# aurelienpierreeng/ansel

Hardware: AMD Instinct MI355X
Metric: MPix/s full export pixelpipe (100 MP raw); % MI355X HBM roofline (higher is better)
Workload: dtype f32

## Files before the change

### __graft_entry__.py

```python
import os
import subprocess
import sys

ROOT = os.path.dirname(os.path.abspath(__file__))
if ROOT not in sys.path:
    sys.path.insert(0, ROOT)


def build():
    from ansel_amd import build as b
    b.build()
    subprocess.check_call(["make", "-s", "-C", os.path.join(ROOT, "oracle"), "oracle"])
    subprocess.check_call(["make", "-s", "-C", os.path.join(ROOT, "oracle"), "ref"])
    nat = os.path.join(ROOT, "tests", "native")
    so = os.path.join(nat, "libdevmath_host.so")
    src = os.path.join(nat, "devmath_host.cpp")
    hdr = os.path.join(ROOT, "ansel_amd", "csrc", "devmath.h")
    if not os.path.exists(so) or os.path.getmtime(so) < max(os.path.getmtime(src), os.path.getmtime(hdr)):
        subprocess.check_call(["g++", "-O2", "-std=c++17", "-mfma", "-ffp-contract=off", "-fPIC", "-shared",
                               "-I" + os.path.join(ROOT, "ansel_amd", "csrc"), src, "-o", so, "-lm"])
    so = os.path.join(nat, "libnlm2_host.so")
    src = os.path.join(nat, "nlm2_host.cpp")
    hdrs = [os.path.join(ROOT, "ansel_amd", "csrc", h) for h in ("nlm2_body.h", "nlm3_body.h", "nlm_tail_body.h")]
    if not os.path.exists(so) or os.path.getmtime(so) < max([os.path.getmtime(src)] + [os.path.getmtime(h) for h in hdrs]):
        subprocess.check_call(["g++", "-O2", "-std=c++20", "-ffp-contract=off", "-fPIC", "-shared", "-pthread",
                               "-I" + os.path.join(ROOT, "ansel_amd", "csrc"), src, "-o", so])
    sys.path.insert(0, os.path.join(ROOT, "tests"))
    import test_amaze_host
    test_amaze_host.build()
    if os.path.isdir("/root/reference/src"):
        sys.path.insert(0, os.path.join(ROOT, "tests"))
        import test_boundary_compile
        test_boundary_compile.build()
    ex = os.path.join(ROOT, "examples", "export_pipe")
    subprocess.check_call(["gcc", "-std=c99", "-O2", "-Wall", "-I" + os.path.join(ROOT, "include"), ex + ".c",
                           "-L" + os.path.join(ROOT, "ansel_amd"), "-lansel_hip", "-Wl,-rpath,$ORIGIN/../ansel_amd", "-o", ex])
    import ansel_amd
    from ansel_amd import lib
    l = lib.load()
    if l._ansel_missing:
        raise RuntimeError("libansel_hip.so lacks: %s" % l._ansel_missing)


def smoke():
    sys.path.insert(0, os.path.join(ROOT, "tests"))
    import numpy as np
    import checkers as ck
    import hipcheck as hc
    from ansel_amd import filmic, lib, params, pipe, synth
    hc.hip()
    w, h = 400, 300
    raw = synth.bayer_mosaic(w, h, seed=1)
    lut = params.srgb_encode_lut()
    coeffs = params.unbounded_coeffs(lut)
    d_lut = lib.DeviceBuffer.from_numpy(0, lut)
    dev_nodes = pipe.light_pipe_nodes(w, h, d_lut.ptr, float(lut[0]), coeffs, with_filmic=True, filmic=filmic.default_data())
    d_in = lib.DeviceBuffer.from_numpy(0, raw)
    d_out = lib.DeviceBuffer(0, w * h * 8)
    p = pipe.DevicePipe(0, dev_nodes, fusion=True)
    groups = p.num_groups
    p.process(d_in.ptr, d_out.ptr)
    assert lib.load().dt_hip_finish(0) == 1
    got = d_out.to_numpy((h, w, 4), np.uint16)
    p.close()
    o = ck.oracle()
    assert o is not None, "oracle/liboracle.so missing: run build()"
    host_nodes = pipe.light_pipe_nodes(w, h, lut.ctypes.data, float(lut[0]), coeffs, with_filmic=True,
                                       filmic=filmic.default_data())
    src = raw
    for n in host_nodes:
        if n.op == "export_u16":
            exp = np.zeros((h, w, 4), np.uint16)
            o.oracle_export_convert_u16(w, h, ck.ptr(src), ck.ptr(exp))
            break
        dst = np.zeros((h, w) if n.op in ("rawprepare", "temperature", "highlights") else (h, w, 4), np.float32)
        assert ck.call(o, "oracle_" + n.op, n.piece, n.data, np.ascontiguousarray(src), dst) == 0, n.op
        src = dst
    bad = int((got != exp).sum())
    assert bad == 0, "smoke: %d of %d output words differ from the oracle" % (bad, got.size)
    print("smoke ok: %d-module light pipe, %d launch groups, %dx%d bit-exact vs oracle on %s"
          % (len(dev_nodes), groups, w, h, hc.hip().dt_hip_get_device_name(0).decode()))


if __name__ == "__main__":
    build()
    if len(sys.argv) > 1 and sys.argv[1] == "smoke":
        smoke()
```

### ansel_amd/csrc/hip_common.h

```cpp
#pragma once
#include <hip/hip_runtime.h>
#include <stdint.h>
#include <stdio.h>
#include <string.h>
#include "ansel_hip.h"
#include "dev_buf.h"

#ifdef ANSEL_HIP_MEASURING
#include <stdlib.h>
static inline const char *measuring_env(const char *name) { return getenv(name); }
#else
static inline constexpr const char *measuring_env(const char *) { return nullptr; }
#endif

namespace ansel
{

enum dispatch_key_t
{
  DISPATCH_NLM_V2 = 0,
  DISPATCH_NLM_FUSED,
  DISPATCH_AMAZE_UNFUSED,
  DISPATCH_AMAZE_SLAB,
  DISPATCH_AMAZE_BLOCKS,
  DISPATCH_BILAT_BLUR_SPLIT,
  DISPATCH_STRIP_ROWS,
  DISPATCH_KEYS
};
int dispatch_override(dispatch_key_t key);

static inline int strip_rows(const int gx, const int classes, const int per_class, const int longest = 32)
{
  const int forced = dispatch_override(DISPATCH_STRIP_ROWS);
  if(forced) return forced;
  int strip = longest;
  while(strip > 4 && (size_t)gx * classes * ((per_class + strip - 1) / strip) < 2048) strip /= 2;
  return strip;
}

void set_last_error(const char *fmt, ...);

hipStream_t stream_of(int devid);
int upload_small(int devid, void *dst_dev, const void *src_host, size_t bytes);
bool make_current(int devid);
int hip_device_of(int devid);
bool valid_device(int devid);

struct launch_scope
{
  int devid;
  const char *tag;
  hipEvent_t start, stop;
  bool active;
  launch_scope(int devid, const char *tag);
  ~launch_scope();
};

static inline int check_launch(const char *what)
{
  const hipError_t e = hipGetLastError();
  if(e != hipSuccess)
  {
    set_last_error("%s: %s", what, hipGetErrorString(e));
    return DT_HIP_DEFAULT_ERROR;
  }
  return DT_HIP_SUCCESS;
}

#define ANSEL_HIP_CHECK(expr)                                                                   \
  do                                                                                            \
  {                                                                                             \
    const hipError_t _e = (expr);                                                               \
    if(_e != hipSuccess)                                                                        \
    {                                                                                           \
      ansel::set_last_error("%s:%d %s: %s", __FILE__, __LINE__, #expr, hipGetErrorString(_e));  \
      return DT_HIP_DEFAULT_ERROR;                                                              \
    }                                                                                           \
  } while(0)

typedef float v4f_t __attribute__((ext_vector_type(4)));
__device__ __forceinline__ void nt_store(float4 *p, const float4 v)
{
  const v4f_t t = { v.x, v.y, v.z, v.w };
  __builtin_nontemporal_store(t, reinterpret_cast<v4f_t *>(p));
}

template <typename T> __device__ __forceinline__ const T &kernarg_at(const int offset)
{
  typedef const T __attribute__((address_space(4))) *p4;
  return *(const T *)(p4)((const char __attribute__((address_space(4))) *)__builtin_amdgcn_kernarg_segment_ptr() + offset);
}
template <typename T, typename... Before> constexpr int kernarg_offset_after()
{
  size_t off = 0;
  ((off = (off + alignof(Before) - 1) / alignof(Before) * alignof(Before) + sizeof(Before)), ...);
  return (int)((off + alignof(T) - 1) / alignof(T) * alignof(T));
}

static inline unsigned xcd_pad(const int gx) { return (unsigned)((gx + 7) / 8) * 8; }
__device__ __forceinline__ int xcd_col() { return (int)((blockIdx.x + blockIdx.y / 64) % gridDim.x); }

#define HL_MIN_CLIPPED 25
struct hl_journal
{
  unsigned long long count;
  unsigned long long index[HL_MIN_CLIPPED];
  float value[HL_MIN_CLIPPED];
};
int highlights_resolve_launch(int devid, float *out, const hl_journal *journal);

struct rcd_band_t
{
  int tv0, tv1;
  int in_row0, in_rows;
  int out_row0, out_rows;
};

struct band_view_t
{
  int frame_h;
  int buf_row0;
  int row0, row1;
};
int nlmeans_halo_rows(const dt_hip_piece_t *piece, const dt_hip_nlmeans_data_t *d);
int nlmeans_process_band(int devid, const dt_hip_piece_t *piece, const dt_hip_nlmeans_data_t *d, const band_view_t *band,
                         dt_hip_mem_t dev_in, dt_hip_mem_t dev_out);
int diffuse_halo_rows(const dt_hip_piece_t *piece, const dt_hip_diffuse_data_t *d);
int diffuse_process_rows(int devid, const dt_hip_piece_t *piece, const dt_hip_diffuse_data_t *d, int first_row,
                         dt_hip_mem_t dev_in, dt_hip_mem_t dev_out);
int diffuse_process_post_lab(int devid, const dt_hip_piece_t *piece, const dt_hip_diffuse_data_t *d, dt_hip_mem_t dev_in,
                             dt_hip_mem_t dev_out, const dt_hip_lab_data_t *lab);
int denoiseprofile_halo_rows(const dt_hip_piece_t *piece, const dt_hip_denoiseprofile_data_t *d);
struct dn_band_job_t;
int denoiseprofile_band_begin(int devid, const dt_hip_piece_t *piece, const dt_hip_denoiseprofile_data_t *d,
                              const band_view_t *band, int buf_rows, dt_hip_mem_t dev_in, dt_hip_mem_t dev_out,
                              dn_band_job_t **job);
int denoiseprofile_band_step(dn_band_job_t *job, dt_hip_mem_t *halo_buf, int *halo_rows, double **sums, size_t *sum_count);
int denoiseprofile_band_finish(dn_band_job_t *job, dt_hip_mem_t dev_out);
void denoiseprofile_band_abort(dn_band_job_t *job);
int guided_filter_launch(int devid, const float4 *guide, float *mask, int width, int height, int w, float sqrt_eps,
                         float guide_weight, float minv, float maxv);
int detail_refine_launch(int devid, const float *rawdetail, const float *form, float fill, float level, int width, int height,
                         float *refined);
int bilat_band_supported(const dt_hip_piece_t *piece, const dt_hip_bilat_data_t *d);
int blend_refines_with_detail_mask(const dt_hip_blend_data_t *d);
int bilat_band_begin(int devid, const dt_hip_piece_t *piece, const dt_hip_bilat_data_t *d, dt_hip_mem_t *grid, size_t *bytes);
int bilat_band_splat(int devid, const dt_hip_piece_t *piece, const dt_hip_bilat_data_t *d, dt_hip_mem_t grid,
                     dt_hip_mem_t in_rows, int row0, int rows);
int bilat_band_finish(int devid, const dt_hip_piece_t *piece, const dt_hip_bilat_data_t *d, dt_hip_mem_t grid,
                      dt_hip_mem_t in_rows, dt_hip_mem_t out_rows, int row0, int rows);

static inline unsigned stream_grid(size_t work_items, unsigned block)
{
  size_t g = (work_items + block - 1) / block;
  if(g > 2048u * 4u) g = 2048u * 4u;
  if(g < 1) g = 1;
  return (unsigned)g;
}

static inline unsigned pixel_grid(size_t pixels)
{
  const size_t g = (pixels + 255) / 256;
  return (unsigned)(g < 1 ? 1 : (g > 0x7fffffffu ? 0x7fffffffu : g));
}

}
```

### ansel_amd/csrc/nlm3_body.h

```cpp
#pragma once

#include "nlm2_body.h"

#include <type_traits>

#define NL3_THREADS 1024
#define NL3_TP 84
#define NL3_XO 3
#define NL3_FP 80
#define NL3_WPH 46
#define NL3_A1_LANES 384

namespace nlm3
{
using nlm2::f2;
using nlm2::imin;

struct alignas(16) f4
{
  float x, y, z, w;
};

#ifdef __HIPCC__
NLM2_FN f4 ld4(const float *const p) { return *reinterpret_cast<const f4 *>(p); }
NLM2_FN void st4(float *const p, const f4 v) { *reinterpret_cast<f4 *>(p) = v; }
NLM2_FN f2 ld2(const float *const p) { return *reinterpret_cast<const f2 *>(p); }
NLM2_FN void st2(float *const p, const f2 v) { *reinterpret_cast<f2 *>(p) = v; }
#else
NLM2_FN f4 ld4(const float *const p)
{
  f4 v;
  __builtin_memcpy(&v, p, 16);
  return v;
}
NLM2_FN void st4(float *const p, const f4 v) { __builtin_memcpy(p, &v, 16); }
NLM2_FN f2 ld2(const float *const p)
{
  f2 v;
  __builtin_memcpy(&v, p, 8);
  return v;
}
NLM2_FN void st2(float *const p, const f2 v) { __builtin_memcpy(p, &v, 8); }
#endif

template <int NPXL> constexpr int max_rows() { return NPXL == 9 ? 56 : 74; }

template <int P> constexpr int a1_segments() { return P == 1 ? 3 : 2; }

template <int NPXL, int P = 2> inline size_t lds_floats(const int chk_h, const int reach)
{
  return (size_t)4 * max_rows<NPXL>() * NL3_TP + 2 * (2 * P + 1) * NL3_FP + (size_t)(chk_h + 2 * reach) * 2 * NL3_WPH * 3;
}

constexpr int FUSED_MAXCH = 64;
template <int NPXL, int P = 2> inline size_t lds_floats_fused(const int chk_h, const int reach)
{
  return (size_t)3 * FUSED_MAXCH * NL3_TP + 2 * (2 * P + 1) * NL3_FP + (size_t)(chk_h + 2 * reach) * 2 * NL3_WPH * 3;
}
template <int MSEG, int P> inline bool a1_fits(const int chk_w, const int chk_h)
{
  constexpr int S = 2 * P + 1, NSEG = a1_segments<P>(), NCH = S * NSEG;
  static_assert(NCH <= 10, "one chain per half-wave of the five main A1 waves");
  const int ncp = (chk_w + 2 * P + 1) / 2;
  if(ncp < 32 || NCH * (ncp - 32) > 64) return false;
  const int m0 = (chk_h - 2) / S + 1;
  return (m0 + NSEG - 1) / NSEG <= MSEG;
}
template <int NPXL, int MSEG, int P = 2> inline bool fits_fused(const int chk_w, const int chk_h, const int radius, const int reach)
{
  constexpr int S = 2 * P + 1, LPR = (72 + NPXL - 1) / NPXL;
  if(radius != P || chk_w > 72 || (chk_w & 1) || chk_w + 2 * reach > 2 * NL3_WPH || chk_h > FUSED_MAXCH || chk_h < 2 * S) return false;
  if(LPR != 8) return false;
  return a1_fits<MSEG, P>(chk_w, chk_h);
}

template <int NPXL, int MSEG, int P = 2> inline bool fits(const int chk_w, const int chk_h, const int radius, const int reach)
{
  constexpr int S = 2 * P + 1, LPR = (72 + NPXL - 1) / NPXL;
  if(radius != P || chk_w > 72 || (chk_w & 1) || chk_w + 2 * reach > 2 * NL3_WPH || chk_h > max_rows<NPXL>() || chk_h < 2 * S) return false;
  if(LPR * chk_h > 448) return false;
  return a1_fits<MSEG, P>(chk_w, chk_h);
}

inline constexpr bool border_fits(const int cw, const int ch) { return ch >= 10 && cw >= 1; }

template <class I2> inline bool regular_grid(const I2 *const patches, const int n, int *const ndx_out)
{
  if(n < 1) return false;
  int ndx = 1;
  while(ndx < n && patches[ndx].x == patches[0].x) ndx++;
  if(n % ndx) return false;
  for(int p = 0; p < n; p++)
  {
    const int row = p / ndx, j = p - row * ndx;
    if(patches[p].x != patches[row * ndx].x || patches[p].y != patches[0].y + j) return false;
  }
  *ndx_out = ndx;
  return true;
}

template <int T0, int T1, int ROWBYTES, class Env, bool BLOCKS = false> struct column_chain
{
  static NLM2_FN void run(const Env &env, float *const wave_base, const int lane, float &v, const float *const term)
  {
    if constexpr(BLOCKS && T0 + 8 <= T1)
    {
      env.template chain8<T0, ROWBYTES>(wave_base, lane, v, term);
      if constexpr(T0 + 8 < T1) column_chain<T0 + 8, T1, ROWBYTES, Env, BLOCKS>::run(env, wave_base, lane, v, term);
    }
    else
    {
      v = v + term[T0];
      env.template st_addtid<T0 * ROWBYTES>(wave_base, lane, v);
      if constexpr(T0 + 1 < T1) column_chain<T0 + 1, T1, ROWBYTES, Env, BLOCKS>::run(env, wave_base, lane, v, term);
    }
  }
};

constexpr int TALL_HEAD = 64;
constexpr int TALL_SEED_PITCH = 80;
template <int NPXL, int MSEG, bool BORDER = false, bool FUSED = false, bool TALL = false, int P = 2, bool CENTER = false, class Env,
          class Args, class F4, class I2>
NLM2_FN void body(const Env &env, const F4 *__restrict__ in, F4 *__restrict__ out, const Args &a, const I2 *__restrict__ patches,
                  const int ndx, float *__restrict__ seeds_out = nullptr)
{
  static_assert(!TALL || FUSED, "the head of a tall chunk runs on the fused body");
  constexpr int S = 2 * P + 1, TP = NL3_TP, XO = NL3_XO, FP = NL3_FP, WPH = NL3_WPH;
  constexpr int NSEG = a1_segments<P>(), NCH = S * NSEG;
  constexpr int MAXCH = FUSED ? FUSED_MAXCH : max_rows<NPXL>();
  constexpr int NT = FUSED ? 3 : 4;
  auto tslot = [](const int p) { return FUSED ? p % 3 : (p & 3); };
  constexpr int LPR = (72 + NPXL - 1) / NPXL;
  const int tid = env.tid();
  const int W = a.W, H = a.H;
  const int cy_launch = env.bid() / a.nchx, cx = env.bid() - cy_launch * a.nchx;
  const int cy = cy_launch + a.cy0;
  const int top = cy * a.chk_h, left = cx * a.chk_w;
  const int bot = imin(top + a.chk_h, H), right = imin(left + a.chk_w, W);
  const int ch_grid = bot - top, cw = right - left;
  const int reach = a.reach;
  const bool interior = top >= reach && bot + reach <= H && left >= reach && right + reach <= W && ch_grid == a.chk_h && cw == a.chk_w;
  const int ch = TALL ? imin(TALL_HEAD, ch_grid) : ch_grid;
  if(BORDER ? (interior || !border_fits(cw, ch)) : !interior) return;

  float *const lds = env.lds();
  constexpr int tabsz = MAXCH * TP;
  const int wh = ch + 2 * reach;
  const int n = a.npatch, ndy = n / ndx;
  float *const XY = lds;
  float *const Z = XY + 2 * (wh * 2 * WPH);
  float *const tab = Z + wh * 2 * WPH;
  float *const Fb = tab + NT * tabsz;
  const int r0 = top - reach, c0 = left - reach;
  const float n0 = a.norm[0], n1 = a.norm[1], n2 = a.norm[2];
  const int ww = cw + 2 * reach;

  for(int i0 = tid; i0 < wh * 2 * WPH; i0 += 4 * NL3_THREADS)
  {
    F4 v[4];
#pragma unroll
    for(int u = 0; u < 4; u++)
    {
      const int i = i0 + u * NL3_THREADS;
      const int wy = i / (2 * WPH), rem = i - wy * (2 * WPH);
      const int par = rem / WPH, h = rem - par * WPH;
      const int wx = 2 * h + par;
      const int r = r0 + wy, c = c0 + wx;
      v[u].x = v[u].y = v[u].z = v[u].w = 0.0f;
      if(i < wh * 2 * WPH && wx < ww && c < W && (!BORDER || (r >= 0 && r < H && c >= 0))) v[u] = in[(long)r * W + c];
    }
#pragma unroll
    for(int u = 0; u < 4; u++)
    {
      const int i = i0 + u * NL3_THREADS;
      if(i < wh * 2 * WPH)
      {
        f2 xy;
        xy.x = v[u].x;
        xy.y = v[u].y;
        st2(XY + 2 * i, xy);
        Z[i] = v[u].z;
      }
    }
  }
  env.sync();
  auto widx = [&](const int wy, const int wx) { return (wy * 2 + (wx & 1)) * WPH + (wx >> 1); };

  const int w = tid >> 6, lane = tid & 63;
#if defined(__HIPCC__) && !defined(ANSEL_HIP_MEASURING)
  constexpr int var = 0;
#else
  const int var = a.variant;
#endif
  const bool lay1 = !FUSED && !CENTER && (var & 4096);
  const int a1_index = FUSED ? ((w >= 2 && w <= 7) ? w - 2 : -1)
                       : CENTER ? (w == 7 ? 0 : (w == 11 ? 1 : (w >= 12 ? w - 10 : -1)))
                                : (lay1 ? ((w >= 3 && w <= 6) ? w - 3 : ((w == 8 || w == 9) ? w - 4 : -1))
                                        : (w == 3 ? 0 : ((w >= 4 && w <= 7) ? w - 3 : (w == 10 ? 5 : -1))));
  const int c_index = FUSED ? w - 8
                      : CENTER ? (w <= 6 ? w - 3 : w - 4)
                               : (lay1 ? (w == 7 ? 0 : w - 9) : (w == 8 ? 0 : (w == 9 ? 1 : w - 9)));
  if(a1_index >= 0)
  {
    const int ai = a1_index;
    const int ncp = (cw + 2 * P + 1) / 2;
    constexpr int nseg = NSEG;
    const int m0 = (ch - 2) / S + 1;
    const int mseg = (m0 + nseg - 1) / nseg;
    const int extra = ncp - 32;
    int g, q;
    if(ai < 5)
    {
      q = imin(2 * ai + (lane >> 5), NCH - 1);
      g = lane & 31;
    }
    else
    {
      const int l = extra > 0 ? imin(lane, S * nseg * extra - 1) : 0;
      q = extra > 0 ? l / extra : 0;
      g = extra > 0 ? 32 + l - q * extra : 0;
    }
    const int k = q % S, seg = q / S;
    const int mk = (ch - 2 - k >= 0) ? (ch - 2 - k) / S + 1 : 0;
    const int j0 = seg * mseg;
    const int left_over = mk - j0;
    const int jn = left_over < 0 ? 0 : (left_over > mseg ? mseg : left_over);
    const bool head = seg == 0;
    const int wr0 = reach - P + k + j0 * S;
    const int x0 = 1 + 2 * g;
    const int wc0 = reach - P - 1 + x0;
    constexpr int RSTEP = S * 2 * WPH;
    const int rowbase = wr0 * 2 * WPH;
    constexpr int DUMMY = 0;
    const int toff0 = (1 + k + j0 * S) * TP + XO + x0;
    const int foff = k * FP + XO + x0;
    float ox[MSEG + 1][2], oy[MSEG + 1][2], oz[MSEG + 1][2];
#pragma unroll
    for(int i = 0; i <= MSEG; i++)
#pragma unroll
      for(int c = 0; c < 2; c++)
      {
        const int wx = wc0 + c;
        const int wi = rowbase + i * RSTEP + (wx & 1) * WPH + (wx >> 1);
        const f2 v = ld2(XY + 2 * wi);
        ox[i][c] = v.x;
        oy[i][c] = v.y;
        oz[i][c] = Z[wi];
      }
    bool own_row[MSEG + 1], row_ok[MSEG + 1], own_col[2];
#pragma unroll
    for(int i = 0; i <= MSEG; i++)
    {
      const int R = r0 + wr0 + i * S;
      own_row[i] = row_ok[i] = !BORDER || (R >= 0 && R < H);
    }
#pragma unroll
    for(int c = 0; c < 2; c++) own_col[c] = !BORDER || (c0 + wc0 + c >= 0 && c0 + wc0 + c < W);
    float sx[MSEG + 1][2], sy[MSEG + 1][2], sz[MSEG + 1][2];
#pragma unroll
    for(int i = 0; i <= MSEG; i++) sx[i][0] = sx[i][1] = sy[i][0] = sy[i][1] = sz[i][0] = sz[i][1] = 0.0f;

    auto load_row_head = [&](const int dy, const int dx) {
      const int dyo = rowbase + dy * 2 * WPH;
#pragma unroll
      for(int c = 0; c < 2; c++)
      {
        const int wx = wc0 + c + dx;
        const int base = dyo + (wx & 1) * WPH + (wx >> 1);
#pragma unroll
        for(int i = 0; i <= MSEG; i++)
        {
          const int wi = base + i * RSTEP;
          const f2 v = ld2(XY + 2 * wi);
          sx[i][c] = v.x;
          sy[i][c] = v.y;
          sz[i][c] = Z[wi];
        }
      }
    };
    auto step = [&](auto ph_tag, const int p, const int dx) {
      constexpr int PH = decltype(ph_tag)::value;
      float *const T = tab + tslot(p) * tabsz;
      float *const F = Fb + (p & 1) * S * FP;
      const int fo = head ? foff : DUMMY;
      bool col_ok[2] = { true, true };
      if(BORDER)
      {
#pragma unroll
        for(int c = 0; c < 2; c++) col_ok[c] = own_col[c] && (unsigned)(c0 + wc0 + c + dx) < (unsigned)W;
      }
      float px2[2], py2[2], pz2[2];
#pragma unroll
      for(int c = 0; c < 2; c++)
      {
        const int sl = (c + PH) & 1;
        const float dx_ = ox[0][c] - sx[0][sl], dy_ = oy[0][c] - sy[0][sl], dz_ = oz[0][c] - sz[0][sl];
        px2[c] = dx_ * dx_;
        py2[c] = dy_ * dy_;
        pz2[c] = dz_ * dz_;
        if(BORDER && !(row_ok[0] && col_ok[c])) px2[c] = py2[c] = pz2[c] = 0.0f;
      }
      {
        f2 d;
        d.x = px2[0] * n0 + py2[0] * n1 + pz2[0] * n2;
        d.y = px2[1] * n0 + py2[1] * n1 + pz2[1] * n2;
        st2(F + fo, d);
      }
#pragma unroll
      for(int i = 1; i <= MSEG; i++)
      {
        f2 t;
        float nx2[2], ny2[2], nz2[2];
#pragma unroll
        for(int c = 0; c < 2; c++)
        {
          const int sl = (c + PH) & 1;
          const float dx_ = ox[i][c] - sx[i][sl], dy_ = oy[i][c] - sy[i][sl], dz_ = oz[i][c] - sz[i][sl];
          nx2[c] = dx_ * dx_;
          ny2[c] = dy_ * dy_;
          nz2[c] = dz_ * dz_;
          if(BORDER && !(row_ok[i] && col_ok[c])) nx2[c] = ny2[c] = nz2[c] = 0.0f;
        }
        t.x = ((nx2[0] - px2[0]) * n0 + (ny2[0] - py2[0]) * n1) + (nz2[0] - pz2[0]) * n2;
        t.y = ((nx2[1] - px2[1]) * n0 + (ny2[1] - py2[1]) * n1) + (nz2[1] - pz2[1]) * n2;
        if(i - 1 < jn) st2(T + toff0 + (i - 1) * S * TP, t);
        env.sched_fence();
#pragma unroll
        for(int c = 0; c < 2; c++)
        {
          px2[c] = nx2[c];
          py2[c] = ny2[c];
          pz2[c] = nz2[c];
        }
      }
    };
    auto slide = [&](auto ph_tag, const int dy, const int dx) {
      constexpr int PH = decltype(ph_tag)::value;
      const int wx = wc0 + 1 + dx + 1;
      const int base = rowbase + dy * 2 * WPH + (wx & 1) * WPH + (wx >> 1);
#pragma unroll
      for(int i = 0; i <= MSEG; i++)
      {
        const int wi = base + i * RSTEP;
        const f2 v = ld2(XY + 2 * wi);
        sx[i][PH] = v.x;
        sy[i][PH] = v.y;
        sz[i][PH] = Z[wi];
      }
    };
    for(int dyi = 0; dyi < ndy; dyi++)
    {
      const int dy = patches[dyi * ndx].x, dx0 = patches[dyi * ndx].y;
      if(BORDER)
      {
#pragma unroll
        for(int i = 0; i <= MSEG; i++) row_ok[i] = own_row[i] && (unsigned)(r0 + wr0 + i * S + dy) < (unsigned)H;
      }
      if(!(var & 16)) load_row_head(dy, dx0);
      for(int jb = 0; jb < ndx; jb += 2)
      {
        if(!(var & 16))
        {
          step(std::integral_constant<int, 0>(), dyi * ndx + jb, dx0 + jb);
          slide(std::integral_constant<int, 0>(), dy, dx0 + jb);
        }
        env.sync();
        if(jb + 1 < ndx)
        {
          if(!(var & 16))
          {
            step(std::integral_constant<int, 1>(), dyi * ndx + jb + 1, dx0 + jb + 1);
            slide(std::integral_constant<int, 1>(), dy, dx0 + jb + 1);
          }
          env.sync();
        }
      }
    }
    env.sync();
    env.sync();
    if(!FUSED) env.sync();
    return;
  }
  if(w < 2)
  {
    const int x = 1 + w * 64 + lane;
    const bool active = x <= cw + 2 * P && !(var & 32);
    if(!(var & 512)) env.prio_high();
    env.sync();
    for(int p = 0; p < n; p++)
    {
      if(active)
      {
        float *const col = tab + tslot(p) * tabsz + XO + x;
        const float *const F = Fb + (p & 1) * S * FP + XO + x;
        float f[S], term[MAXCH];
#pragma unroll
        for(int r = 0; r < S; r++) f[r] = F[r * FP];
#pragma unroll
        for(int t = 1; t < MAXCH; t++) term[t] = col[t * TP];
        float v = 0.0f;
#pragma unroll
        for(int r = 0; r < S; r++) v += f[r];
        float *const wave_base = tab + tslot(p) * tabsz + XO + 1 + w * 64;
        env.template st_addtid<0>(wave_base, lane, v);
        column_chain<1, MAXCH, TP * 4, Env, !FUSED && P == 2 && !CENTER>::run(env, wave_base, lane, v, term);
        if constexpr(TALL)
        {
          static_assert(!TALL || MAXCH == TALL_HEAD, "the exported sum is the one behind the head's last row");
          seeds_out[(size_t)p * TALL_SEED_PITCH + x] = v;
        }
      }
      env.sync();
    }
    env.sync();
    if(!FUSED) env.sync();
    return;
  }
  if(!FUSED && w == 2)
  {
    const bool active = lane < ch && !(var & 64);
    if(!(var & 512)) env.prio_high();
    env.sync();
    env.sync();
    for(int p = 0; p < n; p++)
    {
      if(active)
      {
        float *const rowp = tab + (p & 3) * tabsz + lane * TP;
        float cs[80];
#pragma unroll
        for(int b = 4; b < 80; b += 4)
        {
          const f4 v = ld4(rowp + b);
          cs[b] = v.x;
          cs[b + 1] = v.y;
          cs[b + 2] = v.z;
          cs[b + 3] = v.w;
        }
        cs[XO] = 0.0f;
        float distortion = 0.0f;
#pragma unroll
        for(int kk = 1; kk < S; kk++) distortion += cs[XO + kk];
        float d[72];
#pragma unroll
        for(int b = 0; b < 72; b += 4)
        {
#pragma unroll
          for(int c = b; c < b + 4; c++)
          {
            distortion = distortion + (cs[XO + c + S] - cs[XO + c]);
            d[c] = distortion;
          }
          f4 v;
          v.x = d[b];
          v.y = d[b + 1];
          v.z = d[b + 2];
          v.w = d[b + 3];
          st4(rowp + 4 + b, v);
          if(!(var & 1024)) env.sched_fence();
        }
      }
      env.sync();
    }
    env.sync();
    return;
  }
  {
    constexpr int NR = CENTER ? NPXL : NPXL + 1;
    constexpr int DB = CENTER ? 1 : 2;
    constexpr int AB = CENTER ? 1 : 3;
    static_assert(CENTER || NR % 2 == 0, "the distortions alternate between two register sets with the ring's period");
    const int ci = c_index;
    static_assert(LPR == 8, "the lane layout of the C role");
    const int r = 8 * ci + 2 * ((lane & 31) >> 3) + (lane >> 5), j8 = lane & 7;
    const int cb = NPXL * j8;
    const bool active = r < ch && cb < cw && !(var & 128);
    float accx[NPXL], accy[NPXL], accz[NPXL], accw[NPXL];
    float qx[NR], qy[NR], qz[NR];
    float dist[DB][NPXL];
    unsigned reached[2] = { ~0u, ~0u };
#pragma unroll
    for(int i = 0; i < NPXL; i++) accx[i] = accy[i] = accz[i] = accw[i] = dist[0][i] = dist[DB - 1][i] = 0.0f;
#pragma unroll
    for(int i = 0; i < NR; i++) qx[i] = qy[i] = qz[i] = 0.0f;
    const int doff = r * TP + 4 + cb;
    const float sharp_m23 = a.sharpness * -8388608.0f;
    [[maybe_unused]] float ox[CENTER ? NPXL : 1], oy[CENTER ? NPXL : 1], oz[CENTER ? NPXL : 1];
    [[maybe_unused]] const float cden = 1.0f + a.center_weight;
    [[maybe_unused]] const float crcp = Env::rcp_refined(cden);
    if constexpr(CENTER)
    {
#pragma unroll
      for(int i = 0; i < NPXL; i++)
      {
        const int wi = widx(reach + r, reach + cb + i);
        const f2 v = ld2(XY + 2 * wi);
        ox[i] = v.x;
        oy[i] = v.y;
        oz[i] = Z[wi];
      }
    }
    [[maybe_unused]] float cs[NPXL + S];
    [[maybe_unused]] const bool row_head = j8 == 0;
    [[maybe_unused]] auto fetch_sums = [&](const int p) {
      const float *const T = tab + tslot(p) * tabsz + r * TP + XO + cb;
#pragma unroll
      for(int i = 0; i < NPXL + S; i++) cs[i] = T[i];
    };
    [[maybe_unused]] auto row_chain = [&](auto m_tag) {
      constexpr int M = decltype(m_tag)::value;
      float e[NPXL];
      e[0] = cs[S] - (row_head ? 0.0f : cs[0]);
#pragma unroll
      for(int i = 1; i < NPXL; i++) e[i] = cs[i + S] - cs[i];
      float first = 0.0f;
#pragma unroll
      for(int kk = 1; kk < S; kk++) first += cs[kk];
      float carry = first;
#pragma unroll
      for(int ph = 0; ph < LPR; ph++)
      {
        float d = carry;
#pragma unroll
        for(int i = 0; i < NPXL; i++)
        {
          d = d + e[i];
          dist[M & (DB - 1)][i] = d;
        }
        if(ph + 1 < LPR)
        {
          const float from_left = env.lane_shr1(d);
          carry = row_head ? first : from_left;
        }
      }
    };

    auto fetch = [&](auto m_tag, const int p, const bool first, const int dy, const int dx) {
      constexpr int M = decltype(m_tag)::value;
      if constexpr(!FUSED)
      {
        const float *const T = tab + (p & 3) * tabsz + doff;
#pragma unroll
        for(int i = 0; i < NPXL; i++) dist[M & (DB - 1)][i] = T[i];
      }
      if(BORDER)
      {
        unsigned m = 0;
        if((unsigned)(top + r + dy) < (unsigned)H)
        {
#pragma unroll
          for(int i = 0; i < NPXL; i++) m |= ((unsigned)(left + cb + i + dx) < (unsigned)W ? 1u : 0u) << i;
        }
        reached[M & (DB - 1)] = m;
      }
      const int wy = reach + r + dy;
      if(first)
      {
#pragma unroll
        for(int i = 0; i < NPXL; i++)
        {
          const int wi = widx(wy, reach + cb + i + dx);
          const f2 v = ld2(XY + 2 * wi);
          qx[i] = v.x;
          qy[i] = v.y;
          qz[i] = Z[wi];
        }
      }
      else
      {
        constexpr int SL = (NPXL - 1 + M) % NR;
        const int wi = widx(wy, reach + cb + NPXL - 1 + dx);
        const f2 v = ld2(XY + 2 * wi);
        qx[SL] = v.x;
        qy[SL] = v.y;
        qz[SL] = Z[wi];
      }
    };
    auto accumulate = [&](auto m_tag) {
      constexpr int M = decltype(m_tag)::value;
      static_assert(NPXL % AB == 0, "accumulate() takes the pixels of a lane AB at a time");
#pragma unroll
      for(int g = 0; g < NPXL; g += AB)
      {
        float v[AB], wgt[AB], t[AB];
        int k0[AB];
        if constexpr(CENTER)
        {
          float cx2[AB], cy2[AB], cz2[AB];
#pragma unroll
          for(int j = 0; j < AB; j++)
          {
            const float dx_ = ox[g + j] - qx[(g + j + M) % NR], dy_ = oy[g + j] - qy[(g + j + M) % NR], dz_ = oz[g + j] - qz[(g + j + M) % NR];
            cx2[j] = dx_ * dx_ * a.cpn;
            cy2[j] = dy_ * dy_ * a.cpn;
            cz2[j] = dz_ * dz_ * a.cpn;
          }
          env.sched_fence();
#pragma unroll
          for(int j = 0; j < AB; j++) v[j] = dist[M & (DB - 1)][g + j] + (cx2[j] + cy2[j] + cz2[j]);
          env.sched_fence();
#pragma unroll
          for(int j = 0; j < AB; j++) v[j] = Env::div_uniform(v[j], cden, crcp);
          env.sched_fence();
#pragma unroll
          for(int j = 0; j < AB; j++) v[j] = Env::min_num(0.0f, v[j] * sharp_m23 + 16777216.0f);
          env.sched_fence();
        }
        else
        {
#pragma unroll
          for(int j = 0; j < AB; j++) v[j] = dist[M & (DB - 1)][g + j] * sharp_m23;
          env.sched_fence();
#pragma unroll
          for(int j = 0; j < AB; j++) v[j] = Env::max_num(v[j], -__builtin_inff());
          env.sched_fence();
        }
#pragma unroll
        for(int j = 0; j < AB; j++) k0[j] = Env::cvt_i32_sat(v[j]);
        env.sched_fence();
#pragma unroll
        for(int j = 0; j < AB; j++) k0[j] = (int)(0x3f800000u + (unsigned)k0[j]);
        env.sched_fence();
#pragma unroll
        for(int j = 0; j < AB; j++)
        {
          wgt[j] = Env::int_as_float(k0[j] >= 0x800000 ? k0[j] : 0);
          if(BORDER && !(reached[M & (DB - 1)] >> (g + j) & 1u)) wgt[j] = 0.0f;
        }
        env.sched_fence();
#pragma unroll
        for(int j = 0; j < AB; j++) t[j] = qx[(g + j + M) % NR] * wgt[j];
        env.sched_fence();
#pragma unroll
        for(int j = 0; j < AB; j++) accx[g + j] = accx[g + j] + t[j];
#pragma unroll
        for(int j = 0; j < AB; j++) t[j] = qy[(g + j + M) % NR] * wgt[j];
        env.sched_fence();
#pragma unroll
        for(int j = 0; j < AB; j++) accy[g + j] = accy[g + j] + t[j];
#pragma unroll
        for(int j = 0; j < AB; j++) t[j] = qz[(g + j + M) % NR] * wgt[j];
        env.sched_fence();
#pragma unroll
        for(int j = 0; j < AB; j++) accz[g + j] = accz[g + j] + t[j];
#pragma unroll
        for(int j = 0; j < AB; j++) accw[g + j] = accw[g + j] + 1.0f * wgt[j];
        env.sched_fence();
      }
    };
    env.sync();
    env.sync();
    if(!FUSED) env.sync();
    for(int dyi = 0; dyi < ndy; dyi++)
    {
      const int dy = patches[dyi * ndx].x, dx0 = patches[dyi * ndx].y;
      for(int jb = 0; jb < ndx; jb += NR)
      {
        auto run = [&](auto m_tag) {
          constexpr int M = decltype(m_tag)::value;
          if constexpr(M < NR)
          {
            if(jb + M < ndx)
            {
              if constexpr(CENTER)
              {
                if(active && jb + M > 0) accumulate(std::integral_constant<int, (M + NR - 1) % NR>());
                if constexpr(FUSED) fetch_sums(dyi * ndx + jb + M);
                if(active) fetch(m_tag, dyi * ndx + jb + M, jb + M == 0, dy, dx0 + jb + M);
                if constexpr(FUSED)
                {
                  if(!(var & 64)) row_chain(m_tag);
                }
                if(active && jb + M + 1 == ndx) accumulate(m_tag);
              }
              else if constexpr(FUSED)
              {
                if(active && jb + M > 0) accumulate(std::integral_constant<int, (M + NR - 1) % NR>());
                env.sched_fence();
                fetch_sums(dyi * ndx + jb + M);
                if(active) fetch(m_tag, dyi * ndx + jb + M, jb + M == 0, dy, dx0 + jb + M);
                if(!(var & 64)) row_chain(m_tag);
                if(active && jb + M + 1 == ndx) accumulate(m_tag);
              }
              else if(active)
              {
                if(jb + M > 0) accumulate(std::integral_constant<int, (M + NR - 1) % NR>());
                env.sched_fence();
                fetch(m_tag, dyi * ndx + jb + M, jb + M == 0, dy, dx0 + jb + M);
                if(jb + M + 1 == ndx) accumulate(m_tag);
              }
              env.sync();
            }
          }
        };
        run(std::integral_constant<int, 0>());
        run(std::integral_constant<int, 1>());
        run(std::integral_constant<int, 2>());
        run(std::integral_constant<int, 3>());
        run(std::integral_constant<int, 4>());
        run(std::integral_constant<int, 5>());
        run(std::integral_constant<int, 6>());
        run(std::integral_constant<int, 7>());
        run(std::integral_constant<int, 8>());
        run(std::integral_constant<int, 9>());
        if constexpr(NR > 10)
        {
          run(std::integral_constant<int, 10>());
          run(std::integral_constant<int, 11>());
          run(std::integral_constant<int, 12>());
          run(std::integral_constant<int, 13>());
        }
      }
    }
    if(!active) return;
    const int row = top + r;
    if(row < a.out_row0 || row >= a.out_row1) return;
#pragma unroll
    for(int i = 0; i < NPXL; i++)
    {
      if(cb + i >= cw) continue;
      const long o = (long)row * W + left + cb + i;
      F4 res;
      if(a.skip_blend)
      {
        res.x = accx[i] / accw[i];
        res.y = accy[i] / accw[i];
        res.z = accz[i] / accw[i];
        res.w = accw[i] / accw[i];
      }
      else
      {
        const F4 ip = in[o];
        res.x = (ip.x * (1.0f - a.luma)) + (accx[i] / accw[i] * a.luma);
        res.y = (ip.y * (1.0f - a.chroma)) + (accy[i] / accw[i] * a.chroma);
        res.z = (ip.z * (1.0f - a.chroma)) + (accz[i] / accw[i] * a.chroma);
        res.w = (ip.w * 0.0f) + (accw[i] / accw[i] * 1.0f);
      }
      out[o] = res;
      env.store_cell(a, o, res.x);
    }
  }
}

}
```

### ansel_amd/csrc/nlmeans.hip

```cpp
#include "hip_common.h"
#include "nlmeans_core_params.h"
#include "nlm2_body.h"
#include "ieee_inrange.h"
#include "px_bilat.h"
#include "nlm3_body.h"
#include "nlm_tail_body.h"

#include <math.h>
#include <algorithm>
#include <vector>
#include <type_traits>

using namespace ansel;

namespace
{

#define SLICE_WIDTH 72
#define SLICE_HEIGHT 60
#define NLM_THREADS 1024
#define MAX_PX_PER_THREAD 5
#define CS_LANES 128

struct nlm_args
{
  int W, H;
  int chk_w, chk_h, nchx;
  int radius, npatch;
  int cs_pitch, wt_pitch;
  float sharpness, center_weight, inv_den;
  float cpn;
  float norm[3];
  float luma, chroma;
  int skip_blend;
  int reach;
  int win_pitch;
  int cy0, out_row0, out_row1;
  int variant;
  float2 *zc;
  float zc_sigma_r;
  int zc_size_z;
};

__device__ __forceinline__ void nlm_store_cell(const nlm_args &a, const long o, const float L)
{
  if(a.zc)
  {
    float zf;
    const int zi = bilat_axis(L, a.zc_sigma_r, a.zc_size_z, zf);
    a.zc[o] = make_float2(zf, __int_as_float(zi));
  }
}

__device__ __forceinline__ int imin(const int a, const int b) { return a < b ? a : b; }
__device__ __forceinline__ int imax(const int a, const int b) { return a > b ? a : b; }

__device__ __forceinline__ int cvtt(const float v)
{
  return (v >= -2147483648.0f && v < 2147483648.0f) ? (int)v : (int)0x80000000;
}

__device__ __forceinline__ float mexp2(const float x)
{
  const int k0 = (int)(0x3f800000u + (unsigned)cvtt(x * -8388608.0f));
  return __int_as_float(k0 >= 0x800000 ? k0 : 0);
}

__device__ __forceinline__ float pixdiff(const float4 a, const float4 b, const float n0, const float n1, const float n2)
{
  const float dx = a.x - b.x, dy = a.y - b.y, dz = a.z - b.z;
  return dx * dx * n0 + dy * dy * n1 + dz * dz * n2;
}

__device__ __forceinline__ float pixdiff2(const float4 a, const float4 b, const float4 c, const float4 d, const float n0,
                                          const float n1, const float n2)
{
  const float ax = a.x - b.x, ay = a.y - b.y, az = a.z - b.z;
  const float cx = c.x - d.x, cy = c.y - d.y, cz = c.z - d.z;
  return (ax * ax - cx * cx) * n0 + (ay * ay - cy * cy) * n1 + (az * az - cz * cz) * n2;
}

template <bool STAGED> struct pixel_source
{
  const float4 *in;
  const float *wr, *wg, *wb;
  int W, r0, c0, pitch;
  __device__ __forceinline__ float4 operator()(const int r, const int c) const
  {
    if(STAGED)
    {
      const int i = (r - r0) * pitch + (c - c0);
      return make_float4(wr[i], wg[i], wb[i], 0.0f);
    }
    return in[(long)r * W + c];
  }
};

template <bool STAGED>
__global__ __launch_bounds__(NLM_THREADS) void nlm_chunks(const float4 *__restrict__ in, float4 *__restrict__ out,
                                                          const nlm_args a, const int2 *__restrict__ patches)
{
  extern __shared__ float lds[];
  const int tid = threadIdx.x;
  const int cy_launch = blockIdx.x / a.nchx, cx = blockIdx.x - cy_launch * a.nchx;
  const int cy = cy_launch + a.cy0;
  const int top = cy * a.chk_h, left = cx * a.chk_w;
  const int bot = imin(top + a.chk_h, a.H), right = imin(left + a.chk_w, a.W);
  const int ch = bot - top, cw = right - left;
  const int P = a.radius, W = a.W, H = a.H;
  const int csw = a.chk_w + 2 * P + 1;
  const int cs0 = left - P - 1;
  float *const cs = lds;
  float *const dist = lds + (a.chk_h + 16) * a.cs_pitch;
  const float n0 = a.norm[0], n1 = a.norm[1], n2 = a.norm[2];

  pixel_source<STAGED> px;
  px.in = in;
  px.W = W;
  px.r0 = top - a.reach;
  px.c0 = left - a.reach;
  px.pitch = a.win_pitch;
  if(STAGED)
  {
    float *const win = dist + a.chk_h * a.wt_pitch;
    const int wh = a.chk_h + 2 * a.reach, plane = wh * a.win_pitch;
    px.wr = win;
    px.wg = win + plane;
    px.wb = win + 2 * plane;
    for(int i = tid; i < plane; i += NLM_THREADS)
    {
      const int wy = i / a.win_pitch, wx = i - wy * a.win_pitch;
      const int r = px.r0 + wy, c = px.c0 + wx;
      float4 v = make_float4(0.f, 0.f, 0.f, 0.f);
      if(r >= 0 && r < H && c >= 0 && c < W) v = in[(long)r * W + c];
      win[i] = v.x;
      win[i + plane] = v.y;
      win[i + 2 * plane] = v.z;
    }
    __syncthreads();
  }

  float4 acc[MAX_PX_PER_THREAD];
  int rc[MAX_PX_PER_THREAD];
#pragma unroll
  for(int k = 0; k < MAX_PX_PER_THREAD; k++)
  {
    acc[k] = make_float4(0.f, 0.f, 0.f, 0.f);
    const int idx = tid + NLM_THREADS * k;
    const int r = idx / cw;
    rc[k] = idx < ch * cw ? ((r << 16) | (idx - r * cw)) : -1;
  }

  for(int p = 0; p < a.npatch; p++)
  {
    const int srow = patches[p].x, scol = patches[p].y;
    const int row_min = imax(top, imax(0, -srow)), row_max = imin(bot, H - imax(0, srow));
    if(row_min >= row_max) continue;
    const int row_top = imax(row_min, imax(P, P - srow));
    const int row_bot = imin(row_max, H - 1 - imax(P, P + srow));
    const int col_min = imax(left, -scol), col_max = imin(right, W - scol);
    const int pc_min = left - imin(P, imin(left, left + scol));
    const int pc_max = right + imin(P, imin(W - right, W - (right + scol)));
    const int nrows = row_max - row_min;
    const int first_end = imin(row_top, row_bot);

    const int ci = tid & (CS_LANES - 1);
    for(int t = tid / CS_LANES; t < nrows; t += NLM_THREADS / CS_LANES)
    {
      if(ci >= csw) continue;
      const int c = cs0 + ci;
      float v = 0.0f;
      if(c >= pc_min && c < pc_max)
      {
        if(t == 0)
        {
          const int row = row_min;
          const int rmin = row - imin(P, imin(row, row + srow));
          const int rmax = row + imin(P, imin(H - 1 - row, H - 1 - (row + srow)));
          for(int r = rmin; r <= rmax; r++) v += pixdiff(px(r, c), px(r + srow, c + scol), n0, n1, n2);
        }
        else
        {
          const int row = row_min + t - 1;
          if(row < first_end)
          {
            const int b = row + 1 + P;
            v = pixdiff(px(b, c), px(b + srow, c + scol), n0, n1, n2);
          }
          else if(row < row_bot)
          {
            const int b = row + 1 + P, tt = row - P;
            v = pixdiff2(px(b, c), px(b + srow, c + scol), px(tt, c), px(tt + srow, c + scol), n0, n1, n2);
          }
          else if(row >= row_top)
          {
            const int tt = row - P;
            v = pixdiff(px(tt, c), px(tt + srow, c + scol), n0, n1, n2);
          }
        }
      }
      cs[t * a.cs_pitch + ci] = v;
    }
    __syncthreads();

    if(tid < csw)
    {
      float v = cs[tid];
      for(int t0 = 1; t0 < nrows; t0 += 16)
      {
        float term[16];
        float *const col = cs + t0 * a.cs_pitch + tid;
#pragma unroll
        for(int u = 0; u < 16; u++) term[u] = col[u * a.cs_pitch];
#pragma unroll
        for(int u = 0; u < 16; u++)
        {
          const int row = row_min + t0 + u - 1;
          const bool live = t0 + u < nrows;
          const float plus = v + term[u], minus = v - term[u];
          v = (live && row < row_bot) ? plus : ((live && row >= row_top) ? minus : v);
          term[u] = v;
        }
#pragma unroll
        for(int u = 0; u < 16; u++) col[u * a.cs_pitch] = term[u];
      }
    }
    __syncthreads();

    if(tid < nrows)
    {
      const float *const row_cs = cs + tid * a.cs_pitch - cs0;
      float distortion = 0.0f;
      for(int i = col_min - P; i < imin(col_min + P, col_max); i++) distortion += row_cs[i];
      float *const drow = dist + (row_min + tid - top) * a.wt_pitch - left;
      for(int c0 = col_min; c0 < col_max; c0 += 16)
      {
        float hi[16], lo[16];
#pragma unroll
        for(int u = 0; u < 16; u++)
        {
          hi[u] = row_cs[c0 + u + P];
          lo[u] = row_cs[c0 + u - P - 1];
        }
#pragma unroll
        for(int u = 0; u < 16; u++)
        {
          const float next = distortion + (hi[u] - lo[u]);
          distortion = (c0 + u < col_max) ? next : distortion;
          hi[u] = distortion;
        }
#pragma unroll
        for(int u = 0; u < 16; u++) drow[c0 + u] = hi[u];
      }
    }
    __syncthreads();

#pragma unroll
    for(int k = 0; k < MAX_PX_PER_THREAD; k++)
    {
      if(rc[k] < 0) continue;
      const int row = top + (rc[k] >> 16), col = left + (rc[k] & 0xffff);
      if(row < row_min || row >= row_max || col < col_min || col >= col_max) continue;
      const float distortion = dist[(row - top) * a.wt_pitch + (col - left)];
      const float4 q = px(row + srow, col + scol);
      float w;
      if(a.center_weight < 0)
        w = mexp2(distortion * a.sharpness);
      else
      {
        const float dis = (distortion + pixdiff(px(row, col), q, a.cpn, a.cpn, a.cpn)) / (1.0f + a.center_weight);
        w = mexp2(fmaxf(0.0f, dis * a.sharpness - 2.0f));
      }
      acc[k].x += q.x * w;
      acc[k].y += q.y * w;
      acc[k].z += q.z * w;
      acc[k].w += 1.0f * w;
    }
    __syncthreads();
  }

#pragma unroll
  for(int k = 0; k < MAX_PX_PER_THREAD; k++)
  {
    if(rc[k] < 0) continue;
    const int row = top + (rc[k] >> 16), col = left + (rc[k] & 0xffff);
    if(row < a.out_row0 || row >= a.out_row1) continue;
    const long o = (long)row * W + col;
    const float4 s = acc[k];
    float4 r;
    if(a.skip_blend)
      r = make_float4(s.x / s.w, s.y / s.w, s.z / s.w, s.w / s.w);
    else
    {
      const float4 ip = in[o];
      r.x = (ip.x * (1.0f - a.luma)) + (s.x / s.w * a.luma);
      r.y = (ip.y * (1.0f - a.chroma)) + (s.y / s.w * a.chroma);
      r.z = (ip.z * (1.0f - a.chroma)) + (s.z / s.w * a.chroma);
      r.w = (ip.w * 0.0f) + (s.w / s.w * 1.0f);
    }
    out[o] = r;
    nlm_store_cell(a, o, r.x);
  }
}

#define NLP_SERIAL 256
#define NLP_PAR (NLM_THREADS - NLP_SERIAL)
#define NLP_PX 7
#define NLP_WP 96
#define NLP_TP 81

typedef float f2 __attribute__((ext_vector_type(2)));

struct nlm_geom
{
  int srow, scol, row_min, row_max, row_top, row_bot, col_min, col_max, pc_min, pc_max, nrows;
};

__device__ __forceinline__ nlm_geom geom_of(const int2 sh, const int top, const int bot, const int left, const int right,
                                            const int P, const int W, const int H)
{
  nlm_geom g;
  g.srow = sh.x;
  g.scol = sh.y;
  g.row_min = imax(top, imax(0, -g.srow));
  g.row_max = imin(bot, H - imax(0, g.srow));
  g.nrows = g.row_max - g.row_min;
  g.row_top = imax(g.row_min, imax(P, P - g.srow));
  g.row_bot = imin(g.row_max, H - 1 - imax(P, P + g.srow));
  g.col_min = imax(left, -g.scol);
  g.col_max = imin(right, W - g.scol);
  g.pc_min = left - imin(P, imin(left, left + g.scol));
  g.pc_max = right + imin(P, imin(W - right, W - (right + g.scol)));
  return g;
}

__device__ __forceinline__ void pipelined_body(const int chunk, float *const lds, const float4 *__restrict__ in,
                                               float4 *__restrict__ out, const nlm_args &a, const int2 *__restrict__ patches)
{
  const int tid = threadIdx.x;
  const int cy_launch = chunk / a.nchx, cx = chunk - cy_launch * a.nchx;
  const int cy = cy_launch + a.cy0;
  const int top = cy * a.chk_h, left = cx * a.chk_w;
  const int bot = imin(top + a.chk_h, a.H), right = imin(left + a.chk_w, a.W);
  const int ch = bot - top, cw = right - left;
  const int P = a.radius, W = a.W, H = a.H;
  const int csw = a.chk_w + 2 * P + 1;
  const int cs0 = left - P - 1;
  constexpr int pitch = NLP_TP;
  const int tabsz = a.chk_h * pitch;
  float *const win = lds + 2 * tabsz + 16 * pitch + 64;
  const int r0 = top - a.reach, c0 = left - a.reach;
  const float n0 = a.norm[0], n1 = a.norm[1], n2 = a.norm[2];
  const int n = a.npatch;

  {
    const int wh = a.chk_h + 2 * a.reach;
    for(int i = tid; i < wh * NLP_WP; i += NLM_THREADS)
    {
      const int wy = i / NLP_WP, wx = i - wy * NLP_WP;
      const int r = r0 + wy, c = c0 + wx;
      float4 v = make_float4(0.f, 0.f, 0.f, 0.f);
      if(r >= 0 && r < H && c >= 0 && c < W) v = in[(long)r * W + c];
      float *const w = win + wy * 3 * NLP_WP + wx;
      w[0] = v.x;
      w[NLP_WP] = v.y;
      w[2 * NLP_WP] = v.z;
    }
  }

  const bool par = tid >= NLP_SERIAL;
  if(!par) __builtin_amdgcn_s_setprio(3);
  const int u = tid - NLP_SERIAL;
  float4 acc[NLP_PX];
  int prc[NLP_PX];
#pragma unroll
  for(int k = 0; k < NLP_PX; k++)
  {
    acc[k] = make_float4(0.f, 0.f, 0.f, 0.f);
    const int idx = u + NLP_PAR * k;
    const int r = idx / cw, c = idx - r * cw;
    const bool ok = par && idx < ch * cw;
    prc[k] = ok ? ((r << 16) | c) : -1;
  }
  const int wbase0 = ((top - r0) * 3) * NLP_WP + (left - c0);
  int a1[NLP_PX];
#pragma unroll
  for(int k = 0; k < NLP_PX; k++)
  {
    const int idx = u + NLP_PAR * k;
    const int t = idx / (csw - 1), ci = 1 + idx - t * (csw - 1);
    a1[k] = (t * 3 * NLP_WP + ci) | (((t + 1) * pitch + ci) << 16);
  }
  __syncthreads();

  auto run = [&](auto interior_tag) {
    constexpr bool INTERIOR = decltype(interior_tag)::value;
    auto A1 = [&](const nlm_geom &g, float *const T) {
      const int dS = g.srow * 3 * NLP_WP + g.scol;
      const int dT = (2 * P + 1) * 3 * NLP_WP;
      const float *const wb = win + ((g.row_min + 1 + P - r0) * 3) * NLP_WP + (cs0 - c0);
      const int tend = g.nrows * pitch;
      const bool plain = INTERIOR || (g.row_top <= g.row_min && g.row_bot >= g.row_max - 1 && g.pc_min == left - P
                         && g.pc_max == left + a.chk_w + P);
      const f2 n01 = { n0, n1 };
      if(u < g.nrows - 1) T[(u + 1) * pitch] = 0.0f;
      if(plain)
      {
  #pragma unroll
        for(int k = 0; k < NLP_PX; k++)
        {
          if(k == 4) asm volatile("" ::: "memory");
          int pk = a1[k];
          asm volatile("" : "+v"(pk));
          const int ti = (unsigned)pk >> 16;
          if(ti >= tend) continue;
          const float *const pb = wb + (pk & 0xffff);
          const float *const pt = pb - dT;
          const f2 b = { pb[0], pb[NLP_WP] }, bs = { pb[dS], pb[dS + NLP_WP] };
          const f2 l = { pt[0], pt[NLP_WP] }, ls = { pt[dS], pt[dS + NLP_WP] };
          const f2 z = { pb[2 * NLP_WP], pt[2 * NLP_WP] }, zs = { pb[dS + 2 * NLP_WP], pt[dS + 2 * NLP_WP] };
          f2 e = b - bs, q = l - ls, w = z - zs;
          e = e * e;
          q = q * q;
          w = w * w;
          const f2 d = (e - q) * n01;
          T[ti] = d.x + d.y + (w.x - w.y) * n2;
        }
      }
      else
      {
  #pragma unroll
        for(int k = 0; k < NLP_PX; k++)
        {
          if(k == 4) asm volatile("" ::: "memory");
          int pk = a1[k];
          asm volatile("" : "+v"(pk));
          const int ti = (unsigned)pk >> 16;
          if(ti >= tend) continue;
          const int lw = pk & 0xffff;
          const int t = (int)(((unsigned)lw * 58255u) >> 24);
          const int row = g.row_min + t, c = cs0 + (lw - t * 3 * NLP_WP);
          const float *const pb = wb + lw;
          const float *const pt = pb - dT;
          const float ax = pb[0] - pb[dS], ay = pb[NLP_WP] - pb[dS + NLP_WP], az = pb[2 * NLP_WP] - pb[dS + 2 * NLP_WP];
          const float tx = pt[0] - pt[dS], ty = pt[NLP_WP] - pt[dS + NLP_WP], tz = pt[2 * NLP_WP] - pt[dS + 2 * NLP_WP];
          const bool colok = c >= g.pc_min && c < g.pc_max;
          const bool enter = colok && row < g.row_bot, leave = colok && row >= g.row_top;
          const float ex = enter ? ax * ax : 0.f, ey = enter ? ay * ay : 0.f, ez = enter ? az * az : 0.f;
          const float lx = leave ? tx * tx : 0.f, ly = leave ? ty * ty : 0.f, lz = leave ? tz * tz : 0.f;
          T[ti] = (ex - lx) * n0 + (ey - ly) * n1 + (ez - lz) * n2;
        }
      }
    };
    auto A1_first = [&](const nlm_geom &g, float *const T) {
      const int c = cs0 + tid;
      float v = 0.0f;
      if(c >= g.pc_min && c < g.pc_max)
      {
        const int row = g.row_min;
        const int rmin = row - imin(P, imin(row, row + g.srow));
        const int rmax = row + imin(P, imin(H - 1 - row, H - 1 - (row + g.srow)));
        const int dS = g.srow * 3 * NLP_WP + g.scol;
        const float *pr = win + ((rmin - r0) * 3) * NLP_WP + (c - c0);
        for(int r = rmin; r <= rmax; r++, pr += 3 * NLP_WP)
        {
          const float dx = pr[0] - pr[dS], dy = pr[NLP_WP] - pr[dS + NLP_WP], dz = pr[2 * NLP_WP] - pr[dS + 2 * NLP_WP];
          v += dx * dx * n0 + dy * dy * n1 + dz * dz * n2;
        }
      }
      T[tid] = v;
    };
    auto A2 = [&](const nlm_geom &g, float *const T) {
      float v = T[tid];
      int t0 = 1;
      for(; t0 + 16 <= g.nrows; t0 += 16)
      {
        float term[16];
        float *const col = T + t0 * pitch + tid;
  #pragma unroll
        for(int k = 0; k < 16; k++) term[k] = col[k * pitch];
        term[0] = v + term[0];
  #pragma unroll
        for(int k = 1; k < 16; k++) term[k] = term[k - 1] + term[k];
        v = term[15];
  #pragma unroll
        for(int k = 0; k < 16; k++) col[k * pitch] = term[k];
      }
      if(t0 < g.nrows)
      {
        float term[16];
        float *const col = T + t0 * pitch + tid;
        const int live = g.nrows - t0;
  #pragma unroll
        for(int k = 0; k < 16; k++) term[k] = col[k * pitch];
  #pragma unroll
        for(int k = 0; k < 16; k++)
        {
          const float next = v + term[k];
          v = k < live ? next : v;
          term[k] = v;
        }
  #pragma unroll
        for(int k = 0; k < 16; k++)
          if(k < live) col[k * pitch] = term[k];
      }
    };
    auto B = [&](const nlm_geom &g, float *const T, const int rr) {
      float *const rowp = T + rr * pitch - cs0;
      float distortion = 0.0f;
      for(int i = g.col_min - P; i < imin(g.col_min + P, g.col_max); i++) distortion += rowp[i];
      int cb = g.col_min;
      for(; cb + 16 <= g.col_max; cb += 16)
      {
        float hi[16], lo[16];
  #pragma unroll
        for(int k = 0; k < 16; k++)
        {
          hi[k] = rowp[cb + k + P];
          lo[k] = rowp[cb + k - P - 1];
        }
  #pragma unroll
        for(int k = 0; k < 16; k++) hi[k] = hi[k] - lo[k];
        hi[0] = distortion + hi[0];
  #pragma unroll
        for(int k = 1; k < 16; k++) hi[k] = hi[k - 1] + hi[k];
        distortion = hi[15];
  #pragma unroll
        for(int k = 0; k < 16; k++) rowp[cb + k - P - 1] = hi[k];
      }
      if(cb < g.col_max)
      {
        float hi[16], lo[16];
        const int live = g.col_max - cb;
  #pragma unroll
        for(int k = 0; k < 16; k++)
        {
          hi[k] = rowp[cb + k + P];
          lo[k] = rowp[cb + k - P - 1];
        }
  #pragma unroll
        for(int k = 0; k < 16; k++)
        {
          const float next = distortion + (hi[k] - lo[k]);
          distortion = k < live ? next : distortion;
          hi[k] = distortion;
        }
  #pragma unroll
        for(int k = 0; k < 16; k++)
          if(k < live) rowp[cb + k - P - 1] = hi[k];
      }
    };
    auto C = [&](const nlm_geom &g, const float *const T) {
      const int dS = g.srow * 3 * NLP_WP + g.scol;
      const int trow = (g.row_min - top) * pitch;
      const bool whole = INTERIOR || (g.row_min == top && g.row_max == bot && g.col_min == left && g.col_max == right);
      float dist[NLP_PX], qx[NLP_PX], qy[NLP_PX], qz[NLP_PX];
      bool ok[NLP_PX];
  #pragma unroll
      for(int k = 0; k < NLP_PX; k++)
      {
        int pk = prc[k];
        asm volatile("" : "+v"(pk));
        const int r = pk >> 16, c = pk & 0xffff;
        ok[k] = pk >= 0;
        if(!whole)
        {
          const int row = top + r, col = left + c;
          ok[k] = ok[k] && row >= g.row_min && row < g.row_max && col >= g.col_min && col < g.col_max;
        }
        const int ti = ok[k] ? __mul24(r, pitch) + c - trow : 0;
        dist[k] = T[ti];
        const float *const pq = win + (wbase0 + dS) + __mul24(r, 3 * NLP_WP) + c;
        qx[k] = pq[0];
        qy[k] = pq[NLP_WP];
        qz[k] = pq[2 * NLP_WP];
      }
      if(a.center_weight < 0)
      {
  #pragma unroll
        for(int k = 0; k < NLP_PX; k++)
        {
          const float w = mexp2(dist[k] * a.sharpness);
          const float sx = acc[k].x + qx[k] * w, sy = acc[k].y + qy[k] * w, sz = acc[k].z + qz[k] * w, sw = acc[k].w + 1.0f * w;
          acc[k].x = ok[k] ? sx : acc[k].x;
          acc[k].y = ok[k] ? sy : acc[k].y;
          acc[k].z = ok[k] ? sz : acc[k].z;
          acc[k].w = ok[k] ? sw : acc[k].w;
        }
      }
      else
      {
  #pragma unroll
        for(int k = 0; k < NLP_PX; k++)
        {
          int pk = prc[k];
          asm volatile("" : "+v"(pk));
          const float *const pp = win + wbase0 + __mul24(pk >> 16, 3 * NLP_WP) + (pk & 0xffff);
          const float dx = pp[0] - qx[k], dy = pp[NLP_WP] - qy[k], dz = pp[2 * NLP_WP] - qz[k];
          const float dis = (dist[k] + (dx * dx * a.cpn + dy * dy * a.cpn + dz * dz * a.cpn)) / (1.0f + a.center_weight);
          const float w = mexp2(fmaxf(0.0f, dis * a.sharpness - 2.0f));
          const float sx = acc[k].x + qx[k] * w, sy = acc[k].y + qy[k] * w, sz = acc[k].z + qz[k] * w, sw = acc[k].w + 1.0f * w;
          acc[k].x = ok[k] ? sx : acc[k].x;
          acc[k].y = ok[k] ? sy : acc[k].y;
          acc[k].z = ok[k] ? sz : acc[k].z;
          acc[k].w = ok[k] ? sw : acc[k].w;
        }
      }
    };

    auto geom = [&](const int2 sh) {
      if(!INTERIOR) return geom_of(sh, top, bot, left, right, P, W, H);
      nlm_geom g;
      g.srow = sh.x;
      g.scol = sh.y;
      g.row_min = g.row_top = top;
      g.row_max = g.row_bot = bot;
      g.nrows = ch;
      g.col_min = left;
      g.col_max = right;
      g.pc_min = left - P;
      g.pc_max = right + P;
      return g;
    };
    int2 sh_prev = make_int2(0, 0), sh_cur = patches[0], sh_next = patches[n > 1 ? 1 : 0];
    {
      const nlm_geom g = geom(sh_cur);
      if(g.nrows > 0)
      {
        if(par) A1(g, lds);
        else if(tid < csw) A1_first(g, lds);
      }
    }
    __syncthreads();
    for(int i = 0; i <= n; i++)
    {
      const int2 sh_next2 = patches[i + 2 < n ? i + 2 : n - 1];
      float *const Ti = lds + (i & 1) * tabsz;
      float *const To = lds + ((i + 1) & 1) * tabsz;
      if(par)
      {
        if(i >= 1)
        {
          const nlm_geom g = geom(sh_prev);
          if(g.nrows > 0) C(g, To);
        }
      }
      else if(tid < csw && i < n)
      {
        const nlm_geom g = geom(sh_cur);
        if(g.nrows > 0) A2(g, Ti);
      }
      __syncthreads();
      if(par)
      {
        if(i + 1 < n)
        {
          const nlm_geom g = geom(sh_next);
          if(g.nrows > 0) A1(g, To);
        }
      }
      else if(tid < 128)
      {
        if(tid < csw && i + 1 < n)
        {
          const nlm_geom g = geom(sh_next);
          if(g.nrows > 0) A1_first(g, To);
        }
      }
      else if(i < n)
      {
        const nlm_geom g = geom(sh_cur);
        if(tid - 128 < g.nrows) B(g, Ti, tid - 128);
      }
      __syncthreads();
      sh_prev = sh_cur;
      sh_cur = sh_next;
      sh_next = sh_next2;
    }

  };
  const bool interior = top >= a.reach && bot + a.reach <= H && left >= a.reach && right + a.reach <= W && ch == a.chk_h
                        && cw == a.chk_w;
  if(interior)
    run(std::true_type{});
  else
    run(std::false_type{});

#pragma unroll
  for(int k = 0; k < NLP_PX; k++)
  {
    if(prc[k] < 0) continue;
    const int row = top + (prc[k] >> 16), col = left + (prc[k] & 0xffff);
    if(row < a.out_row0 || row >= a.out_row1) continue;
    const long o = (long)row * W + col;
    const float4 s = acc[k];
    float4 r;
    if(a.skip_blend)
      r = make_float4(s.x / s.w, s.y / s.w, s.z / s.w, s.w / s.w);
    else
    {
      const float4 ip = in[o];
      r.x = (ip.x * (1.0f - a.luma)) + (s.x / s.w * a.luma);
      r.y = (ip.y * (1.0f - a.chroma)) + (s.y / s.w * a.chroma);
      r.z = (ip.z * (1.0f - a.chroma)) + (s.z / s.w * a.chroma);
      r.w = (ip.w * 0.0f) + (s.w / s.w * 1.0f);
    }
    out[o] = r;
    nlm_store_cell(a, o, r.x);
  }
}

__global__ __launch_bounds__(NLM_THREADS) void nlm_chunks_pipelined(const float4 *__restrict__ in, float4 *__restrict__ out,
                                                                    const nlm_args a, const int2 *__restrict__ patches)
{
  extern __shared__ float lds[];
  pipelined_body(blockIdx.x, lds, in, out, a, patches);
}

#pragma clang diagnostic push
#pragma clang diagnostic ignored "-Winline-asm"
struct nlm2_device_env
{
  float *lds_;
  int chunk_;
  __device__ __forceinline__ int tid() const { return threadIdx.x; }
  __device__ __forceinline__ int bid() const { return chunk_; }
  __device__ __forceinline__ float *lds() const { return lds_; }
  __device__ __forceinline__ void sync() const { __syncthreads(); }
  __device__ __forceinline__ void prio_high() const { __builtin_amdgcn_s_setprio(3); }
  __device__ __forceinline__ void store_cell(const nlm_args &a, const long o, const float L) const { nlm_store_cell(a, o, L); }
  __device__ __forceinline__ void sched_fence() const { __builtin_amdgcn_sched_barrier(0); }
  template <int OFF> __device__ __forceinline__ void st_addtid(float *const wave_base, const int, const float v) const
  {
    const unsigned m0v = __builtin_amdgcn_readfirstlane((unsigned)(size_t)(__attribute__((address_space(3))) float *)wave_base);
    asm volatile("s_mov_b32 m0, %0\n\ts_nop 0\n\tds_write_addtid_b32 %1 offset:%2" : : "s"(m0v), "v"(v), "n"(OFF) : "memory", "m0");
  }
  template <int T0, int ROWBYTES> __device__ __forceinline__ void chain8(float *const wave_base, const int, float &v, const float *const term) const
  {
    const unsigned m0v = __builtin_amdgcn_readfirstlane((unsigned)(size_t)(__attribute__((address_space(3))) float *)wave_base);
    asm volatile("s_mov_b32 m0, %[b]\n\ts_nop 0\n\t"
                 "v_add_f32 %[v], %[v], %[t0]\n\tds_write_addtid_b32 %[v] offset:%[o0]\n\t"
                 "v_add_f32 %[v], %[v], %[t1]\n\tds_write_addtid_b32 %[v] offset:%[o1]\n\t"
                 "v_add_f32 %[v], %[v], %[t2]\n\tds_write_addtid_b32 %[v] offset:%[o2]\n\t"
                 "v_add_f32 %[v], %[v], %[t3]\n\tds_write_addtid_b32 %[v] offset:%[o3]\n\t"
                 "v_add_f32 %[v], %[v], %[t4]\n\tds_write_addtid_b32 %[v] offset:%[o4]\n\t"
                 "v_add_f32 %[v], %[v], %[t5]\n\tds_write_addtid_b32 %[v] offset:%[o5]\n\t"
                 "v_add_f32 %[v], %[v], %[t6]\n\tds_write_addtid_b32 %[v] offset:%[o6]\n\t"
                 "v_add_f32 %[v], %[v], %[t7]\n\tds_write_addtid_b32 %[v] offset:%[o7]"
                 : [v] "+v"(v)
                 : [b] "s"(m0v), [t0] "v"(term[T0]), [t1] "v"(term[T0 + 1]), [t2] "v"(term[T0 + 2]), [t3] "v"(term[T0 + 3]),
                   [t4] "v"(term[T0 + 4]), [t5] "v"(term[T0 + 5]), [t6] "v"(term[T0 + 6]), [t7] "v"(term[T0 + 7]),
                   [o0] "n"(T0 * ROWBYTES), [o1] "n"((T0 + 1) * ROWBYTES), [o2] "n"((T0 + 2) * ROWBYTES), [o3] "n"((T0 + 3) * ROWBYTES),
                   [o4] "n"((T0 + 4) * ROWBYTES), [o5] "n"((T0 + 5) * ROWBYTES), [o6] "n"((T0 + 6) * ROWBYTES), [o7] "n"((T0 + 7) * ROWBYTES)
                 : "memory", "m0");
  }
  __device__ __forceinline__ bool any(const bool c) const { return __builtin_amdgcn_ballot_w64(c) != 0; }
  __device__ __forceinline__ float lane_shr1(const float v) const
  {
    return __int_as_float(__builtin_amdgcn_update_dpp(0, __float_as_int(v), 0x111, 0xf, 0xf, true));
  }
  static constexpr bool TIMED = false;
  __device__ __forceinline__ long long clock() const { return 0; }
  static __device__ __forceinline__ float int_as_float(const int v) { return __int_as_float(v); }
  static __device__ __forceinline__ float max_num(const float a, const float b) { return __builtin_fmaxf(a, b); }
  static __device__ __forceinline__ float min_num(const float a, const float b) { return __builtin_fminf(a, b); }
  static __device__ __forceinline__ int cvt_i32_sat(const float v)
  {
    int r;
    asm("v_cvt_i32_f32 %0, %1" : "=v"(r) : "v"(v));
    return r;
  }
  static __device__ __forceinline__ float rcp_refined(const float d) { return ansel_ieee::rcp_refined(d); }
  static __device__ __forceinline__ float div_uniform(const float n, const float d, const float y1) { return ansel_ieee::div_uniform(n, d, y1); }
};
#pragma clang diagnostic pop

template <int P, int WP, int TP, bool DEEP, bool CENTER>
__global__ __launch_bounds__(NL2_THREADS) void nlm_chunks_v2(const float4 *__restrict__ in, float4 *__restrict__ out,
                                                             const nlm_args a, const int2 *__restrict__ patches,
                                                             const int *__restrict__ order, const int n_border)
{
  extern __shared__ float lds[];
  const int chunk = order[blockIdx.x];
  if(blockIdx.x < n_border)
  {
    pipelined_body(chunk, lds, in, out, a, patches);
    return;
  }
  nlm2_device_env env;
  env.lds_ = lds;
  env.chunk_ = chunk;
  nlm2::body<P, WP, TP, DEEP, CENTER>(env, in, out, a, patches);
}

#ifdef ANSEL_HIP_MEASURING
struct nlm2_timed_env : nlm2_device_env
{
  static constexpr bool TIMED = true;
  __device__ __forceinline__ long long clock() const { return (long long)__builtin_readcyclecounter(); }
};
__global__ __launch_bounds__(NL2_THREADS) void nlm_chunks_v2_timed(const float4 *__restrict__ in, float4 *__restrict__ out,
                                                                   const nlm_args a, const int2 *__restrict__ patches,
                                                                   const int *__restrict__ order, const int n_border)
{
  extern __shared__ float lds[];
  if(blockIdx.x < n_border) return;
  nlm2_timed_env env;
  env.lds_ = lds;
  env.chunk_ = order[blockIdx.x];
  nlm2::body<2, NL2_WP_TIGHT, NL2_TP_TIGHT, true>(env, in, out, a, patches);
}
#endif

template <int NPXL, int MSEG, int P = 2, bool CENTER = false>
__global__ __launch_bounds__(NL3_THREADS) void nlm_chunks_v3(const float4 *__restrict__ in, float4 *__restrict__ out,
                                                             const nlm_args a_by_value, const int2 *__restrict__ patches,
                                                             const int *__restrict__ order, const int n_border, const int ndx)
{
  constexpr int at = kernarg_offset_after<nlm_args, const float4 *, float4 *>();
  static_assert(at == 16, "nlm_chunks_v3: the by-value nlm_args follows the two plane pointers");
  const nlm_args &a = kernarg_at<nlm_args>(at);
  (void)a_by_value;
  extern __shared__ float lds[];
  const int chunk = order[blockIdx.x];
  nlm2_device_env env;
  env.lds_ = lds;
  env.chunk_ = chunk;
  if(blockIdx.x < n_border)
  {
    const int cy = chunk / a.nchx + a.cy0, cx = chunk % a.nchx;
    const int cw = min(a.chk_w, a.W - cx * a.chk_w), ch = min(a.chk_h, a.H - cy * a.chk_h);
    if(a.variant & 2048 || !nlm3::border_fits(cw, ch)) pipelined_body(chunk, lds, in, out, a, patches);
    else nlm3::body<NPXL, MSEG, true, false, false, P, CENTER>(env, in, out, a, patches, ndx);
    return;
  }
  nlm3::body<NPXL, MSEG, false, false, false, P, CENTER>(env, in, out, a, patches, ndx);
}

template <int NPXL, int MSEG, bool TALL, int P = 2, bool CENTER = false>
__global__ __launch_bounds__(NL3_THREADS) void nlm_chunks_v4(const float4 *__restrict__ in, float4 *__restrict__ out,
                                                             const nlm_args a_by_value, const int2 *__restrict__ patches,
                                                             const int *__restrict__ order, const int n_border, const int ndx,
                                                             float *__restrict__ seeds)
{
  constexpr int at = kernarg_offset_after<nlm_args, const float4 *, float4 *>();
  static_assert(at == 16, "nlm_chunks_v4: the by-value nlm_args follows the two plane pointers");
  const nlm_args &a = kernarg_at<nlm_args>(at);
  (void)a_by_value;
  extern __shared__ float lds[];
  const int chunk = order[blockIdx.x];
  nlm2_device_env env;
  env.lds_ = lds;
  env.chunk_ = chunk;
  if(blockIdx.x < n_border)
  {
    const int cy = chunk / a.nchx + a.cy0, cx = chunk % a.nchx;
    const int cw = min(a.chk_w, a.W - cx * a.chk_w), ch = min(a.chk_h, a.H - cy * a.chk_h);
    if(!nlm3::border_fits(cw, TALL ? min(ch, nlm3::TALL_HEAD) : ch)) pipelined_body(chunk, lds, in, out, a, patches);
    else nlm3::body<NPXL, MSEG, true, true, TALL, P, CENTER>(env, in, out, a, patches, ndx,
                                                             TALL ? seeds + (size_t)blockIdx.x * a.npatch * nlm3::TALL_SEED_PITCH : nullptr);
    return;
  }
  nlm3::body<NPXL, MSEG, false, true, TALL, P, CENTER>(env, in, out, a, patches, ndx,
                                                       TALL ? seeds + (size_t)blockIdx.x * a.npatch * nlm3::TALL_SEED_PITCH : nullptr);
}

template <bool BORDER, int P = 2, bool CENTER = false>
__global__ __launch_bounds__(NLT_THREADS, 8) void nlm_tail(const float4 *__restrict__ in, float4 *__restrict__ out,
                                                           const nlm_args a, const int2 *__restrict__ patches,
                                                           const int *__restrict__ order, const int first,
                                                           const float *__restrict__ seeds)
{
  extern __shared__ float lds[];
  nlm2_device_env env;
  env.lds_ = lds;
  const int pos = first + (int)blockIdx.x;
  env.chunk_ = order[pos];
  nlmt::body<BORDER, P, CENTER>(env, in, out, a, patches, seeds + (size_t)pos * a.npatch * NLT_SEED_PITCH);
}

typedef void (*nlm2_kernel_t)(const float4 *, float4 *, nlm_args, const int2 *, const int *, int);
template <int P, bool CENTER> nlm2_kernel_t nlm2_kernel_of_(const bool tight, const bool deep)
{
  if(tight) return deep ? nlm_chunks_v2<P, NL2_WP_TIGHT, NL2_TP_TIGHT, true, CENTER> : nlm_chunks_v2<P, NL2_WP_TIGHT, NL2_TP_TIGHT, false, CENTER>;
  return deep ? nlm_chunks_v2<P, NL2_WP_LOOSE, NL2_TP_LOOSE, true, CENTER> : nlm_chunks_v2<P, NL2_WP_LOOSE, NL2_TP_LOOSE, false, CENTER>;
}
template <int P> nlm2_kernel_t nlm2_kernel_of(const bool tight, const bool deep, const bool center)
{
  return center ? nlm2_kernel_of_<P, true>(tight, deep) : nlm2_kernel_of_<P, false>(tight, deep);
}

int sgn(const int v) { return (v > 0) - (v < 0); }

int scatter(const float scale, const float scattering, const int i1, const int i2)
{
  const int a1 = abs(i1), a2 = abs(i2);
  return (int)(scale * ((a1 * a1 * a1 + 7.0 * a1 * sqrt((double)a2)) * sgn(i1) * scattering / 6.0 + i1));
}

int slice_height(const int height)
{
  if(height % SLICE_HEIGHT == 0) return SLICE_HEIGHT;
  int best = height % SLICE_HEIGHT, best_incr = 0;
  for(int incr = 1; incr < 10; incr++)
  {
    const int plus = height % (SLICE_HEIGHT + incr);
    if(plus == 0) return SLICE_HEIGHT + incr;
    if(plus > best)
    {
      best_incr = incr;
      best = plus;
    }
    const int minus = height % (SLICE_HEIGHT - incr);
    if(minus == 0) return SLICE_HEIGHT - incr;
    if(minus > best)
    {
      best_incr = -incr;
      best = minus;
    }
  }
  return SLICE_HEIGHT + best_incr;
}

int slice_width(const int width)
{
  int sl = SLICE_WIDTH;
  int rem = width % sl;
  if(rem < SLICE_WIDTH / 2 && (width % (sl - 4)) > rem)
  {
    sl -= 4;
    rem = width % sl;
    if(rem < SLICE_WIDTH / 2 && (width % (sl - 4)) > rem) sl -= 4;
  }
  return sl;
}

}

namespace ansel
{

enum { NLM_BODY_NONE = 0, NLM_BODY_TALL, NLM_BODY_V4, NLM_BODY_V3, NLM_BODY_V2, NLM_BODY_PIPELINED, NLM_BODY_STAGED, NLM_BODY_GLOBAL };
static int g_nlm_last[8];

int nlmeans_core_launch(int devid, const float4 *in, float4 *out, int width, int height, const nlm_core_params_t &p)
{
  if(p.band && (p.band->frame_h <= 0 || p.band->row0 < 0 || p.band->row1 > p.band->frame_h || p.band->row0 >= p.band->row1))
    return DT_HIP_INVALID_ARG;
  if(width <= 0 || height <= 0) return DT_HIP_SUCCESS;
  if(p.patch_radius < 0 || p.patch_radius > 16 || p.search_radius < 0 || p.search_radius > 32)
  {
    set_last_error("nlmeans: patch radius %d / search radius %d outside the device limits (16 / 32)", p.patch_radius,
                   p.search_radius);
    return DT_HIP_INVALID_ARG;
  }
  const int K = p.search_radius;
  std::vector<int2> patches;
  int max_shift = 0;
  for(int ri = -K; ri <= K; ri++)
    for(int ci = -K; ci <= K; ci++)
    {
      const int r = scatter(p.scale, p.scattering, ri, ci), c = scatter(p.scale, p.scattering, ci, ri);
      patches.push_back(make_int2(r, c));
      max_shift = std::max(max_shift, std::max(abs(r), abs(c)));
    }
  nlm_args a;
  memset(&a, 0, sizeof(a));
  const band_view_t *const bv = p.band;
  if(bv) height = bv->frame_h;
  a.W = width;
  a.H = height;
  a.chk_h = slice_height(height);
  a.chk_w = slice_width(width);
  a.nchx = (width + a.chk_w - 1) / a.chk_w;
  a.cy0 = bv ? bv->row0 / a.chk_h : 0;
  a.out_row0 = bv ? bv->row0 : 0;
  a.out_row1 = bv ? bv->row1 : height;
  const int nchy = bv ? (bv->row1 + a.chk_h - 1) / a.chk_h - a.cy0 : (height + a.chk_h - 1) / a.chk_h;
  if(bv)
  {
    in -= (size_t)bv->buf_row0 * width;
    out -= (size_t)bv->row0 * width;
  }
  a.radius = p.patch_radius;
  a.npatch = (int)patches.size();
  a.cs_pitch = (a.chk_w + 2 * a.radius + 1) | 1;
  a.wt_pitch = (a.chk_w + 16) | 1;
  a.zc = p.band ? nullptr : p.cell_out;
  a.zc_sigma_r = p.cell_sigma_r;
  a.zc_size_z = p.cell_size_z;
  a.sharpness = p.sharpness;
  a.center_weight = p.center_weight;
  a.cpn = p.center_weight * (2 * p.patch_radius + 1) * (2 * p.patch_radius + 1);
  for(int k = 0; k < 3; k++) a.norm[k] = p.norm[k];
  a.luma = p.luma;
  a.chroma = p.chroma;
  a.skip_blend = (p.luma == 1.0 && p.chroma == 1.0);
  if(a.chk_w * a.chk_h > NLM_THREADS * MAX_PX_PER_THREAD || a.chk_h > NLM_THREADS
     || a.chk_w + 2 * a.radius + 1 > CS_LANES)
  {
    set_last_error("nlmeans: chunk %d x %d exceeds the kernel's accumulator budget", a.chk_w, a.chk_h);
    return DT_HIP_DEFAULT_ERROR;
  }
  a.reach = a.radius + 1 + max_shift;
  a.win_pitch = (a.chk_w + 2 * a.reach) | 1;
  const size_t pipe_bytes = ((size_t)2 * a.chk_h * NLP_TP + 16 * NLP_TP + 64
                             + (size_t)(a.chk_h + 2 * a.reach) * 3 * NLP_WP) * sizeof(float);
  const bool pipelined = pipe_bytes <= 160 * 1024 && a.chk_w + 2 * a.reach <= NLP_WP && a.chk_h <= NLP_SERIAL / 2
                         && a.chk_w + 2 * a.radius + 1 <= NLP_TP && a.chk_w * a.chk_h <= NLP_PAR * NLP_PX;
  const size_t table_bytes = ((size_t)(a.chk_h + 16) * a.cs_pitch + (size_t)a.chk_h * a.wt_pitch + 64) * sizeof(float);
  const size_t window_bytes = (size_t)3 * (a.chk_h + 2 * a.reach) * a.win_pitch * sizeof(float);
  const bool staged = table_bytes + window_bytes <= 160 * 1024;
  const size_t lds_bytes = pipelined ? pipe_bytes : table_bytes + (staged ? window_bytes : 0);
  hipStream_t s = stream_of(devid);
  const void *const fn = pipelined ? (const void *)nlm_chunks_pipelined
                                   : (staged ? (const void *)nlm_chunks<true> : (const void *)nlm_chunks<false>);
  if(lds_bytes > 64 * 1024)
    ANSEL_HIP_CHECK(hipFuncSetAttribute(fn, hipFuncAttributeMaxDynamicSharedMemorySize, (int)lds_bytes));
  const int S2 = 2 * a.radius + 1, ncol2 = a.chk_w + 2 * a.radius;
  const bool tight = a.chk_w + 2 * a.reach <= NL2_WP_TIGHT && ncol2 + 1 <= NL2_TP_TIGHT && measuring_env("ANSEL_NLM2_LAYOUT") == nullptr;
  const int WP2 = tight ? NL2_WP_TIGHT : NL2_WP_LOOSE, TP2 = tight ? NL2_TP_TIGHT : NL2_TP_LOOSE;
  const bool deep = nlm2::lds_floats(4, a.chk_h, a.reach, a.npatch, WP2, TP2) * sizeof(float) <= 160 * 1024 && a.chk_h <= 64
                    && measuring_env("ANSEL_NLM2_DEEP") == nullptr;
  const size_t v2_bytes = std::max(nlm2::lds_floats(deep ? 4 : 2, a.chk_h, a.reach, a.npatch, WP2, TP2) * sizeof(float), pipe_bytes);
  const bool center = !(p.center_weight < 0);
  bool v2 = pipelined && a.radius >= 1 && a.radius <= 3 && ncol2 * S2 <= NL2_PAR
            && a.chk_w * a.chk_h <= NL2_PAR * NL2_PX && a.chk_w + 2 * a.reach <= WP2 && ncol2 + 1 <= TP2 && a.npatch <= 4096
            && a.chk_h <= NL2_SERIAL / 2 && v2_bytes <= 160 * 1024 && measuring_env("ANSEL_HIP_NLM_V1") == nullptr;
  if(v2)
  {
    const int nseg = NL2_PAR / (ncol2 * S2), m0 = (a.chk_h - 2) / S2 + 1;
    v2 = (m0 + nseg - 1) / nseg <= NL2_MSEG;
  }
  int ndx3 = 0;
  const bool force_v2 = dispatch_override(DISPATCH_NLM_V2) || measuring_env("ANSEL_HIP_NLM_V2") != nullptr;
  const bool p1 = a.radius == 1;
  const float cden = 1.0f + p.center_weight;
  const bool center_ok = !center || (cden >= 1.0f && cden <= 1048576.0f && p.sharpness >= 0x1p-60f && p.sharpness <= 0x1p60f);
  const bool v3 = v2 && center_ok && (p1 ? nlm3::fits<9, 7, 1>(a.chk_w, a.chk_h, a.radius, a.reach) : nlm3::fits<9, 6>(a.chk_w, a.chk_h, a.radius, a.reach))
                  && nlm3::regular_grid(patches.data(), a.npatch, &ndx3) && !force_v2;
  const size_t v3_bytes = std::max((p1 ? nlm3::lds_floats<9, 1>(a.chk_h, a.reach) : nlm3::lds_floats<9>(a.chk_h, a.reach)) * sizeof(float), pipe_bytes);
  const size_t v4_bytes = std::max((p1 ? nlm3::lds_floats_fused<9, 1>(a.chk_h, a.reach) : nlm3::lds_floats_fused<9>(a.chk_h, a.reach)) * sizeof(float), pipe_bytes);
  const char *const fused_env = measuring_env("ANSEL_HIP_NLM_FUSED");
  const bool force_fused = dispatch_override(DISPATCH_NLM_FUSED) || (fused_env && atoi(fused_env) != 0);
  const bool v4 = v2 && center_ok
                  && (p1 ? nlm3::fits_fused<9, 7, 1>(a.chk_w, a.chk_h, a.radius, a.reach) : nlm3::fits_fused<9, 7>(a.chk_w, a.chk_h, a.radius, a.reach))
                  && nlm3::regular_grid(patches.data(), a.npatch, &ndx3)
                  && v4_bytes <= 160 * 1024 && !force_v2 && (force_fused || !(v3 && v3_bytes <= 160 * 1024));
  typedef void (*nlm3_kernel_t)(const float4 *, float4 *, nlm_args, const int2 *, const int *, int, int);
  typedef void (*nlm4_kernel_t)(const float4 *, float4 *, nlm_args, const int2 *, const int *, int, int, float *);
  const nlm3_kernel_t k3 = p1 ? (center ? nlm_chunks_v3<9, 7, 1, true> : nlm_chunks_v3<9, 7, 1, false>)
                              : (center ? nlm_chunks_v3<9, 6, 2, true> : nlm_chunks_v3<9, 6, 2, false>);
  const nlm4_kernel_t k4 = p1 ? (center ? nlm_chunks_v4<9, 7, false, 1, true> : nlm_chunks_v4<9, 7, false, 1, false>)
                              : (center ? nlm_chunks_v4<9, 7, false, 2, true> : nlm_chunks_v4<9, 7, false, 2, false>);
  static_assert(NLT_HEAD_ROWS == nlm3::TALL_HEAD && NLT_SEED_PITCH == nlm3::TALL_SEED_PITCH, "head and tail share the export's layout");
  const size_t tall_bytes = std::max((p1 ? nlm3::lds_floats_fused<9, 1>(NLT_HEAD_ROWS, a.reach) : nlm3::lds_floats_fused<9>(NLT_HEAD_ROWS, a.reach)) * sizeof(float), pipe_bytes);
  const size_t tail_bytes = nlmt::lds_floats(a.chk_h - NLT_HEAD_ROWS, a.reach, a.npatch) * sizeof(float);
  bool tall = v2 && center_ok && !v3 && !v4 && !force_v2
                    && (p1 ? nlmt::fits<1>(a.chk_w, a.chk_h, a.radius, a.reach, a.npatch) && nlm3::fits_fused<9, 7, 1>(a.chk_w, NLT_HEAD_ROWS, a.radius, a.reach)
                           : nlmt::fits<2>(a.chk_w, a.chk_h, a.radius, a.reach, a.npatch) && nlm3::fits_fused<9, 7>(a.chk_w, NLT_HEAD_ROWS, a.radius, a.reach))
                    && nlm3::regular_grid(patches.data(), a.npatch, &ndx3)
                    && tall_bytes <= 160 * 1024 && tail_bytes <= 64 * 1024;
  const nlm4_kernel_t k4t = p1 ? (center ? nlm_chunks_v4<9, 7, true, 1, true> : nlm_chunks_v4<9, 7, true, 1, false>)
                               : (center ? nlm_chunks_v4<9, 7, true, 2, true> : nlm_chunks_v4<9, 7, true, 2, false>);
  typedef void (*nlmt_kernel_t)(const float4 *, float4 *, nlm_args, const int2 *, const int *, int, const float *);
  const nlmt_kernel_t kt_ring = p1 ? (center ? nlm_tail<true, 1, true> : nlm_tail<true, 1, false>) : (center ? nlm_tail<true, 2, true> : nlm_tail<true, 2, false>);
  const nlmt_kernel_t kt_in = p1 ? (center ? nlm_tail<false, 1, true> : nlm_tail<false, 1, false>) : (center ? nlm_tail<false, 2, true> : nlm_tail<false, 2, false>);
  static_assert(NL2_SERIAL == NLP_SERIAL && NL2_THREADS == NLM_THREADS && NL3_THREADS == NLM_THREADS,
                "nlm_chunks_v2 / _v3 share the launch shape of nlm_chunks_pipelined");
  nlm2_kernel_t k2 = nullptr;
  const int nchunks = a.nchx * nchy;
  std::vector<int> order;
  int n_border = 0;
  if(v2)
  {
    k2 = a.radius == 1 ? nlm2_kernel_of<1>(tight, deep, center)
                       : (a.radius == 2 ? nlm2_kernel_of<2>(tight, deep, center) : nlm2_kernel_of<3>(tight, deep, center));
#ifdef ANSEL_HIP_MEASURING
    if(a.radius == 2 && tight && deep && measuring_env("ANSEL_NLM2_TIMED")) k2 = nlm_chunks_v2_timed;
#endif
    if(v2_bytes > 64 * 1024)
      ANSEL_HIP_CHECK(hipFuncSetAttribute((const void *)k2, hipFuncAttributeMaxDynamicSharedMemorySize, (int)v2_bytes));
    const char *const var_env = measuring_env("ANSEL_NLM2_VARIANT");
    a.variant = var_env ? atoi(var_env) : 0;
    order.resize(nchunks);
    std::vector<int> inner;
    inner.reserve(nchunks);
    for(int c = 0; c < nchunks; c++)
    {
      const int cyl = c / a.nchx, cx = c - cyl * a.nchx, cy = cyl + a.cy0;
      const int top = cy * a.chk_h, left = cx * a.chk_w;
      const int bot = std::min(top + a.chk_h, a.H), right = std::min(left + a.chk_w, a.W);
      const bool interior = top >= a.reach && bot + a.reach <= a.H && left >= a.reach && right + a.reach <= a.W
                            && bot - top == a.chk_h && right - left == a.chk_w;
      if(interior) inner.push_back(c);
      else order[n_border++] = c;
    }
    std::copy(inner.begin(), inner.end(), order.begin() + n_border);
  }
  const size_t patch_bytes = patches.size() * sizeof(int2), order_bytes = order.size() * sizeof(int);
  std::vector<unsigned char> host_blob(patch_bytes + order_bytes);
  memcpy(host_blob.data(), patches.data(), patch_bytes);
  if(order_bytes) memcpy(host_blob.data() + patch_bytes, order.data(), order_bytes);
  const dev_buf_t patches_buf = dev_buf_t::alloc(devid, host_blob.size());
  int2 *const dev_patches = patches_buf.as<int2>();
  if(!dev_patches) return DT_HIP_SYSMEM_ALLOCATION;
  if(const int uerr = upload_small(devid, dev_patches, host_blob.data(), host_blob.size()); uerr != DT_HIP_SUCCESS) return uerr;
  const int *const dev_order = (const int *)((const unsigned char *)dev_patches + patch_bytes);
  dev_buf_t seeds_buf;
  if(tall)
  {
    seeds_buf = dev_buf_t::alloc(devid, (size_t)nchunks * a.npatch * NLT_SEED_PITCH * sizeof(float));
    if(!seeds_buf) tall = false;
  }
  float *const seeds = seeds_buf.as<float>();
  hipError_t attr_err = hipSuccess;
  if(tall)
    attr_err = hipFuncSetAttribute((const void *)k4t, hipFuncAttributeMaxDynamicSharedMemorySize, (int)tall_bytes);
  else if(v4)
    attr_err = hipFuncSetAttribute((const void *)k4, hipFuncAttributeMaxDynamicSharedMemorySize, (int)v4_bytes);
  else if(v3 && v3_bytes <= 160 * 1024)
    attr_err = hipFuncSetAttribute((const void *)k3, hipFuncAttributeMaxDynamicSharedMemorySize, (int)v3_bytes);
  if(attr_err != hipSuccess)
  {
    set_last_error("%s:%d hipFuncSetAttribute(nlm_chunks): %s", __FILE__, __LINE__, hipGetErrorString(attr_err));
    return DT_HIP_DEFAULT_ERROR;
  }
  {
    const bool third = v3 && v3_bytes <= 160 * 1024;
    g_nlm_last[0] = tall ? NLM_BODY_TALL : v4 ? NLM_BODY_V4 : third ? NLM_BODY_V3 : v2 ? NLM_BODY_V2
                    : pipelined ? NLM_BODY_PIPELINED : staged ? NLM_BODY_STAGED : NLM_BODY_GLOBAL;
    g_nlm_last[1] = tight;
    g_nlm_last[2] = deep;
    g_nlm_last[3] = a.radius;
    g_nlm_last[4] = a.npatch;
    g_nlm_last[5] = a.reach;
    g_nlm_last[6] = n_border;
    g_nlm_last[7] = nchunks;
  }
  {
    launch_scope ls(devid, "nlm_chunks");
    const unsigned grid = (unsigned)nchunks;
    if(tall)
      k4t<<<grid, NL3_THREADS, tall_bytes, s>>>(in, out, a, dev_patches, dev_order, n_border, ndx3, seeds);
    else if(v4)
      k4<<<grid, NL3_THREADS, v4_bytes, s>>>(in, out, a, dev_patches, dev_order, n_border, ndx3, nullptr);
    else if(v3 && v3_bytes <= 160 * 1024)
      k3<<<grid, NL3_THREADS, v3_bytes, s>>>(in, out, a, dev_patches, dev_order, n_border, ndx3);
    else if(v2)
      k2<<<grid, NL2_THREADS, v2_bytes, s>>>(in, out, a, dev_patches, dev_order, n_border);
    else if(pipelined)
      nlm_chunks_pipelined<<<grid, NLM_THREADS, lds_bytes, s>>>(in, out, a, dev_patches);
    else if(staged)
      nlm_chunks<true><<<grid, NLM_THREADS, lds_bytes, s>>>(in, out, a, dev_patches);
    else
      nlm_chunks<false><<<grid, NLM_THREADS, lds_bytes, s>>>(in, out, a, dev_patches);
  }
  int err = check_launch("nlm_chunks");
  if(err == DT_HIP_SUCCESS && tall)
  {
    launch_scope ls(devid, "nlm_tail");
    if(n_border > 0) kt_ring<<<(unsigned)n_border, NLT_THREADS, tail_bytes, s>>>(in, out, a, dev_patches, dev_order, 0, seeds);
    if(nchunks > n_border)
      kt_in<<<(unsigned)(nchunks - n_border), NLT_THREADS, tail_bytes, s>>>(in, out, a, dev_patches, dev_order, n_border, seeds);
    err = check_launch("nlm_tail");
  }
  return err;
}

}

extern "C" {

int dt_hip_test_nlm_last(int out[8])
{
  if(!out) return DT_HIP_INVALID_ARG;
  memcpy(out, ansel::g_nlm_last, sizeof(ansel::g_nlm_last));
  return DT_HIP_SUCCESS;
}

int dt_hip_iop_nlmeans_process(int devid, const dt_hip_piece_t *piece, const dt_hip_nlmeans_data_t *d,
                               dt_hip_mem_t dev_in, dt_hip_mem_t dev_out)
{
  return nlmeans_process_band(devid, piece, d, nullptr, dev_in, dev_out);
}

void dt_hip_iop_nlmeans_tiling(const dt_hip_piece_t *piece, const dt_hip_nlmeans_data_t *d, dt_hip_tiling_t *tiling)
{
  const float scale = (float)fmin(piece->roi_in.scale, 2.0f);
  memset(tiling, 0, sizeof(*tiling));
  tiling->factor = 2.0f + 1.0f + 0.25f * 4;
  tiling->factor_cl = 2.0f + (slice_height(piece->roi_in.height) > NLT_HEAD_ROWS ? 0.96f : 0.0f);
  tiling->maxbuf = tiling->maxbuf_cl = 1.0f;
  tiling->overlap = (unsigned)((int)ceilf(d->radius * scale) + (int)ceilf(7 * scale));
  tiling->xalign = tiling->yalign = 1;
}

}

namespace ansel
{

static nlm_core_params_t nlmeans_params(const dt_hip_piece_t *piece, const dt_hip_nlmeans_data_t *d);

int nlmeans_core_halo_rows(const int frame_h, const nlm_core_params_t &p)
{
  const int K = p.search_radius;
  int max_shift = 0;
  for(int ri = -K; ri <= K; ri++)
    for(int ci = -K; ci <= K; ci++)
      max_shift = std::max(max_shift, std::max(abs(scatter(p.scale, p.scattering, ri, ci)), abs(scatter(p.scale, p.scattering, ci, ri))));
  return p.patch_radius + 1 + max_shift + slice_height(frame_h) - 1;
}

int nlmeans_halo_rows(const dt_hip_piece_t *piece, const dt_hip_nlmeans_data_t *d)
{
  return nlmeans_core_halo_rows(piece->roi_out.height, nlmeans_params(piece, d));
}

int nlmeans_process_band(int devid, const dt_hip_piece_t *piece, const dt_hip_nlmeans_data_t *d, const band_view_t *band,
                         dt_hip_mem_t dev_in, dt_hip_mem_t dev_out)
{
  if(!valid_device(devid) || !piece || !d || !dev_in || !dev_out) return DT_HIP_INVALID_ARG;
  if(piece->channels != 4) return DT_HIP_INVALID_ARG;
  nlm_core_params_t p = nlmeans_params(piece, d);
  p.band = band;
  return nlmeans_core_launch(devid, (const float4 *)dev_in, (float4 *)dev_out, piece->roi_out.width,
                             piece->roi_out.height, p);
}

int nlmeans_process_cells(int devid, const dt_hip_piece_t *piece, const dt_hip_nlmeans_data_t *d, dt_hip_mem_t dev_in, dt_hip_mem_t dev_out,
                          dt_hip_mem_t cells, float sigma_r, int size_z)
{
  if(!valid_device(devid) || !piece || !d || !dev_in || !dev_out || !cells) return DT_HIP_INVALID_ARG;
  if(piece->channels != 4) return DT_HIP_INVALID_ARG;
  nlm_core_params_t p = nlmeans_params(piece, d);
  p.cell_out = (float2 *)cells;
  p.cell_sigma_r = sigma_r;
  p.cell_size_z = size_z;
  return nlmeans_core_launch(devid, (const float4 *)dev_in, (float4 *)dev_out, piece->roi_out.width, piece->roi_out.height, p);
}

static nlm_core_params_t nlmeans_params(const dt_hip_piece_t *piece, const dt_hip_nlmeans_data_t *d)
{
  const float scale = (float)fmin(piece->roi_in.scale, 2.0f);
  const float max_L = 120.0f, max_C = 512.0f;
  const float nL = 1.0f / max_L, nC = 1.0f / max_C;
  nlm_core_params_t p;
  memset(&p, 0, sizeof(p));
  p.scattering = 0;
  p.scale = scale;
  p.luma = d->luma;
  p.chroma = d->chroma;
  p.center_weight = -1;
  p.sharpness = 3000.0f / (1.0f + d->strength);
  p.patch_radius = (int)ceilf(d->radius * scale);
  p.search_radius = (int)ceilf(7 * scale);
  p.norm[0] = nL * nL;
  p.norm[1] = nC * nC;
  p.norm[2] = nC * nC;
  p.norm[3] = 1.0f;
  return p;
}

}
```

### ansel_amd/csrc/runtime.cpp

```cpp
#include "hip_common.h"

#include <algorithm>
#include <atomic>
#include <mutex>
#include <unordered_map>
#include <map>
#include <vector>
#include <string>
#include <stdarg.h>

namespace
{

struct event_rec
{
  const char *tag;
  hipEvent_t start, stop;
};

struct device_t
{
  int hip_id = -1;
  std::string name;
  hipStream_t stream = nullptr;
  bool own_stream = false;
  std::mutex lock;
  bool events_enabled = false;
  std::mutex ev_lock;
  std::vector<event_rec> events;
  std::vector<hipEvent_t> event_pool;
  size_t cur_bytes = 0, peak_bytes = 0;
  std::multimap<size_t, void *> free_pool;
  std::atomic<uint64_t> test_fill{ 0 };
  struct staging_t
  {
    void *host = nullptr;
    size_t cap = 0;
    hipEvent_t ev = nullptr;
    bool used = false;
  };
  std::mutex staging_lock;
  staging_t staging[8];
  int staging_next = 0;
};

struct alloc_t
{
  size_t size;
  int devid;
  int width, height, bpp;
  void *host;
};

std::mutex g_mutex;
bool g_inited = false;
std::vector<device_t *> g_devs;
std::unordered_map<void *, alloc_t> g_allocs;
thread_local char t_error[512] = "";

}

namespace ansel
{

void set_last_error(const char *fmt, ...)
{
  va_list ap;
  va_start(ap, fmt);
  vsnprintf(t_error, sizeof(t_error), fmt, ap);
  va_end(ap);
}

bool valid_device(int devid) { return g_inited && devid >= 0 && devid < (int)g_devs.size(); }

bool make_current(int devid)
{
  if(!valid_device(devid)) return false;
  const int want = g_devs[devid]->hip_id;
  int cur = -1;
  if(hipGetDevice(&cur) == hipSuccess && cur == want) return true;
  return hipSetDevice(want) == hipSuccess;
}

int hip_device_of(int devid) { return valid_device(devid) ? g_devs[devid]->hip_id : -1; }

int upload_small(int devid, void *dst_dev, const void *src_host, size_t bytes)
{
  if(!valid_device(devid) || !dst_dev || (!src_host && bytes)) return DT_HIP_INVALID_ARG;
  if(bytes == 0) return DT_HIP_SUCCESS;
  device_t *d = g_devs[devid];
  if(!make_current(devid)) return DT_HIP_DEFAULT_ERROR;
  std::lock_guard<std::mutex> g(d->staging_lock);
  device_t::staging_t &st = d->staging[d->staging_next];
  d->staging_next = (d->staging_next + 1) % 8;
  if(st.used && hipEventSynchronize(st.ev) != hipSuccess) return DT_HIP_DEFAULT_ERROR;
  if(st.cap < bytes)
  {
    if(st.host) (void)hipHostFree(st.host);
    st.host = nullptr;
    st.cap = 0;
    size_t cap = 4096;
    while(cap < bytes) cap *= 2;
    if(hipHostMalloc(&st.host, cap, hipHostMallocDefault) != hipSuccess)
    {
      set_last_error("upload_small: no pinned staging buffer of %zu bytes", cap);
      st.host = nullptr;
      return DT_HIP_SYSMEM_ALLOCATION;
    }
    st.cap = cap;
  }
  if(!st.ev && hipEventCreateWithFlags(&st.ev, hipEventDisableTiming) != hipSuccess) return DT_HIP_DEFAULT_ERROR;
  memcpy(st.host, src_host, bytes);
  if(hipMemcpyAsync(dst_dev, st.host, bytes, hipMemcpyHostToDevice, d->stream) != hipSuccess || hipEventRecord(st.ev, d->stream) != hipSuccess)
  {
    set_last_error("upload_small: the copy of %zu bytes could not be enqueued", bytes);
    return DT_HIP_DEFAULT_ERROR;
  }
  st.used = true;
  return DT_HIP_SUCCESS;
}

hipStream_t stream_of(int devid)
{
  if(!make_current(devid)) return nullptr;
  return g_devs[devid]->stream;
}

launch_scope::launch_scope(int devid_, const char *tag_) : devid(devid_), tag(tag_), active(false)
{
  if(!valid_device(devid)) return;
  device_t *d = g_devs[devid];
  if(!d->events_enabled) return;
  make_current(devid);
  std::lock_guard<std::mutex> g(d->ev_lock);
  auto get = [&]() {
    hipEvent_t e;
    if(!d->event_pool.empty())
    {
      e = d->event_pool.back();
      d->event_pool.pop_back();
    }
    else if(hipEventCreate(&e) != hipSuccess)
      e = nullptr;
    return e;
  };
  start = get();
  stop = get();
  if(!start || !stop || hipEventRecord(start, d->stream) != hipSuccess)
  {
    (void)hipGetLastError();
    if(start) d->event_pool.push_back(start);
    if(stop) d->event_pool.push_back(stop);
    return;
  }
  active = true;
}

launch_scope::~launch_scope()
{
  if(!active) return;
  device_t *d = g_devs[devid];
  std::lock_guard<std::mutex> g(d->ev_lock);
  if(hipEventRecord(stop, d->stream) != hipSuccess)
  {
    (void)hipGetLastError();
    d->event_pool.push_back(start);
    d->event_pool.push_back(stop);
    return;
  }
  d->events.push_back({ tag, start, stop });
}

}

using namespace ansel;

extern "C" {

const char *dt_hip_last_error(void) { return t_error; }

int dt_hip_init(void)
{
  std::lock_guard<std::mutex> g(g_mutex);
  if(g_inited) return DT_HIP_SUCCESS;
  int n = 0;
  if(hipGetDeviceCount(&n) != hipSuccess || n <= 0)
  {
    set_last_error("dt_hip_init: no HIP device visible");
    return DT_HIP_DEFAULT_ERROR;
  }
  for(int i = 0; i < n; i++)
  {
    hipDeviceProp_t prop;
    if(hipGetDeviceProperties(&prop, i) != hipSuccess) continue;
    device_t *d = new device_t;
    d->hip_id = i;
    d->name = prop.name[0] ? prop.name : prop.gcnArchName;
    if(hipSetDevice(i) != hipSuccess || hipStreamCreateWithFlags(&d->stream, hipStreamNonBlocking) != hipSuccess)
    {
      delete d;
      continue;
    }
    d->own_stream = true;
    g_devs.push_back(d);
  }
  if(g_devs.empty())
  {
    set_last_error("dt_hip_init: no usable HIP device");
    return DT_HIP_DEFAULT_ERROR;
  }
  (void)hipSetDevice(g_devs[0]->hip_id);
  g_inited = true;
  return DT_HIP_SUCCESS;
}

void dt_hip_cleanup(void)
{
  std::lock_guard<std::mutex> g(g_mutex);
  if(!g_inited) return;
  for(device_t *d : g_devs)
  {
    (void)hipSetDevice(d->hip_id);
    (void)hipStreamSynchronize(d->stream);
    for(auto &kv : d->free_pool) (void)hipFree(kv.second);
    for(auto &e : d->events)
    {
      (void)hipEventDestroy(e.start);
      (void)hipEventDestroy(e.stop);
    }
    for(auto e : d->event_pool) (void)hipEventDestroy(e);
    for(auto &st : d->staging)
    {
      if(st.ev) (void)hipEventDestroy(st.ev);
      if(st.host) (void)hipHostFree(st.host);
    }
    if(d->own_stream) (void)hipStreamDestroy(d->stream);
    delete d;
  }
  for(auto &kv : g_allocs)
    if(!kv.second.host) (void)hipFree(kv.first);
  g_allocs.clear();
  g_devs.clear();
  g_inited = false;
}

int dt_hip_is_inited(void) { return g_inited ? 1 : 0; }

int dt_hip_get_num_devices(void) { return g_inited ? (int)g_devs.size() : 0; }

const char *dt_hip_get_device_name(int devid) { return valid_device(devid) ? g_devs[devid]->name.c_str() : ""; }

size_t dt_hip_get_device_available(int devid)
{
  if(!valid_device(devid)) return 0;
  size_t fr = 0, tot = 0;
  make_current(devid);
  if(hipMemGetInfo(&fr, &tot) != hipSuccess) return 0;
  std::lock_guard<std::mutex> g(g_mutex);
  for(auto &kv : g_devs[devid]->free_pool) fr += kv.first;
  return fr;
}

size_t dt_hip_get_device_memalloc(int devid)
{
  return dt_hip_get_device_available(devid);
}

int dt_hip_reserve_device_for_pipe(int pipetype)
{
  (void)pipetype;
  if(!g_inited) return -1;
  for(size_t i = 0; i < g_devs.size(); i++)
    if(g_devs[i]->lock.try_lock()) return (int)i;
  return -1;
}

void dt_hip_reserve_device_by_id(int devid)
{
  if(valid_device(devid)) g_devs[devid]->lock.lock();
}

int dt_hip_try_reserve_device_by_id(int devid)
{
  if(!valid_device(devid)) return 1;
  return g_devs[devid]->lock.try_lock() ? 0 : 1;
}

void dt_hip_release_device(int devid)
{
  if(valid_device(devid)) g_devs[devid]->lock.unlock();
}

int dt_hip_get_device_max_image_size(int devid, int *width, int *height)
{
  if(!valid_device(devid)) return 0;
  if(width) *width = 1 << 20;
  if(height) *height = 1 << 20;
  return 1;
}

size_t dt_hip_get_device_max_global_mem(int devid)
{
  if(!valid_device(devid)) return 0;
  size_t free_b = 0, total_b = 0;
  make_current(devid);
  if(hipMemGetInfo(&free_b, &total_b) != hipSuccess) return 0;
  return total_b;
}

static int g_error_count = 0;
static bool g_stopped = false;
int dt_hip_report_pipe_error(void)
{
  if(!g_inited) return 2;
  std::lock_guard<std::mutex> g(g_mutex);
  g_error_count++;
  if(g_error_count < 5) return 1;
  g_stopped = true;
  return 2;
}

int dt_hip_is_enabled(void) { return (g_inited && !g_stopped) ? 1 : 0; }
int dt_hip_update_settings(void) { return dt_hip_is_enabled(); }

void dt_hip_check_tuning(int devid) { (void)devid; }
int dt_hip_avoid_atomics(int devid) { (void)devid; return 0; }
int dt_hip_micro_nap(int devid) { (void)devid; return 0; }
int dt_hip_use_pinned_memory(int devid) { return valid_device(devid) ? 1 : 0; }
int dt_hip_dev_roundup_width(int size, int devid) { (void)devid; return size; }
int dt_hip_dev_roundup_height(int size, int devid) { (void)devid; return size; }

int dt_hip_image_fits_device(int devid, size_t width, size_t height, unsigned bpp, float factor, size_t overhead)
{
  if(!valid_device(devid)) return 0;
  const double need = (double)width * (double)height * (double)bpp * (double)factor + (double)overhead;
  return need <= (double)dt_hip_get_device_available(devid) ? 1 : 0;
}

int dt_hip_image_fits_device_reason(int devid, size_t width, size_t height, unsigned bpp, float factor, size_t overhead,
                                    size_t *needed, size_t *limit)
{
  if(!valid_device(devid)) return 2;
  const double single = (double)width * (double)height * (double)bpp;
  const double total = single * (double)factor + (double)overhead;
  const size_t avail = dt_hip_get_device_available(devid), memalloc = dt_hip_get_device_memalloc(devid);
  if(single > (double)memalloc)
  {
    if(needed) *needed = (size_t)single;
    if(limit) *limit = memalloc;
    return 1;
  }
  if(needed) *needed = (size_t)total;
  if(limit) *limit = avail;
  return total <= (double)avail ? 0 : 2;
}

void *dt_hip_get_stream(int devid) { return (void *)stream_of(devid); }

int dt_hip_set_stream(int devid, void *stream)
{
  if(!valid_device(devid)) return DT_HIP_INVALID_ARG;
  device_t *d = g_devs[devid];
  make_current(devid);
  if((hipStream_t)stream == d->stream) return DT_HIP_SUCCESS;
  if(d->stream || d->own_stream) (void)hipStreamSynchronize(d->stream);
  if(d->own_stream && d->stream) (void)hipStreamDestroy(d->stream);
  d->stream = (hipStream_t)stream;
  d->own_stream = false;
  return DT_HIP_SUCCESS;
}

dt_hip_mem_t dt_hip_alloc_device_buffer(int devid, size_t size)
{
  if(!valid_device(devid) || size == 0) return nullptr;
  device_t *d = g_devs[devid];
  const size_t rounded = (size + 255) & ~(size_t)255;
  std::unique_lock<std::mutex> g(g_mutex);
  void *p = nullptr;
  auto it = d->free_pool.find(rounded);
  if(it != d->free_pool.end())
  {
    p = it->second;
    d->free_pool.erase(it);
  }
  else
  {
    make_current(devid);
    hipError_t e = hipMalloc(&p, rounded);
    if(e != hipSuccess)
    {
      for(auto &kv : d->free_pool) (void)hipFree(kv.second);
      d->free_pool.clear();
      (void)hipGetLastError();
      e = hipMalloc(&p, rounded);
    }
    if(e != hipSuccess)
    {
      set_last_error("dt_hip_alloc_device_buffer: %zu bytes: %s", rounded, hipGetErrorString(e));
      (void)hipGetLastError();
      return nullptr;
    }
  }
  g_allocs[p] = { rounded, devid, 0, 0, 0, nullptr };
  d->cur_bytes += rounded;
  if(d->cur_bytes > d->peak_bytes) d->peak_bytes = d->cur_bytes;
  g.unlock();
  const uint64_t fill = d->test_fill.load(std::memory_order_relaxed);
  if(fill >> 32)
  {
    make_current(devid);
    if(hipMemsetD32Async((hipDeviceptr_t)p, (int)(uint32_t)fill, rounded / 4, d->stream) != hipSuccess
       || hipStreamSynchronize(d->stream) != hipSuccess)
    {
      set_last_error("dt_hip_alloc_device_buffer: the test fill of %zu bytes failed", rounded);
      (void)hipGetLastError();
      dt_hip_release_mem_object(p);
      return nullptr;
    }
  }
  return p;
}

int dt_hip_test_pool_fill(int devid, int enable, uint32_t pattern)
{
  if(!valid_device(devid)) return -1;
  const uint64_t next = enable ? (((uint64_t)1 << 32) | pattern) : 0;
  return (int)(g_devs[devid]->test_fill.exchange(next, std::memory_order_relaxed) >> 32);
}

dt_hip_mem_t dt_hip_alloc_device(int devid, int width, int height, int bpp)
{
  if(width <= 0 || height <= 0 || bpp <= 0) return nullptr;
  dt_hip_mem_t p = dt_hip_alloc_device_buffer(devid, (size_t)width * (size_t)height * (size_t)bpp);
  if(p)
  {
    std::lock_guard<std::mutex> g(g_mutex);
    alloc_t &a = g_allocs[p];
    a.width = width;
    a.height = height;
    a.bpp = bpp;
  }
  return p;
}

void dt_hip_release_mem_object(dt_hip_mem_t mem)
{
  if(!mem) return;
  std::lock_guard<std::mutex> g(g_mutex);
  auto it = g_allocs.find(mem);
  if(it == g_allocs.end()) return;
  const alloc_t a = it->second;
  g_allocs.erase(it);
  if(a.host) return;
  if(a.devid >= 0 && a.devid < (int)g_devs.size())
  {
    device_t *d = g_devs[a.devid];
    d->cur_bytes -= a.size;
    d->free_pool.insert({ a.size, mem });
  }
  else
    (void)hipFree(mem);
}

size_t dt_hip_get_mem_object_size(dt_hip_mem_t mem)
{
  std::lock_guard<std::mutex> g(g_mutex);
  auto it = g_allocs.find(mem);
  return it == g_allocs.end() ? 0 : it->second.size;
}

static alloc_t alloc_of(dt_hip_mem_t mem)
{
  std::lock_guard<std::mutex> g(g_mutex);
  auto it = g_allocs.find(mem);
  return it == g_allocs.end() ? alloc_t{ 0, -1, 0, 0, 0, nullptr } : it->second;
}
int dt_hip_get_image_width(dt_hip_mem_t mem) { return alloc_of(mem).width; }
int dt_hip_get_image_height(dt_hip_mem_t mem) { return alloc_of(mem).height; }
int dt_hip_get_image_element_size(dt_hip_mem_t mem) { return alloc_of(mem).bpp; }
int dt_hip_get_mem_context_id(dt_hip_mem_t mem) { return alloc_of(mem).devid; }

dt_hip_mem_t dt_hip_alloc_device_use_host_pointer(int devid, int width, int height, int bpp, void *host, int flags)
{
  (void)flags;
  if(!valid_device(devid) || !host || width <= 0 || height <= 0 || bpp <= 0 || !dt_hip_is_pinned_memory(host)) return nullptr;
  void *dev = nullptr;
  make_current(devid);
  if(hipHostGetDevicePointer(&dev, host, 0) != hipSuccess || !dev)
  {
    (void)hipGetLastError();
    return nullptr;
  }
  std::lock_guard<std::mutex> g(g_mutex);
  g_allocs[dev] = { (size_t)width * height * bpp, devid, width, height, bpp, host };
  return dev;
}

void *dt_hip_map_buffer(int devid, dt_hip_mem_t buffer, int blocking, int flags, size_t offset, size_t size)
{
  (void)flags;
  (void)size;
  const alloc_t a = alloc_of(buffer);
  if(!a.host || !valid_device(devid)) return nullptr;
  if(blocking && hipStreamSynchronize(stream_of(devid)) != hipSuccess) return nullptr;
  return (char *)a.host + offset;
}
void *dt_hip_map_image(int devid, dt_hip_mem_t buffer, int blocking, int flags, size_t width, size_t height, int bpp)
{
  (void)width;
  (void)height;
  (void)bpp;
  return dt_hip_map_buffer(devid, buffer, blocking, flags, 0, 0);
}
int dt_hip_unmap_mem_object(int devid, dt_hip_mem_t mem, void *mapped_ptr)
{
  (void)mapped_ptr;
  return (valid_device(devid) && alloc_of(mem).host) ? DT_HIP_SUCCESS : DT_HIP_INVALID_ARG;
}

dt_hip_mem_t dt_hip_copy_host_to_device_rowpitch(int devid, void *host, int width, int height, int bpp, int rowpitch)
{
  dt_hip_mem_t d = dt_hip_alloc_device(devid, width, height, bpp);
  if(!d) return nullptr;
  if(dt_hip_write_host_to_device_rowpitch(devid, host, d, width, height, bpp, (size_t)rowpitch, 1) != DT_HIP_SUCCESS)
  {
    dt_hip_release_mem_object(d);
    return nullptr;
  }
  return d;
}
dt_hip_mem_t dt_hip_copy_host_to_device(int devid, void *host, int width, int height, int bpp)
{
  return dt_hip_copy_host_to_device_rowpitch(devid, host, width, height, bpp, 0);
}
dt_hip_mem_t dt_hip_copy_host_to_device_constant(int devid, size_t size, void *host)
{
  dt_hip_mem_t d = dt_hip_alloc_device_buffer(devid, size);
  if(!d) return nullptr;
  if(dt_hip_write_buffer_to_device(devid, host, d, 0, size, 1) != DT_HIP_SUCCESS)
  {
    dt_hip_release_mem_object(d);
    return nullptr;
  }
  return d;
}
int dt_hip_copy_device_to_host(int devid, void *host, dt_hip_mem_t device, int width, int height, int bpp)
{
  return dt_hip_read_host_from_device(devid, host, device, width, height, bpp);
}

int dt_hip_read_buffer_from_device(int devid, void *host, dt_hip_mem_t device, size_t offset, size_t size, int blocking)
{
  if(!valid_device(devid) || !host || !device) return DT_HIP_INVALID_ARG;
  if(!size) return DT_HIP_SUCCESS;
  hipStream_t s = stream_of(devid);
  ANSEL_HIP_CHECK(hipMemcpyAsync(host, (const char *)device + offset, size, hipMemcpyDeviceToHost, s));
  if(blocking) ANSEL_HIP_CHECK(hipStreamSynchronize(s));
  return DT_HIP_SUCCESS;
}
int dt_hip_write_buffer_to_device(int devid, const void *host, dt_hip_mem_t device, size_t offset, size_t size, int blocking)
{
  if(!valid_device(devid) || !host || !device) return DT_HIP_INVALID_ARG;
  if(!size) return DT_HIP_SUCCESS;
  hipStream_t s = stream_of(devid);
  ANSEL_HIP_CHECK(hipMemcpyAsync((char *)device + offset, host, size, hipMemcpyHostToDevice, s));
  if(blocking || dt_hip_is_pinned_memory(host)) ANSEL_HIP_CHECK(hipStreamSynchronize(s));
  return DT_HIP_SUCCESS;
}

int dt_hip_enqueue_barrier(int devid) { return valid_device(devid) ? DT_HIP_SUCCESS : DT_HIP_INVALID_ARG; }

void dt_hip_memory_statistics(int devid, size_t *current, size_t *peak)
{
  if(current) *current = valid_device(devid) ? g_devs[devid]->cur_bytes : 0;
  if(peak) *peak = valid_device(devid) ? g_devs[devid]->peak_bytes : 0;
}

int dt_hip_write_host_to_device_rowpitch(int devid, const void *host, dt_hip_mem_t device, int width, int height,
                                         int bpp, size_t rowpitch, int blocking)
{
  if(!valid_device(devid) || !host || !device) return DT_HIP_INVALID_ARG;
  hipStream_t s = stream_of(devid);
  const size_t wbytes = (size_t)width * bpp;
  launch_scope ls(devid, "[Write Image (from host to device)]");
  if(rowpitch == wbytes || rowpitch == 0)
    ANSEL_HIP_CHECK(hipMemcpyAsync(device, host, wbytes * height, hipMemcpyHostToDevice, s));
  else
    ANSEL_HIP_CHECK(hipMemcpy2DAsync(device, wbytes, host, rowpitch, wbytes, height, hipMemcpyHostToDevice, s));
  if(blocking) ANSEL_HIP_CHECK(hipStreamSynchronize(s));
  return DT_HIP_SUCCESS;
}

int dt_hip_write_host_to_device(int devid, const void *host, dt_hip_mem_t device, int width, int height, int bpp)
{
  return dt_hip_write_host_to_device_rowpitch(devid, host, device, width, height, bpp, (size_t)width * bpp, 1);
}

int dt_hip_read_host_from_device_rowpitch(int devid, void *host, dt_hip_mem_t device, int width, int height,
                                          int bpp, size_t rowpitch, int blocking)
{
  if(!valid_device(devid) || !host || !device) return DT_HIP_INVALID_ARG;
  hipStream_t s = stream_of(devid);
  const size_t wbytes = (size_t)width * bpp;
  launch_scope ls(devid, "[Read Image (from device to host)]");
  if(rowpitch == wbytes || rowpitch == 0)
    ANSEL_HIP_CHECK(hipMemcpyAsync(host, device, wbytes * height, hipMemcpyDeviceToHost, s));
  else
    ANSEL_HIP_CHECK(hipMemcpy2DAsync(host, rowpitch, device, wbytes, wbytes, height, hipMemcpyDeviceToHost, s));
  if(blocking) ANSEL_HIP_CHECK(hipStreamSynchronize(s));
  return DT_HIP_SUCCESS;
}

int dt_hip_read_host_from_device(int devid, void *host, dt_hip_mem_t device, int width, int height, int bpp)
{
  return dt_hip_read_host_from_device_rowpitch(devid, host, device, width, height, bpp, (size_t)width * bpp, 1);
}

static int raw_window(int devid, dt_hip_mem_t device, const size_t *origin, const size_t *region, size_t &wbytes, size_t &dpitch,
                      size_t &doffs)
{
  if(!valid_device(devid) || !device || !origin || !region) return DT_HIP_INVALID_ARG;
  const alloc_t a = alloc_of(device);
  if(a.width <= 0 || a.bpp <= 0)
  {
    set_last_error("window copy: the device object is not a 2-D image of this runtime (dt_hip_alloc_device)");
    return DT_HIP_INVALID_ARG;
  }
  if(origin[0] + region[0] > (size_t)a.width || origin[1] + region[1] > (size_t)a.height) return DT_HIP_INVALID_ARG;
  wbytes = region[0] * a.bpp;
  dpitch = (size_t)a.width * a.bpp;
  doffs = origin[1] * dpitch + origin[0] * a.bpp;
  return DT_HIP_SUCCESS;
}

int dt_hip_read_host_from_device_raw(int devid, void *host, dt_hip_mem_t device, const size_t *origin, const size_t *region,
                                     int rowpitch, int blocking)
{
  size_t wbytes, dpitch, doffs;
  const int rc = raw_window(devid, device, origin, region, wbytes, dpitch, doffs);
  if(rc != DT_HIP_SUCCESS || !host) return rc != DT_HIP_SUCCESS ? rc : DT_HIP_INVALID_ARG;
  if(!wbytes || !region[1]) return DT_HIP_SUCCESS;
  hipStream_t s = stream_of(devid);
  launch_scope ls(devid, "[Read Image (from device to host)]");
  ANSEL_HIP_CHECK(hipMemcpy2DAsync(host, rowpitch ? (size_t)rowpitch : wbytes, (const char *)device + doffs, dpitch, wbytes,
                                   region[1], hipMemcpyDeviceToHost, s));
  if(blocking) ANSEL_HIP_CHECK(hipStreamSynchronize(s));
  return DT_HIP_SUCCESS;
}

int dt_hip_write_host_to_device_raw(int devid, const void *host, dt_hip_mem_t device, const size_t *origin, const size_t *region,
                                    int rowpitch, int blocking)
{
  size_t wbytes, dpitch, doffs;
  const int rc = raw_window(devid, device, origin, region, wbytes, dpitch, doffs);
  if(rc != DT_HIP_SUCCESS || !host) return rc != DT_HIP_SUCCESS ? rc : DT_HIP_INVALID_ARG;
  if(!wbytes || !region[1]) return DT_HIP_SUCCESS;
  hipStream_t s = stream_of(devid);
  launch_scope ls(devid, "[Write Image (from host to device)]");
  ANSEL_HIP_CHECK(hipMemcpy2DAsync((char *)device + doffs, dpitch, host, rowpitch ? (size_t)rowpitch : wbytes, wbytes, region[1],
                                   hipMemcpyHostToDevice, s));
  if(blocking || dt_hip_is_pinned_memory(host)) ANSEL_HIP_CHECK(hipStreamSynchronize(s));
  return DT_HIP_SUCCESS;
}

int dt_hip_enqueue_copy_image(int devid, dt_hip_mem_t src, dt_hip_mem_t dst, const size_t *orig_src, const size_t *orig_dst,
                              const size_t *region)
{
  if(!valid_device(devid) || !src || !dst || !orig_src || !orig_dst || !region) return DT_HIP_INVALID_ARG;
  const alloc_t a = alloc_of(src), b = alloc_of(dst);
  if(a.width <= 0 || b.width <= 0 || a.bpp != b.bpp) return DT_HIP_INVALID_ARG;
  const size_t lim = 0x7fffffff;
  if(region[0] > lim || region[1] > lim || orig_src[0] > lim || orig_src[1] > lim || orig_dst[0] > lim || orig_dst[1] > lim
     || orig_src[0] + region[0] > (size_t)a.width || orig_dst[0] + region[0] > (size_t)b.width
     || (a.height > 0 && orig_src[1] + region[1] > (size_t)a.height) || (b.height > 0 && orig_dst[1] + region[1] > (size_t)b.height))
  {
    set_last_error("enqueue_copy_image: the window leaves the image");
    return DT_HIP_INVALID_ARG;
  }
  return dt_hip_enqueue_copy_region(devid, src, a.width, (int)orig_src[0], (int)orig_src[1], dst, b.width, (int)orig_dst[0],
                                    (int)orig_dst[1], (int)region[0], (int)region[1], a.bpp);
}

void *dt_hip_alloc_host_pinned(size_t size)
{
  void *p = NULL;
  if(size == 0 || hipHostMalloc(&p, size, hipHostMallocDefault) != hipSuccess)
  {
    (void)hipGetLastError();
    return NULL;
  }
  return p;
}

void dt_hip_free_host_pinned(void *host)
{
  if(host) (void)hipHostFree(host);
}

int dt_hip_is_pinned_memory(const void *host)
{
  hipPointerAttribute_t attr;
  if(!host || hipPointerGetAttributes(&attr, host) != hipSuccess)
  {
    (void)hipGetLastError();
    return 0;
  }
  return attr.type == hipMemoryTypeHost;
}

int dt_hip_iop_basebuffer_process(int devid, const dt_hip_piece_t *piece, int iwidth, int iheight, int bpp,
                                  const void *host_full, dt_hip_mem_t dev_out)
{
  if(!valid_device(devid) || !piece || !host_full || !dev_out || iwidth <= 0 || iheight <= 0 || bpp <= 0)
    return DT_HIP_INVALID_ARG;
  const size_t x = piece->roi_out.x > 0 ? (size_t)piece->roi_out.x : 0, y = piece->roi_out.y > 0 ? (size_t)piece->roi_out.y : 0;
  if(piece->roi_out.width <= 0 || piece->roi_out.height <= 0 || x >= (size_t)iwidth || y >= (size_t)iheight)
    return DT_HIP_SUCCESS;
  const size_t in_width = std::min((size_t)piece->roi_out.width, (size_t)iwidth - x);
  const size_t in_height = std::min((size_t)piece->roi_out.height, (size_t)iheight - y);
  const size_t in_stride = (size_t)iwidth * bpp, out_stride = (size_t)piece->roi_out.width * bpp;
  const size_t row_bytes = std::min(in_width * bpp, out_stride);
  const char *src = (const char *)host_full + y * in_stride + x * bpp;
  hipStream_t s = stream_of(devid);
  launch_scope ls(devid, "[Write Image (from host to device)]");
  ANSEL_HIP_CHECK(hipMemcpy2DAsync(dev_out, out_stride, src, in_stride, row_bytes, in_height, hipMemcpyHostToDevice, s));
  ANSEL_HIP_CHECK(hipStreamSynchronize(s));
  return DT_HIP_SUCCESS;
}

int dt_hip_enqueue_copy_buffer_to_buffer(int devid, dt_hip_mem_t src, dt_hip_mem_t dst, size_t srcoffset,
                                         size_t dstoffset, size_t size)
{
  if(!valid_device(devid) || !src || !dst) return DT_HIP_INVALID_ARG;
  launch_scope ls(devid, "[Copy Buffer to Buffer (on device)]");
  ANSEL_HIP_CHECK(hipMemcpyAsync((char *)dst + dstoffset, (const char *)src + srcoffset, size,
                                 hipMemcpyDeviceToDevice, stream_of(devid)));
  return DT_HIP_SUCCESS;
}

int dt_hip_enqueue_copy_region(int devid, dt_hip_mem_t src, int src_width, int src_x, int src_y, dt_hip_mem_t dst,
                               int dst_width, int dst_x, int dst_y, int width, int height, int bpp)
{
  if(!valid_device(devid) || !src || !dst) return DT_HIP_INVALID_ARG;
  if(width <= 0 || height <= 0) return DT_HIP_SUCCESS;
  launch_scope ls(devid, "[Copy Image (on device)]");
  const char *s = (const char *)src + ((size_t)src_y * src_width + src_x) * bpp;
  char *d = (char *)dst + ((size_t)dst_y * dst_width + dst_x) * bpp;
  ANSEL_HIP_CHECK(hipMemcpy2DAsync(d, (size_t)dst_width * bpp, s, (size_t)src_width * bpp, (size_t)width * bpp,
                                   height, hipMemcpyDeviceToDevice, stream_of(devid)));
  return DT_HIP_SUCCESS;
}

int dt_hip_finish(int devid)
{
  if(!valid_device(devid)) return 0;
  const hipError_t e = hipStreamSynchronize(stream_of(devid));
  if(e != hipSuccess)
  {
    set_last_error("dt_hip_finish: %s", hipGetErrorString(e));
    return 0;
  }
  return 1;
}

void dt_hip_events_enable(int devid, int enable)
{
  if(valid_device(devid)) g_devs[devid]->events_enabled = enable != 0;
}

void dt_hip_events_reset(int devid)
{
  if(!valid_device(devid)) return;
  device_t *d = g_devs[devid];
  (void)hipStreamSynchronize(d->stream);
  for(auto &e : d->events)
  {
    d->event_pool.push_back(e.start);
    d->event_pool.push_back(e.stop);
  }
  d->events.clear();
}

void dt_hip_events_wait_for(int devid)
{
  if(valid_device(devid)) (void)hipStreamSynchronize(g_devs[devid]->stream);
}

int dt_hip_events_flush(int devid, int reset)
{
  if(!valid_device(devid)) return DT_HIP_INVALID_ARG;
  const hipError_t e = hipStreamSynchronize(g_devs[devid]->stream);
  if(reset) dt_hip_events_reset(devid);
  if(e != hipSuccess)
  {
    set_last_error("dt_hip_events_flush: %s", hipGetErrorString(e));
    return DT_HIP_DEFAULT_ERROR;
  }
  return DT_HIP_SUCCESS;
}

int dt_hip_events_profiling(int devid, const char **tags, float *ms, int *counts, int max)
{
  if(!valid_device(devid)) return 0;
  device_t *d = g_devs[devid];
  (void)hipStreamSynchronize(d->stream);
  std::vector<const char *> order;
  std::unordered_map<std::string, int> idx;
  std::vector<float> tsum;
  std::vector<int> cnt;
  for(auto &e : d->events)
  {
    float t = 0.f;
    if(hipEventElapsedTime(&t, e.start, e.stop) != hipSuccess) continue;
    auto it = idx.find(e.tag);
    int k;
    if(it == idx.end())
    {
      k = (int)order.size();
      idx[e.tag] = k;
      order.push_back(e.tag);
      tsum.push_back(0.f);
      cnt.push_back(0);
    }
    else
      k = it->second;
    tsum[k] += t;
    cnt[k] += 1;
  }
  const int n = (int)order.size();
  for(int i = 0; i < n && i < max; i++)
  {
    if(tags) tags[i] = order[i];
    if(ms) ms[i] = tsum[i];
    if(counts) counts[i] = cnt[i];
  }
  return n;
}

size_t dt_hip_abi_sizeof(const char *name)
{
#define S(n, t) \
  if(!strcmp(name, n)) return sizeof(t)
  S("roi", dt_hip_roi_t);
  S("piece", dt_hip_piece_t);
  S("tiling", dt_hip_tiling_t);
  S("rawprepare", dt_hip_rawprepare_data_t);
  S("temperature", dt_hip_temperature_data_t);
  S("highlights", dt_hip_highlights_data_t);
  S("demosaic", dt_hip_demosaic_data_t);
  S("exposure", dt_hip_exposure_data_t);
  S("conversion", dt_hip_conversion_t);
  S("channelmixerrgb", dt_hip_channelmixerrgb_data_t);
  S("filmic_spline", dt_hip_filmic_spline_t);
  S("filmicrgb", dt_hip_filmicrgb_data_t);
  S("diffuse", dt_hip_diffuse_data_t);
  S("denoiseprofile", dt_hip_denoiseprofile_data_t);
  S("nlmeans", dt_hip_nlmeans_data_t);
  S("lab", dt_hip_lab_data_t);
  S("bilat", dt_hip_bilat_data_t);
  S("finalscale", dt_hip_finalscale_data_t);
  S("blend", dt_hip_blend_data_t);
  S("detailmask", dt_hip_detailmask_data_t);
  S("flip", dt_hip_flip_data_t);
  S("tile_plan_roi", dt_hip_tile_plan_roi_t);
  S("export_rows", dt_hip_export_rows_t);
  S("jpeg", dt_hip_jpeg_data_t);
  S("png", dt_hip_png_data_t);
  S("tiff", dt_hip_tiff_data_t);
  S("webp", dt_hip_webp_data_t);
  S("tile_plan", dt_hip_tile_plan_t);
  S("band", dt_hip_band_t);
  S("band_state", dt_hip_band_state_t);
  S("band_stats", dt_hip_band_stats_t);
#undef S
  return 0;
}

}
```

### ansel_amd/csrc/testhooks.hip

```cpp
#include "hip_common.h"
#include "devmath.h"
#include "ieee_inrange.h"

#include <atomic>
#include <string.h>

using namespace ansel;

namespace
{
std::atomic<int> g_dispatch[DISPATCH_KEYS];
const char *const g_dispatch_names[DISPATCH_KEYS] = { "nlm_v2", "nlm_fused", "amaze_unfused", "amaze_slab", "amaze_blocks",
                                                       "bilat_blur_split", "strip_rows" };
}
namespace ansel
{
int dispatch_override(const dispatch_key_t key) { return g_dispatch[key].load(std::memory_order_relaxed); }
}
extern "C" int dt_hip_test_dispatch(const char *key, int value)
{
  if(!key) return DT_HIP_INVALID_ARG;
  for(int k = 0; k < DISPATCH_KEYS; k++)
    if(!strcmp(key, g_dispatch_names[k]))
    {
      if(k == DISPATCH_STRIP_ROWS && value != 0 && value != 4 && value != 8 && value != 16 && value != 32) return DT_HIP_INVALID_ARG;
      g_dispatch[k].store(value);
      return DT_HIP_SUCCESS;
    }
  return DT_HIP_INVALID_ARG;
}

extern "C" int dt_hip_test_strip_rows(int gx, int classes, int per_class) { return strip_rows(gx, classes, per_class); }

namespace
{
template <int FN>
__global__ void devmath_test(const float *__restrict__ x, const float *__restrict__ y, float *__restrict__ o, const size_t n)
{
  for(size_t k = (size_t)blockIdx.x * blockDim.x + threadIdx.x; k < n; k += (size_t)gridDim.x * blockDim.x)
  {
    float r;
    if(FN == 0) r = ansel_math::powf_exact(x[k], y[k]);
    else if(FN == 1) r = ansel_math::log2f_exact(x[k]);
    else if(FN == 2) r = ansel_math::exp2f_exact(x[k]);
    else if(FN == 3) r = ansel_math::expf_exact(x[k]);
    else if(FN == 4) r = ansel_math::atan2f_exact(x[k], y[k]);
    else if(FN == 5) r = ansel_math::hypotf_exact(x[k], y[k]);
    else if(FN == 6) r = ansel_math::sinf_exact(x[k]);
    else if(FN == 7) r = ansel_math::cosf_exact(x[k]);
    else if(FN == 9) r = ansel_math::logf_exact(x[k]);
    else if(FN == 10) r = ansel_ieee::div_core(x[k], y[k]);
    else if(FN == 11) r = ansel_ieee::rcp_core(x[k]);
    else if(FN == 12) r = ansel_ieee::sqrt_core(x[k]);
    else if(FN == 13) r = ansel_ieee::zero_or_above_2m96(x[k]) ? 1.0f : 0.0f;
    else if(FN == 14) r = ansel_ieee::div_uniform(x[k], y[k], ansel_ieee::rcp_refined(y[k]));
    else r = fmodf(x[k], y[k]);
    o[k] = r;
  }
}
template <int FN> int devmath_launch(int devid, const void *x, const void *y, void *o, size_t n)
{
  if(!valid_device(devid)) return DT_HIP_INVALID_ARG;
  devmath_test<FN><<<stream_grid(n, 256), 256, 0, stream_of(devid)>>>((const float *)x, (const float *)y, (float *)o, n);
  return check_launch("devmath_test");
}
}
extern "C" {
int dt_hip_test_powf(int devid, const void *x, const void *y, void *o, size_t n) { return devmath_launch<0>(devid, x, y, o, n); }
int dt_hip_test_log2f(int devid, const void *x, const void *y, void *o, size_t n) { return devmath_launch<1>(devid, x, y, o, n); }
int dt_hip_test_exp2f(int devid, const void *x, const void *y, void *o, size_t n) { return devmath_launch<2>(devid, x, y, o, n); }
int dt_hip_test_expf(int devid, const void *x, const void *y, void *o, size_t n) { return devmath_launch<3>(devid, x, y, o, n); }
int dt_hip_test_atan2f(int devid, const void *x, const void *y, void *o, size_t n) { return devmath_launch<4>(devid, x, y, o, n); }
int dt_hip_test_hypotf(int devid, const void *x, const void *y, void *o, size_t n) { return devmath_launch<5>(devid, x, y, o, n); }
int dt_hip_test_sinf(int devid, const void *x, const void *y, void *o, size_t n) { return devmath_launch<6>(devid, x, y, o, n); }
int dt_hip_test_cosf(int devid, const void *x, const void *y, void *o, size_t n) { return devmath_launch<7>(devid, x, y, o, n); }
int dt_hip_test_fmodf(int devid, const void *x, const void *y, void *o, size_t n) { return devmath_launch<8>(devid, x, y, o, n); }
int dt_hip_test_logf(int devid, const void *x, const void *y, void *o, size_t n) { return devmath_launch<9>(devid, x, y, o, n); }
int dt_hip_test_div_core(int devid, const void *x, const void *y, void *o, size_t n) { return devmath_launch<10>(devid, x, y, o, n); }
int dt_hip_test_rcp_core(int devid, const void *x, const void *y, void *o, size_t n) { return devmath_launch<11>(devid, x, y, o, n); }
int dt_hip_test_sqrt_core(int devid, const void *x, const void *y, void *o, size_t n) { return devmath_launch<12>(devid, x, y, o, n); }
int dt_hip_test_zero_or_above_2m96(int devid, const void *x, const void *y, void *o, size_t n) { return devmath_launch<13>(devid, x, y, o, n); }
int dt_hip_test_div_uniform(int devid, const void *x, const void *y, void *o, size_t n) { return devmath_launch<14>(devid, x, y, o, n); }
}

namespace
{
__global__ __launch_bounds__(64) void lds_dma_x3_test(const float *__restrict__ src, unsigned *__restrict__ dst, const unsigned base)
{
  __shared__ unsigned lds[512];
  for(int i = threadIdx.x; i < 512; i += 64) lds[i] = 0xdeadbeefu;
  __syncthreads();
  using lds_u32_ptr = __attribute__((address_space(3))) unsigned *;
  const unsigned m0v = (unsigned)__builtin_amdgcn_readfirstlane((int)(unsigned)(__UINTPTR_TYPE__)(lds_u32_ptr)lds) + base;
  const unsigned voff = (63u - threadIdx.x) * 12u;
  unsigned keep;
  asm volatile("s_waitcnt lgkmcnt(0)\n\ts_nop 4\n\ts_mov_b32 %0, m0\n\t"
               "s_mov_b32 m0, %3\n\ts_nop 0\n\tglobal_load_lds_dwordx3 %1, %2\n\t"
               "s_mov_b32 m0, %0\n\ts_waitcnt vmcnt(0)"
               : "=&s"(keep)
               : "v"(voff), "s"(src), "s"(m0v)
               : "memory");
  __syncthreads();
  for(int i = threadIdx.x; i < 512; i += 64) dst[i] = lds[i];
}
}
extern "C" int dt_hip_test_lds_dma_x3(int devid, const void *src, void *dst, unsigned base)
{
  if(!valid_device(devid) || !src || !dst || base % 4 != 0 || base + 1024 > 2048) return DT_HIP_INVALID_ARG;
  lds_dma_x3_test<<<1, 64, 0, stream_of(devid)>>>((const float *)src, (unsigned *)dst, base);
  return check_launch("lds_dma_x3_test");
}
```

### ansel_amd/lib.py

```python
import ctypes as C
import os

from . import abi

HERE = os.path.dirname(os.path.abspath(__file__))
LIB_PATH = os.environ.get("ANSEL_HIP_LIB") or os.path.join(HERE, "libansel_hip.so")

_lib = None
_env_fill = False
_env_fill_applied = False


class AnselHipError(RuntimeError):
    pass


def load():
    global _lib
    if _lib is not None:
        return _lib
    if not os.path.exists(LIB_PATH):
        if os.environ.get("ANSEL_HIP_LIB"):
            raise AnselHipError(
                "ANSEL_HIP_LIB=%s does not exist: the measuring build is made by `python -m ansel_amd.build --measuring` "
                "(tools/ default to it; unset the variable for the product library)" % LIB_PATH)
        raise AnselHipError(
            "%s not found: build it with `python -m ansel_amd.build` (hipcc, gfx950). "
            "There is no CPU fallback." % LIB_PATH)
    if os.environ.get("ANSEL_HIP_NO_TORCH") != "1":
        try:
            import torch
        except Exception:
            pass
    lib = C.CDLL(LIB_PATH)
    vp, i, u, sz = C.c_void_p, C.c_int, C.c_uint32, C.c_size_t
    P = C.POINTER
    protos = {
        "dt_hip_init": (i, []),
        "dt_hip_cleanup": (None, []),
        "dt_hip_is_inited": (i, []),
        "dt_hip_get_num_devices": (i, []),
        "dt_hip_get_device_name": (C.c_char_p, [i]),
        "dt_hip_get_device_available": (sz, [i]),
        "dt_hip_get_device_memalloc": (sz, [i]),
        "dt_hip_reserve_device_for_pipe": (i, [i]),
        "dt_hip_reserve_device_by_id": (None, [i]),
        "dt_hip_try_reserve_device_by_id": (i, [i]),
        "dt_hip_release_device": (None, [i]),
        "dt_hip_get_device_max_image_size": (i, [i, P(i), P(i)]),
        "dt_hip_get_device_max_global_mem": (sz, [i]),
        "dt_hip_report_pipe_error": (i, []),
        "dt_hip_is_enabled": (i, []),
        "dt_hip_update_settings": (i, []),
        "dt_hip_check_tuning": (None, [i]),
        "dt_hip_avoid_atomics": (i, [i]),
        "dt_hip_micro_nap": (i, [i]),
        "dt_hip_use_pinned_memory": (i, [i]),
        "dt_hip_dev_roundup_width": (i, [i, i]),
        "dt_hip_dev_roundup_height": (i, [i, i]),
        "dt_hip_image_fits_device_reason": (i, [i, sz, sz, C.c_uint, C.c_float, sz, P(sz), P(sz)]),
        "dt_hip_get_image_width": (i, [vp]),
        "dt_hip_get_image_height": (i, [vp]),
        "dt_hip_get_image_element_size": (i, [vp]),
        "dt_hip_get_mem_context_id": (i, [vp]),
        "dt_hip_alloc_device_use_host_pointer": (vp, [i, i, i, i, vp, i]),
        "dt_hip_map_buffer": (vp, [i, vp, i, i, sz, sz]),
        "dt_hip_map_image": (vp, [i, vp, i, i, sz, sz, i]),
        "dt_hip_unmap_mem_object": (i, [i, vp, vp]),
        "dt_hip_copy_host_to_device": (vp, [i, vp, i, i, i]),
        "dt_hip_copy_host_to_device_rowpitch": (vp, [i, vp, i, i, i, i]),
        "dt_hip_copy_host_to_device_constant": (vp, [i, sz, vp]),
        "dt_hip_copy_device_to_host": (i, [i, vp, vp, i, i, i]),
        "dt_hip_read_buffer_from_device": (i, [i, vp, vp, sz, sz, i]),
        "dt_hip_write_buffer_to_device": (i, [i, vp, vp, sz, sz, i]),
        "dt_hip_enqueue_barrier": (i, [i]),
        "dt_hip_events_wait_for": (None, [i]),
        "dt_hip_events_flush": (i, [i, i]),
        "dt_hip_image_fits_device": (i, [i, sz, sz, C.c_uint, C.c_float, sz]),
        "dt_hip_get_stream": (vp, [i]),
        "dt_hip_set_stream": (i, [i, vp]),
        "dt_hip_alloc_device": (vp, [i, i, i, i]),
        "dt_hip_alloc_device_buffer": (vp, [i, sz]),
        "dt_hip_release_mem_object": (None, [vp]),
        "dt_hip_get_mem_object_size": (sz, [vp]),
        "dt_hip_memory_statistics": (None, [i, P(sz), P(sz)]),
        "dt_hip_write_host_to_device": (i, [i, vp, vp, i, i, i]),
        "dt_hip_write_host_to_device_rowpitch": (i, [i, vp, vp, i, i, i, sz, i]),
        "dt_hip_read_host_from_device": (i, [i, vp, vp, i, i, i]),
        "dt_hip_read_host_from_device_rowpitch": (i, [i, vp, vp, i, i, i, sz, i]),
        "dt_hip_enqueue_copy_buffer_to_buffer": (i, [i, vp, vp, sz, sz, sz]),
        "dt_hip_read_host_from_device_raw": (i, [i, vp, vp, P(sz), P(sz), i, i]),
        "dt_hip_write_host_to_device_raw": (i, [i, vp, vp, P(sz), P(sz), i, i]),
        "dt_hip_enqueue_copy_image": (i, [i, vp, vp, P(sz), P(sz), P(sz)]),
        "dt_hip_enqueue_copy_region": (i, [i, vp, i, i, i, vp, i, i, i, i, i, i]),
        "dt_hip_finish": (i, [i]),
        "dt_hip_events_enable": (None, [i, i]),
        "dt_hip_events_reset": (None, [i]),
        "dt_hip_events_profiling": (i, [i, P(C.c_char_p), P(C.c_float), P(i), i]),
        "dt_hip_last_error": (C.c_char_p, []),
        "dt_hip_abi_sizeof": (sz, [C.c_char_p]),
        "dt_hip_crop_dcraw_filters": (u, [u, u, u]),
        "dt_hip_iop_rawprepare_process": (i, [i, P(abi.Piece), P(abi.RawprepareData), vp, vp]),
        "dt_hip_iop_temperature_process": (i, [i, P(abi.Piece), P(abi.TemperatureData), vp, vp]),
        "dt_hip_iop_highlights_process": (i, [i, P(abi.Piece), P(abi.HighlightsData), vp, vp]),
        "dt_hip_iop_demosaic_process": (i, [i, P(abi.Piece), P(abi.DemosaicData), vp, vp]),
        "dt_hip_iop_demosaic_tiling": (None, [P(abi.Piece), P(abi.DemosaicData), P(abi.Tiling)]),
        "dt_hip_iop_exposure_process": (i, [i, P(abi.Piece), P(abi.ExposureData), vp, vp]),
        "dt_hip_iop_colorin_process": (i, [i, P(abi.Piece), P(abi.Conversion), vp, vp]),
        "dt_hip_iop_colorout_process": (i, [i, P(abi.Piece), P(abi.Conversion), vp, vp]),
        "dt_hip_iop_channelmixerrgb_process": (i, [i, P(abi.Piece), P(abi.ChannelmixerrgbData), vp, vp]),
        "dt_hip_iop_filmicrgb_process": (i, [i, P(abi.Piece), P(abi.FilmicrgbData), vp, vp]),
        "dt_hip_iop_diffuse_process": (i, [i, P(abi.Piece), P(abi.DiffuseData), vp, vp]),
        "dt_hip_iop_denoiseprofile_process": (i, [i, P(abi.Piece), P(abi.DenoiseprofileData), vp, vp]),
        "dt_hip_iop_nlmeans_process": (i, [i, P(abi.Piece), P(abi.NlmeansData), vp, vp]),
        "dt_hip_iop_detailmask_process": (i, [i, P(abi.Piece), P(abi.DetailmaskData), vp, vp]),
        "dt_hip_transform_rgb_to_lab": (i, [i, P(abi.Piece), P(abi.LabData), vp, vp]),
        "dt_hip_transform_lab_to_rgb": (i, [i, P(abi.Piece), P(abi.LabData), vp, vp]),
        "dt_hip_iop_bilat_process": (i, [i, P(abi.Piece), P(abi.BilatData), vp, vp]),
        "dt_hip_iop_finalscale_process": (i, [i, P(abi.Piece), P(abi.FinalscaleData), vp, vp]),
        "dt_hip_iop_initialscale_process": (i, [i, P(abi.Piece), P(abi.FinalscaleData), vp, vp]),
        "dt_hip_iop_flip_process": (i, [i, P(abi.Piece), P(abi.FlipData), vp, vp]),
        "dt_hip_iop_flip_modify_roi_out": (i, [P(abi.FlipData), i, i, P(abi.Roi), P(abi.Roi)]),
        "dt_hip_iop_flip_modify_roi_in": (i, [P(abi.FlipData), i, i, P(abi.Roi), P(abi.Roi)]),
        "dt_hip_iop_flip_distort_transform": (i, [P(abi.FlipData), i, i, P(C.c_float), sz]),
        "dt_hip_iop_flip_distort_backtransform": (i, [P(abi.FlipData), i, i, P(C.c_float), sz]),
        "dt_hip_raw_unpack": (i, [i, vp, i, i, C.c_size_t, i, i, vp]),
        "dt_hip_develop_blend_process": (i, [i, P(abi.Piece), P(abi.BlendData), vp, vp]),
        "dt_hip_iop_basebuffer_process": (i, [i, P(abi.Piece), i, i, i, vp, vp]),
        "dt_hip_alloc_host_pinned": (vp, [sz]),
        "dt_hip_free_host_pinned": (None, [vp]),
        "dt_hip_is_pinned_memory": (i, [vp]),
        "dt_hip_plan_tiles_ptp": (i, [i, i, i, i, P(abi.Tiling), C.c_uint, sz, sz, i, i, P(abi.TilePlan)]),
        "dt_hip_default_process_tiling_ptp": (i, [i, C.c_char_p, P(abi.Piece), vp, sz, P(abi.Tiling), vp, vp, i, i, sz]),
        "dt_hip_default_tiling": (None, [P(abi.Piece), i, P(abi.Tiling)]),
        "dt_hip_plan_tiles_roi": (i, [P(abi.Roi), P(abi.Roi), i, i, P(abi.Tiling), C.c_uint, sz, sz, i, i, P(abi.TilePlanRoi)]),
        "dt_hip_tile_rois_finalscale": (i, [P(abi.TilePlanRoi), P(abi.Roi), P(abi.Roi), i, i, P(abi.Roi), P(abi.Roi), P(abi.Roi)]),
        "dt_hip_tile_rois_flip": (i, [P(abi.TilePlanRoi), P(abi.Roi), P(abi.Roi), P(abi.FlipData), i, i, P(abi.Roi), P(abi.Roi),
                                      P(abi.Roi)]),
        "dt_hip_default_process_tiling_roi": (i, [i, C.c_char_p, P(abi.Piece), vp, sz, P(abi.Tiling), vp, vp, i, i, sz]),
        "dt_hip_iop_denoiseprofile_tiling": (None, [P(abi.Piece), P(abi.DenoiseprofileData), P(abi.Tiling)]),
        "dt_hip_iop_nlmeans_tiling": (None, [P(abi.Piece), P(abi.NlmeansData), P(abi.Tiling)]),
        "dt_hip_iop_bilat_tiling": (None, [P(abi.Piece), P(abi.BilatData), P(abi.Tiling)]),
        "dt_hip_iop_diffuse_tiling": (None, [P(abi.Piece), P(abi.DiffuseData), P(abi.Tiling)]),
        "dt_hip_export_convert_u16": (i, [i, i, i, vp, vp]),
        "dt_hip_export_convert_u8": (i, [i, i, i, vp, vp]),
        "dt_hip_export_pack_rows": (i, [i, i, i, i, i, vp, vp]),
        "dt_hip_jpeg_bound": (sz, [i, i, P(abi.JpegData)]),
        "dt_hip_export_jpeg": (i, [i, i, i, P(abi.JpegData), vp, vp]),
        "dt_hip_png_bound": (sz, [i, i, P(abi.PngData)]),
        "dt_hip_export_png": (i, [i, i, i, P(abi.PngData), vp, vp]),
        "dt_hip_tiff_bound": (sz, [i, i, P(abi.TiffData)]),
        "dt_hip_export_tiff": (i, [i, i, i, P(abi.TiffData), vp, vp]),
        "dt_hip_webp_bound": (sz, [i, i, P(abi.WebpData)]),
        "dt_hip_export_webp": (i, [i, i, i, P(abi.WebpData), vp, vp]),
        "dt_hip_pipe_new": (vp, [i]),
        "dt_hip_pipe_free": (None, [vp]),
        "dt_hip_pipe_add_node": (i, [vp, C.c_char_p, P(abi.Piece), vp, sz]),
        "dt_hip_pipe_set_fusion": (None, [vp, i]),
        "dt_hip_pipe_num_groups": (i, [vp]),
        "dt_hip_pipe_process": (i, [vp, vp, vp]),
        "dt_hip_batch_new": (vp, [vp, i, sz, sz]),
        "dt_hip_batch_free": (None, [vp]),
        "dt_hip_batch_submit": (i, [vp, vp, vp]),
        "dt_hip_batch_wait": (i, [vp, i]),
        "dt_hip_batch_drain": (i, [vp]),
        "dt_hip_batch_set_writer": (i, [vp, vp, vp]),
        "dt_hip_plan_bands": (i, [i, i, i, i, P(abi.Band)]),
        "dt_hip_band_halo_rows": (i, [C.c_char_p, P(abi.Piece), vp, sz]),
        "dt_hip_pipe_band_begin": (i, [vp, P(abi.Band), vp, P(abi.BandState)]),
        "dt_hip_pipe_band_resolve": (i, [vp, P(abi.Band), P(abi.BandState)]),
        "dt_hip_pipe_band_finish": (i, [vp, P(abi.Band), P(abi.BandState), vp]),
        "dt_hip_pipe_band_relay": (i, [vp, P(abi.Band), P(abi.BandState)]),
        "dt_hip_pipe_band_abort": (None, [vp, P(abi.BandState)]),
        "dt_hip_pipe_process_bands": (i, [P(vp), i, P(abi.Band), P(vp), P(vp)]),
        "dt_hip_pipe_bands_stats": (None, [P(abi.BandStats)]),
        "dt_hip_peer_selftest": (i, [P(i), i]),
        "dt_hip_iop_highlights_process_deferred": (i, [i, P(abi.Piece), P(abi.HighlightsData), vp, vp, vp]),
        "dt_hip_iop_highlights_resolve": (i, [i, vp, vp]),
        "dt_hip_test_dispatch": (i, [C.c_char_p, i]),
        "dt_hip_test_strip_rows": (i, [i, i, i]),
        "dt_hip_test_nlm_last": (i, [P(i)]),
        "dt_hip_test_pool_fill": (i, [i, i, u]),
    }
    missing = []
    for name, (res, args) in protos.items():
        try:
            fn = getattr(lib, name)
        except AttributeError:
            missing.append(name)
            continue
        fn.restype = res
        fn.argtypes = args
    lib._ansel_missing = missing
    lib._ansel_protos = protos
    _lib = lib
    return lib


def test_dispatch(key, value):
    check(load().dt_hip_test_dispatch(key.encode(), int(value)), "dt_hip_test_dispatch(%s)" % key)


def test_strip_rows(gx, classes, per_class):
    return load().dt_hip_test_strip_rows(int(gx), int(classes), int(per_class))


def test_pool_fill(devid, enable, pattern=0):
    was = load().dt_hip_test_pool_fill(devid, 1 if enable else 0, int(pattern) & 0xFFFFFFFF)
    if was < 0:
        raise AnselHipError("dt_hip_test_pool_fill: no device %d" % devid)
    return bool(was)


NLM_BODIES = ("none", "tall", "v4", "v3", "v2", "pipelined", "staged", "global")


def test_nlm_last():
    out = (C.c_int * 8)()
    check(load().dt_hip_test_nlm_last(out), "dt_hip_test_nlm_last")
    keys = ("body", "tight", "deep", "radius", "npatch", "reach", "n_border", "nchunks")
    d = dict(zip(keys, list(out)))
    d["body"] = NLM_BODIES[d["body"]]
    return d


def check(rc, what=""):
    if rc != abi.DT_HIP_SUCCESS:
        msg = load().dt_hip_last_error()
        raise AnselHipError("%s failed with %d: %s" % (what, rc, msg.decode() if msg else ""))


def init():
    lib = load()
    if lib._ansel_missing:
        raise AnselHipError("libansel_hip.so lacks symbols declared in include/ansel_hip.h: %s"
                            % ", ".join(lib._ansel_missing))
    check(lib.dt_hip_init(), "dt_hip_init")
    global _env_fill_applied
    if not _env_fill_applied:
        _env_fill_applied = True
        if env_pool_fill() is not None:
            test_pool_fill(0, True, env_pool_fill())
    return lib


def env_pool_fill():
    global _env_fill
    if _env_fill is False:
        env = os.environ.get("ANSEL_TEST_POOL_FILL")
        _env_fill = (int(env, 16) & 0xFFFFFFFF) if env else None
    return _env_fill


class DeviceBuffer:

    def __init__(self, devid, nbytes):
        self.lib = load()
        self.devid = devid
        self.nbytes = int(nbytes)
        self.ptr = self.lib.dt_hip_alloc_device_buffer(devid, self.nbytes)
        if not self.ptr:
            raise AnselHipError("device allocation of %d bytes failed: %s"
                                % (self.nbytes, self.lib.dt_hip_last_error().decode()))

    @classmethod
    def from_numpy(cls, devid, arr):
        import numpy as np
        arr = np.ascontiguousarray(arr)
        b = cls(devid, arr.nbytes)
        check(b.lib.dt_hip_write_buffer_to_device(devid, arr.ctypes.data_as(C.c_void_p), b.ptr, 0, arr.nbytes, 1),
              "write_buffer_to_device")
        return b

    def upload(self, arr):
        import numpy as np
        arr = np.ascontiguousarray(arr)
        assert arr.nbytes <= self.nbytes
        check(self.lib.dt_hip_write_buffer_to_device(self.devid, arr.ctypes.data_as(C.c_void_p), self.ptr, 0, arr.nbytes, 1),
              "write_buffer_to_device")

    def to_numpy(self, shape, dtype):
        import numpy as np
        out = np.empty(shape, dtype=dtype)
        assert out.nbytes <= self.nbytes
        check(self.lib.dt_hip_read_buffer_from_device(self.devid, out.ctypes.data_as(C.c_void_p), self.ptr, 0,
                                                      out.nbytes, 1), "read_buffer_from_device")
        return out

    def release(self):
        if self.ptr:
            self.lib.dt_hip_release_mem_object(self.ptr)
            self.ptr = None

    def __del__(self):
        try:
            self.release()
        except Exception:
            pass
```

Before: 1614.

## Make NLM v3 interior blocks walk multiple chunks with window prefetch overlap

```diff
diff --git a/__graft_entry__.py b/__graft_entry__.py
--- a/__graft_entry__.py
+++ b/__graft_entry__.py
@@ -28,6 +28,8 @@
     sys.path.insert(0, os.path.join(ROOT, "tests"))
     import test_amaze_host
     test_amaze_host.build()
+    import test_nlm3_walk_host
+    test_nlm3_walk_host.build()
     if os.path.isdir("/root/reference/src"):
         sys.path.insert(0, os.path.join(ROOT, "tests"))
         import test_boundary_compile
diff --git a/ansel_amd/csrc/hip_common.h b/ansel_amd/csrc/hip_common.h
--- a/ansel_amd/csrc/hip_common.h
+++ b/ansel_amd/csrc/hip_common.h
@@ -25,6 +25,7 @@
   DISPATCH_AMAZE_BLOCKS,
   DISPATCH_BILAT_BLUR_SPLIT,
   DISPATCH_STRIP_ROWS,
+  DISPATCH_NLM_WALK,
   DISPATCH_KEYS
 };
 int dispatch_override(dispatch_key_t key);
@@ -44,6 +45,7 @@
 int upload_small(int devid, void *dst_dev, const void *src_host, size_t bytes);
 bool make_current(int devid);
 int hip_device_of(int devid);
+int device_cus(int devid);
 bool valid_device(int devid);
 
 struct launch_scope
diff --git a/ansel_amd/csrc/nlm3_body.h b/ansel_amd/csrc/nlm3_body.h
--- a/ansel_amd/csrc/nlm3_body.h
+++ b/ansel_amd/csrc/nlm3_body.h
@@ -119,23 +119,48 @@
 
 constexpr int TALL_HEAD = 64;
 constexpr int TALL_SEED_PITCH = 80;
-template <int NPXL, int MSEG, bool BORDER = false, bool FUSED = false, bool TALL = false, int P = 2, bool CENTER = false, class Env,
-          class Args, class F4, class I2>
-NLM2_FN void body(const Env &env, const F4 *__restrict__ in, F4 *__restrict__ out, const Args &a, const I2 *__restrict__ patches,
-                  const int ndx, float *__restrict__ seeds_out = nullptr)
+
+template <bool FUSED> constexpr int fill_stages() { return FUSED ? 2 : 3; }
+
+constexpr int WALK_ROWS = (NL3_A1_LANES + 192) / (2 * NL3_WPH);
+constexpr int WALK_PF = 13;
+inline constexpr bool walk_fits(const int chk_h, const int reach) { return chk_h + 2 * reach <= WALK_ROWS * WALK_PF; }
+template <int P, bool CENTER> constexpr bool walks() { return P == 2 && !CENTER; }
+
+template <class Args> NLM2_FN bool interior_chunk(const Args &a, const int chunk)
+{
+  const int cy_launch = chunk / a.nchx, cx = chunk - cy_launch * a.nchx;
+  const int top = (cy_launch + a.cy0) * a.chk_h, left = cx * a.chk_w;
+  return top >= a.reach && top + a.chk_h + a.reach <= a.H && left >= a.reach && left + a.chk_w + a.reach <= a.W;
+}
+
+template <int NPXL, int MSEG, bool BORDER, bool FUSED, bool TALL, int P, bool CENTER, bool WALK, class Env, class Args, class F4, class I2>
+NLM2_FN void life(const Env &env, const F4 *__restrict__ in, F4 *__restrict__ out, const Args &a, const I2 *__restrict__ patches,
+                  const int ndx, float *__restrict__ seeds_out, const int *__restrict__ order, const int pos0, const int stride,
+                  const int count)
 {
   static_assert(!TALL || FUSED, "the head of a tall chunk runs on the fused body");
+  static_assert(!WALK || (!BORDER && !FUSED && !TALL), "the walk is the interior chunks' on the four-table body");
   constexpr int S = 2 * P + 1, TP = NL3_TP, XO = NL3_XO, FP = NL3_FP, WPH = NL3_WPH;
   constexpr int NSEG = a1_segments<P>(), NCH = S * NSEG;
   constexpr int MAXCH = FUSED ? FUSED_MAXCH : max_rows<NPXL>();
   constexpr int NT = FUSED ? 3 : 4;
+  constexpr int FILL = fill_stages<FUSED>();
   auto tslot = [](const int p) { return FUSED ? p % 3 : (p & 3); };
   constexpr int LPR = (72 + NPXL - 1) / NPXL;
   const int tid = env.tid();
   const int W = a.W, H = a.H;
-  const int cy_launch = env.bid() / a.nchx, cx = env.bid() - cy_launch * a.nchx;
-  const int cy = cy_launch + a.cy0;
-  const int top = cy * a.chk_h, left = cx * a.chk_w;
+  const int m = WALK ? count : 1;
+  auto chunk_at = [&](const int k) { return WALK ? order[pos0 + k * stride] : env.bid(); };
+  int top, left, r0, c0;
+  auto place = [&](const int chunk) {
+    const int cy_launch = chunk / a.nchx, cx = chunk - cy_launch * a.nchx;
+    top = (cy_launch + a.cy0) * a.chk_h;
+    left = cx * a.chk_w;
+    r0 = top - a.reach;
+    c0 = left - a.reach;
+  };
+  place(chunk_at(0));
   const int bot = imin(top + a.chk_h, H), right = imin(left + a.chk_w, W);
   const int ch_grid = bot - top, cw = right - left;
   const int reach = a.reach;
@@ -151,47 +176,83 @@
   float *const Z = XY + 2 * (wh * 2 * WPH);
   float *const tab = Z + wh * 2 * WPH;
   float *const Fb = tab + NT * tabsz;
-  const int r0 = top - reach, c0 = left - reach;
   const float n0 = a.norm[0], n1 = a.norm[1], n2 = a.norm[2];
   const int ww = cw + 2 * reach;
-
-  for(int i0 = tid; i0 < wh * 2 * WPH; i0 += 4 * NL3_THREADS)
-  {
-    F4 v[4];
-#pragma unroll
-    for(int u = 0; u < 4; u++)
-    {
-      const int i = i0 + u * NL3_THREADS;
-      const int wy = i / (2 * WPH), rem = i - wy * (2 * WPH);
-      const int par = rem / WPH, h = rem - par * WPH;
-      const int wx = 2 * h + par;
-      const int r = r0 + wy, c = c0 + wx;
-      v[u].x = v[u].y = v[u].z = v[u].w = 0.0f;
-      if(i < wh * 2 * WPH && wx < ww && c < W && (!BORDER || (r >= 0 && r < H && c >= 0))) v[u] = in[(long)r * W + c];
-    }
-#pragma unroll
-    for(int u = 0; u < 4; u++)
-    {
-      const int i = i0 + u * NL3_THREADS;
-      if(i < wh * 2 * WPH)
-      {
-        f2 xy;
-        xy.x = v[u].x;
-        xy.y = v[u].y;
-        st2(XY + 2 * i, xy);
-        Z[i] = v[u].z;
-      }
-    }
-  }
-  env.sync();
-  auto widx = [&](const int wy, const int wx) { return (wy * 2 + (wx & 1)) * WPH + (wx >> 1); };
-
-  const int w = tid >> 6, lane = tid & 63;
+  const int w = tid >> 6;
+  const int lane = tid & 63;
 #if defined(__HIPCC__) && !defined(ANSEL_HIP_MEASURING)
   constexpr int var = 0;
 #else
   const int var = a.variant;
 #endif
+  auto stage_sync = [&]() {
+    if(!(var & 8192)) env.sync();
+  };
+  auto lead = [&](const int depth) {
+    for(int s = 0; s < depth; s++) stage_sync();
+  };
+  auto trail = [&](const int depth) {
+    for(int s = depth; s < FILL; s++) stage_sync();
+  };
+  auto window_at = [&](const int wy, const int rem) {
+    const int par = rem / WPH, h = rem - par * WPH;
+    const int wx = 2 * h + par;
+    const int r = r0 + wy, c = c0 + wx;
+    F4 v;
+    v.x = v.y = v.z = v.w = 0.0f;
+    if(wy < wh && wx < ww && c < W && (!BORDER || (r >= 0 && r < H && c >= 0))) v = in[(long)r * W + c];
+    return v;
+  };
+  auto window_px = [&](const int i) { return window_at(i / (2 * WPH), i % (2 * WPH)); };
+  auto window_st = [&](const int i, const F4 &v) {
+    if(i < wh * 2 * WPH)
+    {
+      f2 xy;
+      xy.x = v.x;
+      xy.y = v.y;
+      st2(XY + 2 * i, xy);
+      Z[i] = v.z;
+    }
+  };
+
+  for(int i0 = tid; i0 < wh * 2 * WPH; i0 += 4 * NL3_THREADS)
+  {
+    F4 v[4];
+#pragma unroll
+    for(int u = 0; u < 4; u++) v[u] = window_px(i0 + u * NL3_THREADS);
+#pragma unroll
+    for(int u = 0; u < 4; u++) window_st(i0 + u * NL3_THREADS, v[u]);
+  }
+  env.sync();
+  [[maybe_unused]] auto prefetch = [&](F4 *const pf, const int pl, const int zero) {
+    const int row = pl / (2 * WPH) + zero, rem = pl % (2 * WPH);
+#pragma unroll
+    for(int u = 0; u < WALK_PF; u++) pf[u] = window_at(row < WALK_ROWS ? row + u * WALK_ROWS : wh, rem);
+  };
+  [[maybe_unused]] auto commit = [&](const F4 *const pf, const int pl, const int zero) {
+    const int row = pl / (2 * WPH) + zero, rem = pl % (2 * WPH);
+#pragma unroll
+    for(int u = 0; u < WALK_PF; u++) window_st(row < WALK_ROWS ? (row + u * WALK_ROWS) * (2 * WPH) + rem : wh * 2 * WPH, pf[u]);
+  };
+  auto drain = [&](const int depth, [[maybe_unused]] const int pl, [[maybe_unused]] const int wk) {
+    if constexpr(WALK)
+    {
+      if(wk + 1 < m)
+      {
+        F4 pf[WALK_PF];
+        const int next = chunk_at(wk + 1);
+        place(next);
+        prefetch(pf, pl, next >> 31);
+        trail(depth);
+        commit(pf, pl, next >> 31);
+        env.sync();
+        return;
+      }
+    }
+    trail(depth);
+  };
+  auto widx = [&](const int wy, const int wx) { return (wy * 2 + (wx & 1)) * WPH + (wx >> 1); };
+
   const bool lay1 = !FUSED && !CENTER && (var & 4096);
   const int a1_index = FUSED ? ((w >= 2 && w <= 7) ? w - 2 : -1)
                        : CENTER ? (w == 7 ? 0 : (w == 11 ? 1 : (w >= 12 ? w - 10 : -1)))
@@ -234,151 +295,153 @@
     constexpr int DUMMY = 0;
     const int toff0 = (1 + k + j0 * S) * TP + XO + x0;
     const int foff = k * FP + XO + x0;
-    float ox[MSEG + 1][2], oy[MSEG + 1][2], oz[MSEG + 1][2];
-#pragma unroll
-    for(int i = 0; i <= MSEG; i++)
-#pragma unroll
-      for(int c = 0; c < 2; c++)
-      {
-        const int wx = wc0 + c;
-        const int wi = rowbase + i * RSTEP + (wx & 1) * WPH + (wx >> 1);
-        const f2 v = ld2(XY + 2 * wi);
-        ox[i][c] = v.x;
-        oy[i][c] = v.y;
-        oz[i][c] = Z[wi];
-      }
-    bool own_row[MSEG + 1], row_ok[MSEG + 1], own_col[2];
-#pragma unroll
-    for(int i = 0; i <= MSEG; i++)
-    {
-      const int R = r0 + wr0 + i * S;
-      own_row[i] = row_ok[i] = !BORDER || (R >= 0 && R < H);
-    }
-#pragma unroll
-    for(int c = 0; c < 2; c++) own_col[c] = !BORDER || (c0 + wc0 + c >= 0 && c0 + wc0 + c < W);
-    float sx[MSEG + 1][2], sy[MSEG + 1][2], sz[MSEG + 1][2];
-#pragma unroll
-    for(int i = 0; i <= MSEG; i++) sx[i][0] = sx[i][1] = sy[i][0] = sy[i][1] = sz[i][0] = sz[i][1] = 0.0f;
-
-    auto load_row_head = [&](const int dy, const int dx) {
-      const int dyo = rowbase + dy * 2 * WPH;
-#pragma unroll
-      for(int c = 0; c < 2; c++)
-      {
-        const int wx = wc0 + c + dx;
-        const int base = dyo + (wx & 1) * WPH + (wx >> 1);
+    const int pl = ai * 64 + lane;
+    for(int wk = 0; wk < m; wk++)
+    {
+      float ox[MSEG + 1][2], oy[MSEG + 1][2], oz[MSEG + 1][2];
+#pragma unroll
+      for(int i = 0; i <= MSEG; i++)
+#pragma unroll
+        for(int c = 0; c < 2; c++)
+        {
+          const int wx = wc0 + c;
+          const int wi = rowbase + i * RSTEP + (wx & 1) * WPH + (wx >> 1);
+          const f2 v = ld2(XY + 2 * wi);
+          ox[i][c] = v.x;
+          oy[i][c] = v.y;
+          oz[i][c] = Z[wi];
+        }
+      bool own_row[MSEG + 1], row_ok[MSEG + 1], own_col[2];
+#pragma unroll
+      for(int i = 0; i <= MSEG; i++)
+      {
+        const int R = r0 + wr0 + i * S;
+        own_row[i] = row_ok[i] = !BORDER || (R >= 0 && R < H);
+      }
+#pragma unroll
+      for(int c = 0; c < 2; c++) own_col[c] = !BORDER || (c0 + wc0 + c >= 0 && c0 + wc0 + c < W);
+      float sx[MSEG + 1][2], sy[MSEG + 1][2], sz[MSEG + 1][2];
+#pragma unroll
+      for(int i = 0; i <= MSEG; i++) sx[i][0] = sx[i][1] = sy[i][0] = sy[i][1] = sz[i][0] = sz[i][1] = 0.0f;
+
+      auto load_row_head = [&](const int dy, const int dx) {
+        const int dyo = rowbase + dy * 2 * WPH;
+#pragma unroll
+        for(int c = 0; c < 2; c++)
+        {
+          const int wx = wc0 + c + dx;
+          const int base = dyo + (wx & 1) * WPH + (wx >> 1);
+#pragma unroll
+          for(int i = 0; i <= MSEG; i++)
+          {
+            const int wi = base + i * RSTEP;
+            const f2 v = ld2(XY + 2 * wi);
+            sx[i][c] = v.x;
+            sy[i][c] = v.y;
+            sz[i][c] = Z[wi];
+          }
+        }
+      };
+      auto step = [&](auto ph_tag, const int p, const int dx) {
+        constexpr int PH = decltype(ph_tag)::value;
+        float *const T = tab + tslot(p) * tabsz;
+        float *const F = Fb + (p & 1) * S * FP;
+        const int fo = head ? foff : DUMMY;
+        bool col_ok[2] = { true, true };
+        if(BORDER)
+        {
+#pragma unroll
+          for(int c = 0; c < 2; c++) col_ok[c] = own_col[c] && (unsigned)(c0 + wc0 + c + dx) < (unsigned)W;
+        }
+        float px2[2], py2[2], pz2[2];
+#pragma unroll
+        for(int c = 0; c < 2; c++)
+        {
+          const int sl = (c + PH) & 1;
+          const float dx_ = ox[0][c] - sx[0][sl], dy_ = oy[0][c] - sy[0][sl], dz_ = oz[0][c] - sz[0][sl];
+          px2[c] = dx_ * dx_;
+          py2[c] = dy_ * dy_;
+          pz2[c] = dz_ * dz_;
+          if(BORDER && !(row_ok[0] && col_ok[c])) px2[c] = py2[c] = pz2[c] = 0.0f;
+        }
+        {
+          f2 d;
+          d.x = px2[0] * n0 + py2[0] * n1 + pz2[0] * n2;
+          d.y = px2[1] * n0 + py2[1] * n1 + pz2[1] * n2;
+          st2(F + fo, d);
+        }
+#pragma unroll
+        for(int i = 1; i <= MSEG; i++)
+        {
+          f2 t;
+          float nx2[2], ny2[2], nz2[2];
+#pragma unroll
+          for(int c = 0; c < 2; c++)
+          {
+            const int sl = (c + PH) & 1;
+            const float dx_ = ox[i][c] - sx[i][sl], dy_ = oy[i][c] - sy[i][sl], dz_ = oz[i][c] - sz[i][sl];
+            nx2[c] = dx_ * dx_;
+            ny2[c] = dy_ * dy_;
+            nz2[c] = dz_ * dz_;
+            if(BORDER && !(row_ok[i] && col_ok[c])) nx2[c] = ny2[c] = nz2[c] = 0.0f;
+          }
+          t.x = ((nx2[0] - px2[0]) * n0 + (ny2[0] - py2[0]) * n1) + (nz2[0] - pz2[0]) * n2;
+          t.y = ((nx2[1] - px2[1]) * n0 + (ny2[1] - py2[1]) * n1) + (nz2[1] - pz2[1]) * n2;
+          if(i - 1 < jn) st2(T + toff0 + (i - 1) * S * TP, t);
+          env.sched_fence();
+#pragma unroll
+          for(int c = 0; c < 2; c++)
+          {
+            px2[c] = nx2[c];
+            py2[c] = ny2[c];
+            pz2[c] = nz2[c];
+          }
+        }
+      };
+      auto slide = [&](auto ph_tag, const int dy, const int dx) {
+        constexpr int PH = decltype(ph_tag)::value;
+        const int wx = wc0 + 1 + dx + 1;
+        const int base = rowbase + dy * 2 * WPH + (wx & 1) * WPH + (wx >> 1);
 #pragma unroll
         for(int i = 0; i <= MSEG; i++)
         {
           const int wi = base + i * RSTEP;
           const f2 v = ld2(XY + 2 * wi);
-          sx[i][c] = v.x;
-          sy[i][c] = v.y;
-          sz[i][c] = Z[wi];
-        }
-      }
-    };
-    auto step = [&](auto ph_tag, const int p, const int dx) {
-      constexpr int PH = decltype(ph_tag)::value;
-      float *const T = tab + tslot(p) * tabsz;
-      float *const F = Fb + (p & 1) * S * FP;
-      const int fo = head ? foff : DUMMY;
-      bool col_ok[2] = { true, true };
-      if(BORDER)
-      {
-#pragma unroll
-        for(int c = 0; c < 2; c++) col_ok[c] = own_col[c] && (unsigned)(c0 + wc0 + c + dx) < (unsigned)W;
-      }
-      float px2[2], py2[2], pz2[2];
-#pragma unroll
-      for(int c = 0; c < 2; c++)
-      {
-        const int sl = (c + PH) & 1;
-        const float dx_ = ox[0][c] - sx[0][sl], dy_ = oy[0][c] - sy[0][sl], dz_ = oz[0][c] - sz[0][sl];
-        px2[c] = dx_ * dx_;
-        py2[c] = dy_ * dy_;
-        pz2[c] = dz_ * dz_;
-        if(BORDER && !(row_ok[0] && col_ok[c])) px2[c] = py2[c] = pz2[c] = 0.0f;
-      }
-      {
-        f2 d;
-        d.x = px2[0] * n0 + py2[0] * n1 + pz2[0] * n2;
-        d.y = px2[1] * n0 + py2[1] * n1 + pz2[1] * n2;
-        st2(F + fo, d);
-      }
-#pragma unroll
-      for(int i = 1; i <= MSEG; i++)
-      {
-        f2 t;
-        float nx2[2], ny2[2], nz2[2];
-#pragma unroll
-        for(int c = 0; c < 2; c++)
-        {
-          const int sl = (c + PH) & 1;
-          const float dx_ = ox[i][c] - sx[i][sl], dy_ = oy[i][c] - sy[i][sl], dz_ = oz[i][c] - sz[i][sl];
-          nx2[c] = dx_ * dx_;
-          ny2[c] = dy_ * dy_;
-          nz2[c] = dz_ * dz_;
-          if(BORDER && !(row_ok[i] && col_ok[c])) nx2[c] = ny2[c] = nz2[c] = 0.0f;
-        }
-        t.x = ((nx2[0] - px2[0]) * n0 + (ny2[0] - py2[0]) * n1) + (nz2[0] - pz2[0]) * n2;
-        t.y = ((nx2[1] - px2[1]) * n0 + (ny2[1] - py2[1]) * n1) + (nz2[1] - pz2[1]) * n2;
-        if(i - 1 < jn) st2(T + toff0 + (i - 1) * S * TP, t);
-        env.sched_fence();
-#pragma unroll
-        for(int c = 0; c < 2; c++)
-        {
-          px2[c] = nx2[c];
-          py2[c] = ny2[c];
-          pz2[c] = nz2[c];
-        }
-      }
-    };
-    auto slide = [&](auto ph_tag, const int dy, const int dx) {
-      constexpr int PH = decltype(ph_tag)::value;
-      const int wx = wc0 + 1 + dx + 1;
-      const int base = rowbase + dy * 2 * WPH + (wx & 1) * WPH + (wx >> 1);
-#pragma unroll
-      for(int i = 0; i <= MSEG; i++)
-      {
-        const int wi = base + i * RSTEP;
-        const f2 v = ld2(XY + 2 * wi);
-        sx[i][PH] = v.x;
-        sy[i][PH] = v.y;
-        sz[i][PH] = Z[wi];
-      }
-    };
-    for(int dyi = 0; dyi < ndy; dyi++)
-    {
-      const int dy = patches[dyi * ndx].x, dx0 = patches[dyi * ndx].y;
-      if(BORDER)
-      {
-#pragma unroll
-        for(int i = 0; i <= MSEG; i++) row_ok[i] = own_row[i] && (unsigned)(r0 + wr0 + i * S + dy) < (unsigned)H;
-      }
-      if(!(var & 16)) load_row_head(dy, dx0);
-      for(int jb = 0; jb < ndx; jb += 2)
-      {
-        if(!(var & 16))
-        {
-          step(std::integral_constant<int, 0>(), dyi * ndx + jb, dx0 + jb);
-          slide(std::integral_constant<int, 0>(), dy, dx0 + jb);
-        }
-        env.sync();
-        if(jb + 1 < ndx)
+          sx[i][PH] = v.x;
+          sy[i][PH] = v.y;
+          sz[i][PH] = Z[wi];
+        }
+      };
+      for(int dyi = 0; dyi < ndy; dyi++)
+      {
+        const int dy = patches[dyi * ndx].x, dx0 = patches[dyi * ndx].y;
+        if(BORDER)
+        {
+#pragma unroll
+          for(int i = 0; i <= MSEG; i++) row_ok[i] = own_row[i] && (unsigned)(r0 + wr0 + i * S + dy) < (unsigned)H;
+        }
+        if(!(var & 16)) load_row_head(dy, dx0);
+        for(int jb = 0; jb < ndx; jb += 2)
         {
           if(!(var & 16))
           {
-            step(std::integral_constant<int, 1>(), dyi * ndx + jb + 1, dx0 + jb + 1);
-            slide(std::integral_constant<int, 1>(), dy, dx0 + jb + 1);
-          }
-          env.sync();
-        }
-      }
-    }
-    env.sync();
-    env.sync();
-    if(!FUSED) env.sync();
+            step(std::integral_constant<int, 0>(), dyi * ndx + jb, dx0 + jb);
+            slide(std::integral_constant<int, 0>(), dy, dx0 + jb);
+          }
+          stage_sync();
+          if(jb + 1 < ndx)
+          {
+            if(!(var & 16))
+            {
+              step(std::integral_constant<int, 1>(), dyi * ndx + jb + 1, dx0 + jb + 1);
+              slide(std::integral_constant<int, 1>(), dy, dx0 + jb + 1);
+            }
+            stage_sync();
+          }
+        }
+      }
+      drain(0, pl, wk);
+    }
     return;
   }
   if(w < 2)
@@ -386,83 +449,89 @@
     const int x = 1 + w * 64 + lane;
     const bool active = x <= cw + 2 * P && !(var & 32);
     if(!(var & 512)) env.prio_high();
-    env.sync();
-    for(int p = 0; p < n; p++)
-    {
-      if(active)
-      {
-        float *const col = tab + tslot(p) * tabsz + XO + x;
-        const float *const F = Fb + (p & 1) * S * FP + XO + x;
-        float f[S], term[MAXCH];
-#pragma unroll
-        for(int r = 0; r < S; r++) f[r] = F[r * FP];
-#pragma unroll
-        for(int t = 1; t < MAXCH; t++) term[t] = col[t * TP];
-        float v = 0.0f;
-#pragma unroll
-        for(int r = 0; r < S; r++) v += f[r];
-        float *const wave_base = tab + tslot(p) * tabsz + XO + 1 + w * 64;
-        env.template st_addtid<0>(wave_base, lane, v);
-        column_chain<1, MAXCH, TP * 4, Env, !FUSED && P == 2 && !CENTER>::run(env, wave_base, lane, v, term);
-        if constexpr(TALL)
-        {
-          static_assert(!TALL || MAXCH == TALL_HEAD, "the exported sum is the one behind the head's last row");
-          seeds_out[(size_t)p * TALL_SEED_PITCH + x] = v;
-        }
-      }
-      env.sync();
-    }
-    env.sync();
-    if(!FUSED) env.sync();
+    const int pl = NL3_A1_LANES + w * 64 + lane;
+    for(int wk = 0; wk < m; wk++)
+    {
+      lead(1);
+      for(int p = 0; p < n; p++)
+      {
+        if(active)
+        {
+          float *const col = tab + tslot(p) * tabsz + XO + x;
+          const float *const F = Fb + (p & 1) * S * FP + XO + x;
+          float f[S], term[MAXCH];
+#pragma unroll
+          for(int r = 0; r < S; r++) f[r] = F[r * FP];
+#pragma unroll
+          for(int t = 1; t < MAXCH; t++) term[t] = col[t * TP];
+          float v = 0.0f;
+#pragma unroll
+          for(int r = 0; r < S; r++) v += f[r];
+          float *const wave_base = tab + tslot(p) * tabsz + XO + 1 + w * 64;
+          env.template st_addtid<0>(wave_base, lane, v);
+          column_chain<1, MAXCH, TP * 4, Env, !FUSED && P == 2 && !CENTER>::run(env, wave_base, lane, v, term);
+          if constexpr(TALL)
+          {
+            static_assert(!TALL || MAXCH == TALL_HEAD, "the exported sum is the one behind the head's last row");
+            seeds_out[(size_t)p * TALL_SEED_PITCH + x] = v;
+          }
+        }
+        stage_sync();
+      }
+      drain(1, pl, wk);
+    }
     return;
   }
   if(!FUSED && w == 2)
   {
     const bool active = lane < ch && !(var & 64);
     if(!(var & 512)) env.prio_high();
-    env.sync();
-    env.sync();
-    for(int p = 0; p < n; p++)
-    {
-      if(active)
-      {
-        float *const rowp = tab + (p & 3) * tabsz + lane * TP;
-        float cs[80];
-#pragma unroll
-        for(int b = 4; b < 80; b += 4)
-        {
-          const f4 v = ld4(rowp + b);
-          cs[b] = v.x;
-          cs[b + 1] = v.y;
-          cs[b + 2] = v.z;
-          cs[b + 3] = v.w;
-        }
-        cs[XO] = 0.0f;
-        float distortion = 0.0f;
-#pragma unroll
-        for(int kk = 1; kk < S; kk++) distortion += cs[XO + kk];
-        float d[72];
-#pragma unroll
-        for(int b = 0; b < 72; b += 4)
-        {
-#pragma unroll
-          for(int c = b; c < b + 4; c++)
-          {
-            distortion = distortion + (cs[XO + c + S] - cs[XO + c]);
-            d[c] = distortion;
-          }
-          f4 v;
-          v.x = d[b];
-          v.y = d[b + 1];
-          v.z = d[b + 2];
-          v.w = d[b + 3];
-          st4(rowp + 4 + b, v);
-          if(!(var & 1024)) env.sched_fence();
-        }
-      }
-      env.sync();
-    }
-    env.sync();
+    const int pl = NL3_A1_LANES + 128 + lane;
+    for(int wk = 0; wk < m; wk++)
+    {
+      lead(2);
+      for(int p = 0; p < n; p++)
+      {
+        if(active)
+        {
+          float *const rowp = tab + (p & 3) * tabsz + lane * TP;
+          float cs[80];
+#pragma unroll
+          for(int b = 4; b < 80; b += 4)
+          {
+            const f4 v = ld4(rowp + b);
+            cs[b] = v.x;
+            cs[b + 1] = v.y;
+            cs[b + 2] = v.z;
+            cs[b + 3] = v.w;
+          }
+          cs[XO] = 0.0f;
+          float distortion = 0.0f;
+#pragma unroll
+          for(int kk = 1; kk < S; kk++) distortion += cs[XO + kk];
+          float d[72];
+#pragma unroll
+          for(int b = 0; b < 72; b += 4)
+          {
+#pragma unroll
+            for(int c = b; c < b + 4; c++)
+            {
+              distortion = distortion + (cs[XO + c + S] - cs[XO + c]);
+              d[c] = distortion;
+            }
+            f4 v;
+            v.x = d[b];
+            v.y = d[b + 1];
+            v.z = d[b + 2];
+            v.w = d[b + 3];
+            st4(rowp + 4 + b, v);
+            if(!(var & 1024)) env.sched_fence();
+          }
+        }
+        stage_sync();
+      }
+      drain(2, pl, wk);
+    }
     return;
   }
   {
@@ -648,78 +717,7 @@
         env.sched_fence();
       }
     };
-    env.sync();
-    env.sync();
-    if(!FUSED) env.sync();
-    for(int dyi = 0; dyi < ndy; dyi++)
-    {
-      const int dy = patches[dyi * ndx].x, dx0 = patches[dyi * ndx].y;
-      for(int jb = 0; jb < ndx; jb += NR)
-      {
-        auto run = [&](auto m_tag) {
-          constexpr int M = decltype(m_tag)::value;
-          if constexpr(M < NR)
-          {
-            if(jb + M < ndx)
-            {
-              if constexpr(CENTER)
-              {
-                if(active && jb + M > 0) accumulate(std::integral_constant<int, (M + NR - 1) % NR>());
-                if constexpr(FUSED) fetch_sums(dyi * ndx + jb + M);
-                if(active) fetch(m_tag, dyi * ndx + jb + M, jb + M == 0, dy, dx0 + jb + M);
-                if constexpr(FUSED)
-                {
-                  if(!(var & 64)) row_chain(m_tag);
-                }
-                if(active && jb + M + 1 == ndx) accumulate(m_tag);
-              }
-              else if constexpr(FUSED)
-              {
-                if(active && jb + M > 0) accumulate(std::integral_constant<int, (M + NR - 1) % NR>());
-                env.sched_fence();
-                fetch_sums(dyi * ndx + jb + M);
-                if(active) fetch(m_tag, dyi * ndx + jb + M, jb + M == 0, dy, dx0 + jb + M);
-                if(!(var & 64)) row_chain(m_tag);
-                if(active && jb + M + 1 == ndx) accumulate(m_tag);
-              }
-              else if(active)
-              {
-                if(jb + M > 0) accumulate(std::integral_constant<int, (M + NR - 1) % NR>());
-                env.sched_fence();
-                fetch(m_tag, dyi * ndx + jb + M, jb + M == 0, dy, dx0 + jb + M);
-                if(jb + M + 1 == ndx) accumulate(m_tag);
-              }
-              env.sync();
-            }
-          }
-        };
-        run(std::integral_constant<int, 0>());
-        run(std::integral_constant<int, 1>());
-        run(std::integral_constant<int, 2>());
-        run(std::integral_constant<int, 3>());
-        run(std::integral_constant<int, 4>());
-        run(std::integral_constant<int, 5>());
-        run(std::integral_constant<int, 6>());
-        run(std::integral_constant<int, 7>());
-        run(std::integral_constant<int, 8>());
-        run(std::integral_constant<int, 9>());
-        if constexpr(NR > 10)
-        {
-          run(std::integral_constant<int, 10>());
-          run(std::integral_constant<int, 11>());
-          run(std::integral_constant<int, 12>());
-          run(std::integral_constant<int, 13>());
-        }
-      }
-    }
-    if(!active) return;
-    const int row = top + r;
-    if(row < a.out_row0 || row >= a.out_row1) return;
-#pragma unroll
-    for(int i = 0; i < NPXL; i++)
-    {
-      if(cb + i >= cw) continue;
-      const long o = (long)row * W + left + cb + i;
+    auto finish = [&](const int i, const long o, const F4 &ip) {
       F4 res;
       if(a.skip_blend)
       {
@@ -730,7 +728,6 @@
       }
       else
       {
-        const F4 ip = in[o];
         res.x = (ip.x * (1.0f - a.luma)) + (accx[i] / accw[i] * a.luma);
         res.y = (ip.y * (1.0f - a.chroma)) + (accy[i] / accw[i] * a.chroma);
         res.z = (ip.z * (1.0f - a.chroma)) + (accz[i] / accw[i] * a.chroma);
@@ -738,8 +735,114 @@
       }
       out[o] = res;
       env.store_cell(a, o, res.x);
+    };
+    for(int wk = 0; wk < m; wk++)
+    {
+      if constexpr(WALK)
+      {
+        if(wk > 0)
+        {
+          place(chunk_at(wk));
+#pragma unroll
+          for(int i = 0; i < NPXL; i++) accx[i] = accy[i] = accz[i] = accw[i] = dist[0][i] = dist[DB - 1][i] = 0.0f;
+#pragma unroll
+          for(int i = 0; i < NR; i++) qx[i] = qy[i] = qz[i] = 0.0f;
+        }
+      }
+      lead(FILL);
+      for(int dyi = 0; dyi < ndy; dyi++)
+      {
+        const int dy = patches[dyi * ndx].x, dx0 = patches[dyi * ndx].y;
+        for(int jb = 0; jb < ndx; jb += NR)
+        {
+          auto run = [&](auto m_tag) {
+            constexpr int M = decltype(m_tag)::value;
+            if constexpr(M < NR)
+            {
+              if(jb + M < ndx)
+              {
+                if constexpr(CENTER)
+                {
+                  if(active && jb + M > 0) accumulate(std::integral_constant<int, (M + NR - 1) % NR>());
+                  if constexpr(FUSED) fetch_sums(dyi * ndx + jb + M);
+                  if(active) fetch(m_tag, dyi * ndx + jb + M, jb + M == 0, dy, dx0 + jb + M);
+                  if constexpr(FUSED)
+                  {
+                    if(!(var & 64)) row_chain(m_tag);
+                  }
+                  if(active && jb + M + 1 == ndx) accumulate(m_tag);
+                }
+                else if constexpr(FUSED)
+                {
+                  if(active && jb + M > 0) accumulate(std::integral_constant<int, (M + NR - 1) % NR>());
+                  env.sched_fence();
+                  fetch_sums(dyi * ndx + jb + M);
+                  if(active) fetch(m_tag, dyi * ndx + jb + M, jb + M == 0, dy, dx0 + jb + M);
+                  if(!(var & 64)) row_chain(m_tag);
+                  if(active && jb + M + 1 == ndx) accumulate(m_tag);
+                }
+                else if(active)
+                {
+                  if(jb + M > 0) accumulate(std::integral_constant<int, (M + NR - 1) % NR>());
+                  env.sched_fence();
+                  fetch(m_tag, dyi * ndx + jb + M, jb + M == 0, dy, dx0 + jb + M);
+                  if(jb + M + 1 == ndx) accumulate(m_tag);
+                }
+                stage_sync();
+              }
+            }
+          };
+          run(std::integral_constant<int, 0>());
+          run(std::integral_constant<int, 1>());
+          run(std::integral_constant<int, 2>());
+          run(std::integral_constant<int, 3>());
+          run(std::integral_constant<int, 4>());
+          run(std::integral_constant<int, 5>());
+          run(std::integral_constant<int, 6>());
+          run(std::integral_constant<int, 7>());
+          run(std::integral_constant<int, 8>());
+          run(std::integral_constant<int, 9>());
+          if constexpr(NR > 10)
+          {
+            run(std::integral_constant<int, 10>());
+            run(std::integral_constant<int, 11>());
+            run(std::integral_constant<int, 12>());
+            run(std::integral_constant<int, 13>());
+          }
+        }
+      }
+      const int row = top + r;
+      if(active && row >= a.out_row0 && row < a.out_row1)
+      {
+#pragma unroll
+        for(int i = 0; i < NPXL; i++)
+        {
+          if(cb + i >= cw) continue;
+          const long o = (long)row * W + left + cb + i;
+          F4 ip;
+          ip.x = ip.y = ip.z = ip.w = 0.0f;
+          if(!a.skip_blend) ip = in[o];
+          finish(i, o, ip);
+        }
+      }
+      if(WALK && wk + 1 < m) env.sync();
     }
   }
 }
 
-}
+template <int NPXL, int MSEG, bool BORDER = false, bool FUSED = false, bool TALL = false, int P = 2, bool CENTER = false, class Env,
+          class Args, class F4, class I2>
+NLM2_FN void body(const Env &env, const F4 *__restrict__ in, F4 *__restrict__ out, const Args &a, const I2 *__restrict__ patches,
+                  const int ndx, float *__restrict__ seeds_out = nullptr)
+{
+  life<NPXL, MSEG, BORDER, FUSED, TALL, P, CENTER, false>(env, in, out, a, patches, ndx, seeds_out, (const int *)nullptr, 0, 0, 1);
+}
+
+template <int NPXL, int MSEG, int P = 2, bool CENTER = false, class Env, class Args, class F4, class I2>
+NLM2_FN void walk(const Env &env, const F4 *__restrict__ in, F4 *__restrict__ out, const Args &a, const I2 *__restrict__ patches,
+                  const int ndx, const int *__restrict__ order, const int first, const int stride, const int count)
+{
+  life<NPXL, MSEG, false, false, false, P, CENTER, true>(env, in, out, a, patches, ndx, (float *)nullptr, order, first, stride, count);
+}
+
+}
diff --git a/ansel_amd/csrc/nlmeans.hip b/ansel_amd/csrc/nlmeans.hip
--- a/ansel_amd/csrc/nlmeans.hip
+++ b/ansel_amd/csrc/nlmeans.hip
@@ -815,7 +815,8 @@
 template <int NPXL, int MSEG, int P = 2, bool CENTER = false>
 __global__ __launch_bounds__(NL3_THREADS) void nlm_chunks_v3(const float4 *__restrict__ in, float4 *__restrict__ out,
                                                              const nlm_args a_by_value, const int2 *__restrict__ patches,
-                                                             const int *__restrict__ order, const int n_border, const int ndx)
+                                                             const int *__restrict__ order, const int n_border, const int ndx,
+                                                             const int nchunks)
 {
   constexpr int at = kernarg_offset_after<nlm_args, const float4 *, float4 *>();
   static_assert(at == 16, "nlm_chunks_v3: the by-value nlm_args follows the two plane pointers");
@@ -834,7 +835,13 @@
     else nlm3::body<NPXL, MSEG, true, false, false, P, CENTER>(env, in, out, a, patches, ndx);
     return;
   }
-  nlm3::body<NPXL, MSEG, false, false, false, P, CENTER>(env, in, out, a, patches, ndx);
+  if constexpr(nlm3::walks<P, CENTER>())
+  {
+    const int b = (int)blockIdx.x - n_border, walkers = (int)gridDim.x - n_border;
+    const int count = (nchunks - n_border - b + walkers - 1) / walkers;
+    nlm3::walk<NPXL, MSEG, P, CENTER>(env, in, out, a, patches, ndx, order, n_border + b, walkers, count);
+  }
+  else nlm3::body<NPXL, MSEG, false, false, false, P, CENTER>(env, in, out, a, patches, ndx);
 }
 
 template <int NPXL, int MSEG, bool TALL, int P = 2, bool CENTER = false>
@@ -942,6 +949,7 @@
 
 enum { NLM_BODY_NONE = 0, NLM_BODY_TALL, NLM_BODY_V4, NLM_BODY_V3, NLM_BODY_V2, NLM_BODY_PIPELINED, NLM_BODY_STAGED, NLM_BODY_GLOBAL };
 static int g_nlm_last[8];
+static int g_nlm_last_grid;
 
 int nlmeans_core_launch(int devid, const float4 *in, float4 *out, int width, int height, const nlm_core_params_t &p)
 {
@@ -1047,7 +1055,7 @@
                   && (p1 ? nlm3::fits_fused<9, 7, 1>(a.chk_w, a.chk_h, a.radius, a.reach) : nlm3::fits_fused<9, 7>(a.chk_w, a.chk_h, a.radius, a.reach))
                   && nlm3::regular_grid(patches.data(), a.npatch, &ndx3)
                   && v4_bytes <= 160 * 1024 && !force_v2 && (force_fused || !(v3 && v3_bytes <= 160 * 1024));
-  typedef void (*nlm3_kernel_t)(const float4 *, float4 *, nlm_args, const int2 *, const int *, int, int);
+  typedef void (*nlm3_kernel_t)(const float4 *, float4 *, nlm_args, const int2 *, const int *, int, int, int);
   typedef void (*nlm4_kernel_t)(const float4 *, float4 *, nlm_args, const int2 *, const int *, int, int, float *);
   const nlm3_kernel_t k3 = p1 ? (center ? nlm_chunks_v3<9, 7, 1, true> : nlm_chunks_v3<9, 7, 1, false>)
                               : (center ? nlm_chunks_v3<9, 6, 2, true> : nlm_chunks_v3<9, 6, 2, false>);
@@ -1141,12 +1149,17 @@
   {
     launch_scope ls(devid, "nlm_chunks");
     const unsigned grid = (unsigned)nchunks;
+    const int ov_walk = dispatch_override(DISPATCH_NLM_WALK);
+    const bool walks = !p1 && (center ? nlm3::walks<2, true>() : nlm3::walks<2, false>()) && nlm3::walk_fits(a.chk_h, a.reach);
+    const int walkers = std::min(nchunks - n_border, ov_walk > 0 ? ov_walk : device_cus(devid));
+    const unsigned grid3 = !walks || ov_walk < 0 ? grid : (unsigned)(n_border + walkers);
+    g_nlm_last_grid = (int)(!tall && !v4 && v3 && v3_bytes <= 160 * 1024 ? grid3 : grid);
     if(tall)
       k4t<<<grid, NL3_THREADS, tall_bytes, s>>>(in, out, a, dev_patches, dev_order, n_border, ndx3, seeds);
     else if(v4)
       k4<<<grid, NL3_THREADS, v4_bytes, s>>>(in, out, a, dev_patches, dev_order, n_border, ndx3, nullptr);
     else if(v3 && v3_bytes <= 160 * 1024)
-      k3<<<grid, NL3_THREADS, v3_bytes, s>>>(in, out, a, dev_patches, dev_order, n_border, ndx3);
+      k3<<<grid3, NL3_THREADS, v3_bytes, s>>>(in, out, a, dev_patches, dev_order, n_border, ndx3, nchunks);
     else if(v2)
       k2<<<grid, NL2_THREADS, v2_bytes, s>>>(in, out, a, dev_patches, dev_order, n_border);
     else if(pipelined)
@@ -1178,6 +1191,8 @@
   memcpy(out, ansel::g_nlm_last, sizeof(ansel::g_nlm_last));
   return DT_HIP_SUCCESS;
 }
+
+int dt_hip_test_nlm_grid(void) { return ansel::g_nlm_last_grid; }
 
 int dt_hip_iop_nlmeans_process(int devid, const dt_hip_piece_t *piece, const dt_hip_nlmeans_data_t *d,
                                dt_hip_mem_t dev_in, dt_hip_mem_t dev_out)
diff --git a/ansel_amd/csrc/runtime.cpp b/ansel_amd/csrc/runtime.cpp
--- a/ansel_amd/csrc/runtime.cpp
+++ b/ansel_amd/csrc/runtime.cpp
@@ -21,6 +21,7 @@
 struct device_t
 {
   int hip_id = -1;
+  int cus = 1;
   std::string name;
   hipStream_t stream = nullptr;
   bool own_stream = false;
@@ -83,6 +84,7 @@
 }
 
 int hip_device_of(int devid) { return valid_device(devid) ? g_devs[devid]->hip_id : -1; }
+int device_cus(int devid) { return valid_device(devid) ? g_devs[devid]->cus : 1; }
 
 int upload_small(int devid, void *dst_dev, const void *src_host, size_t bytes)
 {
@@ -196,6 +198,7 @@
     device_t *d = new device_t;
     d->hip_id = i;
     d->name = prop.name[0] ? prop.name : prop.gcnArchName;
+    d->cus = prop.multiProcessorCount > 0 ? prop.multiProcessorCount : 1;
     if(hipSetDevice(i) != hipSuccess || hipStreamCreateWithFlags(&d->stream, hipStreamNonBlocking) != hipSuccess)
     {
       delete d;
diff --git a/ansel_amd/csrc/testhooks.hip b/ansel_amd/csrc/testhooks.hip
--- a/ansel_amd/csrc/testhooks.hip
+++ b/ansel_amd/csrc/testhooks.hip
@@ -11,7 +11,7 @@
 {
 std::atomic<int> g_dispatch[DISPATCH_KEYS];
 const char *const g_dispatch_names[DISPATCH_KEYS] = { "nlm_v2", "nlm_fused", "amaze_unfused", "amaze_slab", "amaze_blocks",
-                                                       "bilat_blur_split", "strip_rows" };
+                                                       "bilat_blur_split", "strip_rows", "nlm_walk" };
 }
 namespace ansel
 {
diff --git a/ansel_amd/lib.py b/ansel_amd/lib.py
--- a/ansel_amd/lib.py
+++ b/ansel_amd/lib.py
@@ -180,6 +180,7 @@
         "dt_hip_test_dispatch": (i, [C.c_char_p, i]),
         "dt_hip_test_strip_rows": (i, [i, i, i]),
         "dt_hip_test_nlm_last": (i, [P(i)]),
+        "dt_hip_test_nlm_grid": (i, []),
         "dt_hip_test_pool_fill": (i, [i, i, u]),
     }
     missing = []
@@ -224,6 +225,10 @@
     return d
 
 
+def test_nlm_grid():
+    return int(load().dt_hip_test_nlm_grid())
+
+
 def check(rc, what=""):
     if rc != abi.DT_HIP_SUCCESS:
         msg = load().dt_hip_last_error()
```

Result: no change. 1600 (-0.9%).
